# alibaba/EasyRec

Hardware: NVIDIA H100
Metric: samples_per_sec (higher is better)
Workload: dtype f32

## Files before the change

easyrec_b200/_lib.py:

```python
import ctypes
import os

import numpy as np

_HERE = os.path.dirname(os.path.abspath(__file__))
LIB_PATH = os.environ.get('ER_LIB_PATH') or os.path.join(_HERE, 'lib', 'liber_b200.so')

c_i32, c_i64, c_f32 = ctypes.c_int32, ctypes.c_int64, ctypes.c_float
c_vp, c_sz = ctypes.c_void_p, ctypes.c_size_t

SLOT_DTYPE = np.dtype(
    [('num_buckets', '<i8'), ('row_offset', '<i8'), ('seg_begin', '<i4'),
     ('n_seg', '<i4'), ('bucket_mode', '<i4'), ('combiner', '<i4'),
     ('out_buf', '<i4'), ('out_stride', '<i4'), ('out_col', '<i4'),
     ('shard_n', '<i4')],
    align=True)
assert SLOT_DTYPE.itemsize == 48
DENSE_SEG_DTYPE = np.dtype([('offset', '<i8'), ('n', '<i8'), ('l2', '<f4'), ('lr_mult', '<f4')], align=True)
assert DENSE_SEG_DTYPE.itemsize == 24

BUCKET_FARM_DECIMAL, BUCKET_MOD, BUCKET_IDENTITY, BUCKET_NONE, BUCKET_ONE_ROW = 0, 1, 2, 3, 4
COMBINER_SUM, COMBINER_MEAN, COMBINER_SQRTN = 0, 1, 2
COMBINER_UNIT_WEIGHTS = 16
OPT_SGD, OPT_ADAGRAD, OPT_LAZY_ADAM, OPT_ADAM_ROWS, OPT_MOMENTUM = 0, 1, 2, 3, 4
ACT_GELU, ACT_LEAKY_RELU, ACT_ELU, ACT_SELU, ACT_TANH, ACT_SWISH, ACT_SIGMOID = 1, 2, 3, 4, 5, 6, 7
MAX_BUFS = 8
ABI_VERSION = 3
HYPER_LR, HYPER_BETA1_POWER, HYPER_BETA2_POWER, HYPER_GRAD_SCALE, HYPER_N = 0, 1, 2, 3, 4


class ErOpt(ctypes.Structure):
  _fields_ = [('kind', c_i32), ('lr', c_f32), ('beta1', c_f32),
              ('beta2', c_f32), ('eps', c_f32), ('beta1_power', c_f32),
              ('beta2_power', c_f32), ('grad_scale', c_f32), ('hyper_dev', c_vp)]


class ErBnStats(ctypes.Structure):
  _fields_ = [('bias', c_vp), ('save_mean', c_vp), ('save_rstd', c_vp), ('moving_mean', c_vp),
              ('moving_var', c_vp), ('eps', c_f32), ('momentum', c_f32)]


class ErCsvCol(ctypes.Structure):
  _fields_ = [('kind', c_i32), ('width', c_i32), ('inner_sep', ctypes.c_char), ('kv_sep', ctypes.c_char), ('pad_', ctypes.c_char * 6),
              ('default_i64', c_i64), ('default_f32', c_f32), ('pad2_', c_i32), ('default_str', ctypes.c_char_p),
              ('out', c_vp), ('lens', c_vp), ('list_cap', c_i64), ('n_vals', c_i64), ('hash_mod', ctypes.c_uint64), ('weights', c_vp),
              ('step_lens', c_vp)]


ER_OK, ER_ERR_INVALID_ARG, ER_ERR_WORKSPACE, ER_ERR_CUDA, ER_ERR_UNSUPPORTED = range(5)
CSV_SKIP, CSV_I64, CSV_F32, CSV_HASH, CSV_I64_LIST, CSV_F32_VEC, CSV_HASH_LIST, CSV_I64_KV_LIST, CSV_HASH_KV_LIST, CSV_F32_LIST, \
    CSV_I64_STEP_LIST, CSV_HASH_STEP_LIST = range(12)

SIGNATURES = {
    'er_abi_version': (c_i32, []),
    'er_last_error': (ctypes.c_char_p, []),
    'er_launch_count': (ctypes.c_uint64, []),
    'er_csr_workspace_bytes': (c_sz, [c_i64]),
    'er_csr_from_lens': (c_i32, [c_vp, c_i64, c_vp, c_vp, c_i64, c_vp, c_sz,
                                 c_vp]),
    'er_bucketize': (c_i32, [c_vp, c_vp, c_vp, c_i64, c_i64, c_vp, c_i32,
                             c_vp, c_vp, c_vp]),
    'er_bucketize_weighted': (c_i32, [c_vp, c_vp, c_vp, c_vp, c_i64, c_i64, c_vp, c_i32,
                                      c_vp, c_vp, c_vp]),
    'er_bucketize_seq': (c_i32, [c_vp, c_vp, c_i64, c_i32, c_i32, c_vp, c_i32, c_vp, c_vp, c_vp]),
    'er_dropout': (c_i32, [c_vp, c_i64, ctypes.c_float, ctypes.c_uint64, c_vp, c_vp, c_vp]),
    'er_gemm_small_workspace_bytes': (c_sz, [c_i64, c_i64, c_i64]),
    'er_gemm_small': (c_i32, [c_vp, c_i64, c_i64, c_vp, c_i64, c_i64, c_vp, c_vp, c_i64, c_i64, c_i64, c_i64, c_vp, c_sz,
                              c_vp]),
    'er_dice_fwd': (c_i32, [c_vp, c_vp, c_vp, c_i64, c_i32, c_vp, c_vp]),
    'er_dice_bwd': (c_i32, [c_vp, c_vp, c_vp, c_vp, c_i64, c_i32, c_vp, c_vp, c_vp, c_vp]),
    'er_act_fwd': (c_i32, [c_vp, c_i64, c_i32, c_vp, c_vp]),
    'er_act_bwd': (c_i32, [c_vp, c_vp, c_i64, c_i32, c_vp, c_vp]),
    'er_auc_hist': (c_i32, [c_vp, c_vp, c_i64, c_vp, c_i32, c_vp, c_vp]),
    'er_shard_group_workspace_bytes': (c_sz, [c_i64]),
    'er_shard_group': (c_i32, [c_vp, c_vp, c_i64, c_i32, c_i64, c_vp, c_vp, c_vp, c_vp, c_sz, c_vp]),
    'er_fingerprint64_host': (ctypes.c_uint64, [ctypes.c_char_p, c_sz]),
    'er_csv_parse': (c_i32, [c_vp, c_sz, ctypes.c_char, ctypes.POINTER(ErCsvCol), c_i32, c_i64, c_i32,
                             ctypes.POINTER(c_i64), ctypes.POINTER(c_sz)]),
    'er_fingerprint64_i64': (c_i32, [c_vp, c_i64, c_vp]),
    'er_load_embed': (c_i32, [ctypes.c_char_p, ctypes.c_char_p, c_i32, c_i32, c_i32, c_i64, c_vp, c_vp]),
    'er_embedding_fwd': (c_i32, [
        c_vp, c_i64, c_i32, c_i32, c_vp, c_vp, c_vp, c_i64, c_i64, c_vp,
        c_i32, ctypes.POINTER(c_vp), c_i32, c_vp, c_vp
    ]),
    'er_embedding_bwd_workspace_bytes': (c_sz, [c_i64, c_i32]),
    'er_embedding_bwd_presort': (c_i32, [c_vp, c_i64, c_vp, c_vp, c_i64, c_i64, c_vp, c_i32, c_i32, c_vp, c_sz, c_vp]),
    'er_embedding_bwd_reuse_sort': (c_i32, [
        c_vp, c_vp, c_vp, c_i64, c_i32, c_i32, c_vp, c_vp, c_vp, c_vp, c_i64,
        c_i64, c_vp, c_i32, ctypes.POINTER(c_vp), c_i32, c_vp,
        ctypes.POINTER(ErOpt), c_vp, c_vp, c_vp, c_vp, c_sz, c_vp, c_sz, c_i32, c_vp
    ]),
    'er_embedding_bwd': (c_i32, [
        c_vp, c_vp, c_vp, c_i64, c_i32, c_i32, c_vp, c_vp, c_vp, c_vp, c_i64,
        c_i64, c_vp, c_i32, ctypes.POINTER(c_vp), c_i32, c_vp,
        ctypes.POINTER(ErOpt), c_vp, c_vp, c_vp, c_vp, c_sz, c_vp
    ]),
    'er_sparse_apply': (c_i32, [
        c_vp, c_vp, c_vp, c_i32, c_i32, c_vp, c_vp, c_vp, c_i64,
        ctypes.POINTER(ErOpt), c_vp
    ]),
    'er_adam_dense_sweep': (c_i32, [
        c_vp, c_vp, c_vp, c_i64, c_i32, c_i32, c_vp,
        ctypes.POINTER(ErOpt), c_vp
    ]),
    'er_mark_rows': (c_i32, [c_vp, c_i64, c_vp, c_i64, c_vp, c_i32, c_vp]),
    'er_sort_workspace_bytes': (c_sz, [c_i64]),
    'er_sort_rows': (c_i32, [c_vp, c_i64, c_vp, c_i64, c_vp, c_vp, c_vp, c_sz,
                             c_vp]),
    'er_fm_fwd': (c_i32, [c_vp, c_i64, c_i32, c_i32, c_i32, c_vp, c_vp]),
    'er_fm_bwd': (c_i32, [c_vp, c_vp, c_i64, c_i32, c_i32, c_i32, c_vp, c_i32,
                          c_i32, c_vp]),
    'er_sigmoid_ce_fwd_bwd': (c_i32, [c_vp, c_vp, c_vp, c_i64, c_f32, c_vp,
                                      c_vp, c_vp, c_vp]),
    'er_dense_workspace_bytes': (c_sz, [c_i64, c_i32]),
    'er_dense_apply': (c_i32, [c_vp, c_vp, c_vp, c_vp, c_vp, c_i32, c_i64, ctypes.POINTER(ErOpt), c_vp,
                               c_vp, c_vp]),
    'er_concat_cols': (c_i32, [ctypes.POINTER(c_vp), ctypes.POINTER(c_i32), ctypes.POINTER(c_i32), c_i32, c_i64,
                               c_vp, c_i32, c_vp]),
    'er_split_cols': (c_i32, [c_vp, c_i32, c_i64, ctypes.POINTER(c_vp), ctypes.POINTER(c_i32),
                              ctypes.POINTER(c_i32), c_i32, c_vp]),
    'er_rowsum_block_fwd': (c_i32, [c_vp, c_i64, c_i32, c_i32, c_vp, c_vp, c_vp, c_sz, c_vp]),
    'er_rowsum_block_bwd': (c_i32, [c_vp, c_vp, c_vp, c_f32, c_i64, c_i32, c_i32, c_vp, c_i32, c_vp]),
    'er_dense1_workspace_bytes': (c_sz, [c_i32]),
    'er_dense1_fwd': (c_i32, [c_vp, c_vp, c_vp, c_i64, c_i32, c_i32, c_vp, c_vp]),
    'er_dense1_bwd': (c_i32, [c_vp, c_vp, c_vp, c_i64, c_i32, c_i32, c_vp, c_i32, c_vp, c_vp, c_vp, c_sz, c_vp]),
    'er_gemm_bn_workspace_bytes': (c_sz, [c_i64, c_i64]),
    'er_gemm_bn': (c_i32, [c_vp, c_i64, c_i32, c_vp, c_i64, c_i32, c_vp, c_i64, c_i64, c_i64, c_i64,
                           ctypes.POINTER(ErBnStats), c_vp, c_sz, c_vp]),
    'er_bn_act_apply': (c_i32, [c_vp, c_vp, c_vp, c_vp, c_vp, c_vp, c_i64, c_i32, c_i32, c_vp, c_vp]),
    'er_fm_block_workspace_bytes': (c_sz, [c_i64]),
    'er_fm_block_fwd': (c_i32, [c_vp, c_i64, c_i32, c_i32, c_i32, c_vp, c_vp, c_vp, c_sz, c_vp]),
    'er_fm_block_bwd': (c_i32, [c_vp, c_vp, c_vp, c_vp, c_f32, c_i64, c_i32, c_i32, c_i32, c_i32, c_vp, c_i32,
                                c_vp]),
    'er_gemm_workspace_bytes': (c_sz, [c_i64, c_i64, c_i64]),
    'er_gemm': (c_i32, [c_vp, c_i64, c_i32, c_vp, c_i64, c_i32, c_vp, c_vp, c_i64, c_i64, c_i64, c_i64,
                        c_vp, c_sz, c_vp]),
    'er_bias_bn_act_fwd': (c_i32, [c_vp, c_vp, c_vp, c_vp, c_vp, c_vp, c_i64,
                                   c_i32, c_f32, c_f32, c_i32, c_i32, c_vp,
                                   c_vp, c_vp, c_vp, c_sz, c_vp]),
    'er_bias_bn_act_bwd': (c_i32, [c_vp, c_vp, c_vp, c_vp, c_vp, c_vp, c_vp,
                                   c_i64, c_i32, c_i32, c_vp, c_vp, c_vp, c_vp,
                                   c_vp, c_sz, c_vp]),
    'er_din_concat_fwd': (c_i32, [c_vp, c_vp, c_i64, c_i32, c_i32, c_vp, c_vp]),
    'er_din_concat_bwd': (c_i32, [c_vp, c_vp, c_vp, c_i64, c_i32, c_i32, c_vp, c_vp, c_i32, c_vp]),
    'er_din_pool_fwd': (c_i32, [c_vp, c_vp, c_vp, c_i64, c_i32, c_i32, c_vp, c_vp, c_vp]),
    'er_din_pool_bwd': (c_i32, [c_vp, c_vp, c_vp, c_vp, c_i64, c_i32, c_i32, c_vp, c_vp, c_i32, c_vp]),
    'er_din_sigmoid_pool_fwd': (c_i32, [c_vp, c_vp, c_vp, c_i64, c_i32, c_i32, c_f32, c_vp, c_vp, c_vp]),
    'er_din_sigmoid_pool_bwd': (c_i32, [c_vp, c_vp, c_vp, c_vp, c_i64, c_i32, c_i32, c_f32, c_vp, c_vp, c_i32,
                                        c_vp]),
    'er_cross_fwd': (c_i32, [c_vp, c_vp, c_vp, c_vp, c_i64, c_i32, c_vp, c_vp, c_vp]),
    'er_cross_workspace_bytes': (c_sz, [c_i64, c_i32]),
    'er_cross_bwd': (c_i32, [c_vp, c_vp, c_vp, c_vp, c_vp, c_i64, c_i32, c_vp, c_vp, c_vp, c_vp, c_i32,
                             c_vp, c_sz, c_vp]),
    'er_mmoe_mix_fwd': (c_i32, [c_vp, c_vp, c_i64, c_i32, c_i32, c_vp, c_vp, c_vp]),
    'er_mmoe_mix_bwd': (c_i32, [c_vp, c_vp, c_vp, c_i64, c_i32, c_i32, c_vp, c_vp, c_i32, c_vp]),
    'er_gram_fwd': (c_i32, [c_vp, c_i64, c_i32, c_i32, c_vp, c_vp]),
    'er_gram_bwd': (c_i32, [c_vp, c_vp, c_i64, c_i32, c_i32, c_vp, c_vp]),
    'er_l2norm_fwd': (c_i32, [c_vp, c_i64, c_i32, c_vp, c_vp, c_vp]),
    'er_l2norm_bwd': (c_i32, [c_vp, c_vp, c_vp, c_i64, c_i32, c_vp, c_vp]),
    'er_inbatch_softmax_ce': (c_i32, [c_vp, c_vp, c_vp, c_i64, c_i32, c_f32, c_vp, c_vp, c_vp, c_vp]),
}

_lib = None


class ErError(RuntimeError):
  pass


def load():
  global _lib
  if _lib is not None:
    return _lib
  if not os.path.exists(LIB_PATH):
    raise ErError(
        'liber_b200.so not found at %s: build it with '
        '`python -c "import __graft_entry__ as g; g.build()"` or '
        '`make -C easyrec_b200/csrc`. There is no CPU fallback.' % LIB_PATH)
  lib = ctypes.CDLL(LIB_PATH)
  for name, (res, args) in SIGNATURES.items():
    fn = getattr(lib, name)
    fn.restype = res
    fn.argtypes = args
  if lib.er_abi_version() != ABI_VERSION:
    raise ErError('liber_b200.so has ABI version %d, this binding needs %d: rebuild it (make -C easyrec_b200/csrc)'
                  % (lib.er_abi_version(), ABI_VERSION))
  _lib = lib
  return lib


def check(status, what):
  if status != 0:
    msg = load().er_last_error()
    raise ErError('%s failed (status %d): %s' %
                  (what, status, msg.decode() if msg else ''))


def fingerprint64(data):
  if isinstance(data, str):
    data = data.encode('utf-8')
  return int(load().er_fingerprint64_host(data, len(data)))
```

easyrec_b200/csrc/embedding_bwd.cu:

```cuda
#include "common.cuh"
#include "scan.cuh"
#include "slots.cuh"
#include "sort.cuh"
#include "bucket_bwd.cuh"

namespace er {

struct CBufs {
  const float* p[ER_MAX_BUFS];
};

constexpr int kLongRun = 64;
constexpr int kBatch = 4;
constexpr int kChunk = 512;

struct BwdArgs {
  float* table;
  float* state0;
  float* state1;
  int dim;
  int row_stride;
  uint32_t sentinel;
  const uint32_t* keys;
  const uint32_t* vals;
  const uint64_t* pairs;
  int64_t n;
  const float* weights;
  const int32_t* seg_ids;
  const er_slot_t* slots;
  int n_slots;
  CBufs gbufs;
  const float* seg_scale;
  er_opt_t opt;
  float lr_t;
  const float* hyper;
  int64_t* uniq_rows;
  float* uniq_grads;
  const int32_t* head_rank;
  int32_t* counters;
  int4* long_list;
  int32_t* run_done;
  int2* chunk_list;
  float* partials;
  const int64_t* or_rows;
  float* or_partials;
  int32_t* or_tickets;
  int or_chunks;
  int main_ctas;
};

__device__ __forceinline__ const float* grad_src(const BwdArgs& a, const SlotView& sv, uint32_t l,
                                                 float* coef) {
  const int32_t s = a.seg_ids ? a.seg_ids[l] : (int32_t)l;
  const SlotLite sl = slot_lite(sv, slot_of(sv, s));
  float c = (a.weights && !slot_unit_weights(sl)) ? a.weights[l] : 1.0f;
  if (a.seg_scale) c = __fmul_rn(c, a.seg_scale[s]);
  *coef = c;
  return a.gbufs.p[sl.misc & 0xff] + (int64_t)(s - sl.seg_begin) * sl.out_stride + sl.out_col;
}

struct Hyper {
  float lr, lr_t, grad_scale;
};

__device__ __forceinline__ Hyper load_hyper(const er_opt_t& o, float lr_t_arg, const float* __restrict__ hyper) {
  Hyper h;
  if (hyper) {
    h.lr = __ldg(hyper + ER_HYPER_LR);
    h.grad_scale = __ldg(hyper + ER_HYPER_GRAD_SCALE);
    h.lr_t = h.lr;
    if (o.kind == ER_OPT_LAZY_ADAM || o.kind == ER_OPT_ADAM_ROWS)
      h.lr_t = adam_lr_t_of(h.lr, __ldg(hyper + ER_HYPER_BETA1_POWER), __ldg(hyper + ER_HYPER_BETA2_POWER));
  } else {
    h.lr = o.lr;
    h.lr_t = lr_t_arg;
    h.grad_scale = o.grad_scale;
  }
  return h;
}

__device__ __forceinline__ void upd_one(const BwdArgs& a, const Hyper& h, float g, float& w, float& s0, float& s1) {
  switch (a.opt.kind) {
    case ER_OPT_ADAGRAD: {
      s0 = __fadd_rn(s0, __fmul_rn(g, g));
      w = __fsub_rn(w, __fmul_rn(__fmul_rn(h.lr, g), __frsqrt_rn(s0)));
      break;
    }
    case ER_OPT_LAZY_ADAM:
    case ER_OPT_ADAM_ROWS: {
      s0 = __fadd_rn(__fmul_rn(g, 1.0f - a.opt.beta1), __fmul_rn(s0, a.opt.beta1));
      s1 = __fadd_rn(__fmul_rn(__fmul_rn(g, g), 1.0f - a.opt.beta2), __fmul_rn(s1, a.opt.beta2));
      w = __fadd_rn(w, __fdiv_rn(__fmul_rn(-h.lr_t, s0), __fadd_rn(__fsqrt_rn(s1), a.opt.eps)));
      break;
    }
    case ER_OPT_MOMENTUM: {
      s0 = __fadd_rn(__fmul_rn(s0, a.opt.beta1), g);
      w = __fsub_rn(w, __fmul_rn(h.lr, s0));
      break;
    }
    default:
      w = __fsub_rn(w, __fmul_rn(h.lr, g));
  }
}

__device__ __forceinline__ void f4_fma_sep(float4& g, const float4& v, float c) {
  g.x = __fadd_rn(g.x, __fmul_rn(v.x, c));
  g.y = __fadd_rn(g.y, __fmul_rn(v.y, c));
  g.z = __fadd_rn(g.z, __fmul_rn(v.z, c));
  g.w = __fadd_rn(g.w, __fmul_rn(v.w, c));
}
__device__ __forceinline__ void f4_acc(float4& g, const float4& v) {
  g.x = __fadd_rn(g.x, v.x);
  g.y = __fadd_rn(g.y, v.y);
  g.z = __fadd_rn(g.z, v.z);
  g.w = __fadd_rn(g.w, v.w);
}

__device__ __forceinline__ float4 f4_scale1(const float4& v, float c) {
  return make_float4(__fmul_rn(v.x, c), __fmul_rn(v.y, c), __fmul_rn(v.z, c), __fmul_rn(v.w, c));
}

struct RowRegs {
  float4 w, s0, s1;
};

__device__ __forceinline__ RowRegs load_row(const BwdArgs& a, uint32_t row, int lane) {
  RowRegs r;
  r.w = r.s0 = r.s1 = make_float4(0.f, 0.f, 0.f, 0.f);
  if (!a.table) return r;
  const int64_t off = (int64_t)row * a.row_stride;
  r.w = reinterpret_cast<const float4*>(a.table + off)[lane];
  if (a.state0) r.s0 = reinterpret_cast<const float4*>(a.state0 + off)[lane];
  if (a.state1) r.s1 = reinterpret_cast<const float4*>(a.state1 + off)[lane];
  return r;
}

__device__ __forceinline__ void apply_row_vec(const BwdArgs& a, uint32_t row, int lane, float4 g,
                                              int64_t head_pos, RowRegs r) {
  const Hyper h = load_hyper(a.opt, a.lr_t, a.hyper);
  g.x = __fmul_rn(g.x, h.grad_scale);
  g.y = __fmul_rn(g.y, h.grad_scale);
  g.z = __fmul_rn(g.z, h.grad_scale);
  g.w = __fmul_rn(g.w, h.grad_scale);
  if (a.uniq_rows) {
    const int32_t u = a.head_rank[head_pos];
    if (lane == 0) a.uniq_rows[u] = (int64_t)row;
    reinterpret_cast<float4*>(a.uniq_grads + (int64_t)u * a.dim)[lane] = g;
  }
  if (!a.table) return;
  upd_one(a, h, g.x, r.w.x, r.s0.x, r.s1.x);
  upd_one(a, h, g.y, r.w.y, r.s0.y, r.s1.y);
  upd_one(a, h, g.z, r.w.z, r.s0.z, r.s1.z);
  upd_one(a, h, g.w, r.w.w, r.s0.w, r.s1.w);
  const int64_t off = (int64_t)row * a.row_stride;
  reinterpret_cast<float4*>(a.table + off)[lane] = r.w;
  if (a.state0) reinterpret_cast<float4*>(a.state0 + off)[lane] = r.s0;
  if (a.state1) reinterpret_cast<float4*>(a.state1 + off)[lane] = r.s1;
}

// ... 221 lines not shown
  }
}

template <int LANES>
__global__ void __launch_bounds__(256) bwd_scan_vec_kernel(const __grid_constant__ BwdArgs a) {
  extern __shared__ __align__(16) unsigned char s_raw[];
  const SlotView sv = load_slots(s_raw, a.slots, a.n_slots);
  constexpr int D4 = LANES;
  constexpr int GROUPS = 32 / LANES;
  float4* s_stage = reinterpret_cast<float4*>(s_raw + ((slot_smem_bytes(a.n_slots) + 15) & ~(size_t)15));
  const int warp = threadIdx.x >> 5, lane = threadIdx.x & 31;
  float4* my_stage = s_stage + (size_t)warp * 32 * D4;
  __shared__ int s_tail_lane[8][32];
  __shared__ int s_tail_head[8][32];
  const int64_t base = ((int64_t)blockIdx.x * 8 + warp) * 32;
  if (base >= a.n) return;
  const int64_t pos = base + lane;
  const bool in = pos < a.n;
  const uint32_t k = in ? a.keys[pos] : a.sentinel;
  const uint32_t l = in ? a.vals[pos] : 0u;
  const bool valid = in && k < a.sentinel;
  uint32_t kprev = __shfl_up_sync(0xffffffffu, k, 1);
  if (lane == 0) kprev = (base > 0) ? a.keys[base - 1] : ~k;
  uint32_t knext = __shfl_down_sync(0xffffffffu, k, 1);
  if (lane == 31) knext = (base + 32 < a.n) ? a.keys[base + 32] : ~k;
  const bool is_head = valid && (pos == 0 || kprev != k);
  const uint32_t k0 = __shfl_sync(0xffffffffu, k, 0);
  const int head0 = __shfl_sync(0xffffffffu, (int)is_head, 0);
  const bool owned = valid && (head0 || k != k0);
  bool is_tail = owned && (knext != k);
  const int cont = __shfl_sync(0xffffffffu, (int)(owned && knext == k), 31);
  const unsigned lt_mask = (1u << lane) - 1u;
  const unsigned tails0 = __ballot_sync(0xffffffffu, is_tail || (lane == 31 && cont));
  if (is_tail || (lane == 31 && cont)) s_tail_lane[warp][__popc(tails0 & lt_mask)] = lane;
  __syncwarp();
  const int n_tails = __popc(tails0);
  const int glane = lane % LANES, grp = lane / LANES;
  RowRegs row0, row1;
  uint32_t row0_key = a.sentinel, row1_key = a.sentinel;
  if (grp < n_tails) {
    const int tl = s_tail_lane[warp][grp];
    row0_key = a.keys[base + tl];
    row0 = load_row(a, row0_key, glane);
  }
  if (grp + GROUPS < n_tails) {
    const int tl = s_tail_lane[warp][grp + GROUPS];
    row1_key = a.keys[base + tl];
    row1 = load_row(a, row1_key, glane);
  }
  float4 g[D4];
#pragma unroll
  for (int c = 0; c < D4; ++c) g[c] = make_float4(0.f, 0.f, 0.f, 0.f);
  if (owned) {
    float coef;
    const float4* src = reinterpret_cast<const float4*>(grad_src(a, sv, l, &coef));
    float4 v[D4];
#pragma unroll
    for (int c = 0; c < D4; ++c) v[c] = src[c];
#pragma unroll
    for (int c = 0; c < D4; ++c) f4_fma_sep(g[c], v[c], coef);
  }
  int cnt = owned ? 1 : 0;
#pragma unroll
  for (int off = 1; off < 32; off <<= 1) {
    const uint32_t kk = __shfl_up_sync(0xffffffffu, k, off);
    const int oo = __shfl_up_sync(0xffffffffu, (int)owned, off);
    const int cc = __shfl_up_sync(0xffffffffu, cnt, off);
    const bool take = lane >= off && owned && oo && kk == k;
#pragma unroll
    for (int c = 0; c < D4; ++c) {
      float4 y;
      y.x = __shfl_up_sync(0xffffffffu, g[c].x, off);
      y.y = __shfl_up_sync(0xffffffffu, g[c].y, off);
      y.z = __shfl_up_sync(0xffffffffu, g[c].z, off);
      y.w = __shfl_up_sync(0xffffffffu, g[c].w, off);
      if (take) f4_acc(g[c], y);
    }
    if (take) cnt += cc;
  }
  int handed_off = 0;
  if (cont) {
    const uint32_t key = __shfl_sync(0xffffffffu, k, 31);
    int total = __shfl_sync(0xffffffffu, cnt, 31);
    const int64_t start = base + 32 - total;
    int64_t j = base + 32;
    while (true) {
      const int64_t p = j + lane;
      const bool m = p < a.n && a.keys[p] == key;
      const unsigned mm = __ballot_sync(0xffffffffu, m);
      float4 x[D4];
#pragma unroll
      for (int c = 0; c < D4; ++c) x[c] = make_float4(0.f, 0.f, 0.f, 0.f);
      if (m) {
        float coef;
        const float4* src = reinterpret_cast<const float4*>(grad_src(a, sv, a.vals[p], &coef));
#pragma unroll
        for (int c = 0; c < D4; ++c) f4_fma_sep(x[c], src[c], coef);
      }
#pragma unroll
      for (int o = 16; o >= 1; o >>= 1) {
#pragma unroll
        for (int c = 0; c < D4; ++c) {
          float4 y;
          y.x = __shfl_xor_sync(0xffffffffu, x[c].x, o);
          y.y = __shfl_xor_sync(0xffffffffu, x[c].y, o);
          y.z = __shfl_xor_sync(0xffffffffu, x[c].z, o);
          y.w = __shfl_xor_sync(0xffffffffu, x[c].w, o);
          f4_acc(x[c], y);
        }
      }
      if (lane == 31) {
#pragma unroll
        for (int c = 0; c < D4; ++c) f4_acc(g[c], x[c]);
      }
      const int got = __popc(mm);
      total += got;
      j += got;
      if (mm != 0xffffffffu) break;
      if (total >= kLongRun) {
        if (j < a.n && a.keys[j] == key) {
          if (lane == 0) enqueue_long(a, start, j, key);
          handed_off = 1;
        }
        break;
      }
    }
  }
  const bool finish = (is_tail || (lane == 31 && cont && !handed_off));
  if (finish) {
#pragma unroll
    for (int c = 0; c < D4; ++c) my_stage[lane * D4 + c] = g[c];
  }
  if (is_tail || (lane == 31 && cont))
    s_tail_head[warp][__popc(tails0 & lt_mask)] = (lane == 31 && cont && handed_off) ? -1 : cnt;
  __syncwarp();
  for (int r = grp; r < n_tails; r += GROUPS) {
    const int tl = s_tail_lane[warp][r];
    const int run_cnt = s_tail_head[warp][r];
    if (run_cnt < 0) continue;
    const uint32_t key = (r == grp) ? row0_key : (r == grp + GROUPS) ? row1_key : a.keys[base + tl];
    RowRegs row = (r == grp) ? row0 : (r == grp + GROUPS) ? row1 : load_row(a, key, glane);
    const int64_t head_pos = base + tl - (run_cnt - 1);
    apply_row_vec(a, key, glane, my_stage[tl * D4 + glane], head_pos, row);
  }
}

__device__ __forceinline__ uint32_t key_at(const BwdArgs& a, int64_t i) {
  return a.pairs ? (uint32_t)(a.pairs[i] >> 32) : a.keys[i];
}
__device__ __forceinline__ uint32_t val_at(const BwdArgs& a, int64_t i) {
  return a.pairs ? (uint32_t)a.pairs[i] : a.vals[i];
}

template <int LANES, int TPE>
__global__ void __launch_bounds__(256) bwd_long_vec_kernel(const __grid_constant__ BwdArgs a) {
  extern __shared__ __align__(16) unsigned char s_raw[];
  const SlotView sv = load_slots(s_raw, a.slots, a.n_slots);
  float4* s_part = reinterpret_cast<float4*>(s_raw + ((slot_smem_bytes(a.n_slots) + 15) & ~(size_t)15));
  __shared__ int s_last;
  constexpr int CH = LANES / TPE;
  constexpr int G = 256 / TPE;
  const int lane32 = threadIdx.x & 31, warp = threadIdx.x >> 5;
  const int sub = threadIdx.x % TPE;
  const int grp = threadIdx.x / TPE;
  const int n_chunks = a.counters[1];
  for (int x = blockIdx.x; x < n_chunks; x += gridDim.x) {
    const int2 qc = a.chunk_list[x];
    const int4 run = a.long_list[qc.x];
    const int64_t i = run.x;
    const int len = run.y, c0 = run.z, nch = run.w;
    const uint32_t key = key_at(a, i);
    const int e0 = qc.y * kChunk, e1 = min(len, e0 + kChunk);
    float4 g[CH];
#pragma unroll
    for (int c = 0; c < CH; ++c) g[c] = make_float4(0.f, 0.f, 0.f, 0.f);
    for (int e = e0 + grp; e < e1; e += 2 * G) {
      const bool two = (e + G < e1);
      float w0, w1 = 0.f;
      const float* p0 = grad_src(a, sv, val_at(a, i + e), &w0);
      const float* p1 = two ? grad_src(a, sv, val_at(a, i + e + G), &w1) : p0;
      float4 v0[CH], v1[CH];
#pragma unroll
      for (int c = 0; c < CH; ++c) {
        v0[c] = reinterpret_cast<const float4*>(p0)[sub * CH + c];
        v1[c] = reinterpret_cast<const float4*>(p1)[sub * CH + c];
      }
#pragma unroll
      for (int c = 0; c < CH; ++c) {
        f4_fma_sep(g[c], v0[c], w0);
        if (two) f4_fma_sep(g[c], v1[c], w1);
      }
    }
#pragma unroll
    for (int o = 16; o >= TPE; o >>= 1) {
#pragma unroll
      for (int c = 0; c < CH; ++c) {
        float4 y;
        y.x = __shfl_xor_sync(0xffffffffu, g[c].x, o);
        y.y = __shfl_xor_sync(0xffffffffu, g[c].y, o);
        y.z = __shfl_xor_sync(0xffffffffu, g[c].z, o);
        y.w = __shfl_xor_sync(0xffffffffu, g[c].w, o);
        f4_acc(g[c], y);
      }
    }
    if (lane32 < TPE) {
#pragma unroll
      for (int c = 0; c < CH; ++c) s_part[warp * LANES + lane32 * CH + c] = g[c];
    }
    __syncthreads();
    float4 tot = make_float4(0.f, 0.f, 0.f, 0.f);
    if (threadIdx.x < LANES) {
      for (int ww = 0; ww < 8; ++ww) f4_acc(tot, s_part[ww * LANES + threadIdx.x]);
    }
    bool finish = (nch == 1);
    if (nch > 1) {
      if (threadIdx.x < LANES)
        __stcg(reinterpret_cast<float4*>(a.partials + (int64_t)(c0 + qc.y) * a.dim) + threadIdx.x, tot);
      __threadfence();
      __syncthreads();
      if (threadIdx.x == 0) s_last = (atomicAdd(&a.run_done[qc.x], 1) == nch - 1);
      __syncthreads();
      finish = s_last != 0;
      if (finish && threadIdx.x < LANES) {
        __threadfence();
        tot = make_float4(0.f, 0.f, 0.f, 0.f);
        for (int c = 0; c < nch; ++c)
          f4_acc(tot, __ldcg(reinterpret_cast<const float4*>(a.partials + (int64_t)(c0 + c) * a.dim) +
                             threadIdx.x));
      }
    }
    if (finish && threadIdx.x < LANES) {
      RowRegs row = load_row(a, key, threadIdx.x);
      apply_row_vec(a, key, threadIdx.x, tot, i, row);
    }
    __syncthreads();
  }
}

__global__ void __launch_bounds__(256) bwd_runs_scalar_kernel(const __grid_constant__ BwdArgs a) {
  extern __shared__ __align__(16) unsigned char s_raw[];
  const SlotView sv = load_slots(s_raw, a.slots, a.n_slots);
  const int64_t t = (int64_t)blockIdx.x * blockDim.x + threadIdx.x;
  const int64_t i = t / a.dim;
  const int c = (int)(t - i * a.dim);
  if (i >= a.n) return;
  const uint32_t key = a.keys[i];
  if (key >= a.sentinel) return;
  if (i > 0 && a.keys[i - 1] == key) return;
  float g = 0.f;
  int64_t j = i;
  for (; j < a.n && a.keys[j] == key; ++j) {
    if (j - i >= kLongRun) {
      if (c == 0) enqueue_long(a, i, j, key);
      return;
    }
    float coef;
    const float* src = grad_src(a, sv, a.vals[j], &coef);
    g = __fadd_rn(g, __fmul_rn(src[c], coef));
  }
  apply_scalar(a, key, c, g, i);
}

__global__ void __launch_bounds__(256) bwd_long_scalar_kernel(const __grid_constant__ BwdArgs a) {
  extern __shared__ __align__(16) unsigned char s_raw[];
  const SlotView sv = load_slots(s_raw, a.slots, a.n_slots);
  __shared__ float s_w[8];
  __shared__ int s_last;
  const int lane32 = threadIdx.x & 31, warp = threadIdx.x >> 5;
  const int n_chunks = a.counters[1];
  for (int x = blockIdx.x; x < n_chunks; x += gridDim.x) {
    const int2 qc = a.chunk_list[x];
    const int4 run = a.long_list[qc.x];
    const int64_t i = run.x;
    const int len = run.y, c0 = run.z, nch = run.w;
    const uint32_t key = key_at(a, i);
    const int e0 = qc.y * kChunk, e1 = min(len, e0 + kChunk);
    for (int c = 0; c < a.dim; ++c) {
      float g = 0.f;
      for (int e = e0 + threadIdx.x; e < e1; e += 256) {
        float coef;
        const float* src = grad_src(a, sv, val_at(a, i + e), &coef);
        g = __fadd_rn(g, __fmul_rn(src[c], coef));
      }
#pragma unroll
      for (int o = 16; o >= 1; o >>= 1) g = __fadd_rn(g, __shfl_xor_sync(0xffffffffu, g, o));
      if (lane32 == 0) s_w[warp] = g;
      __syncthreads();
      if (threadIdx.x == 0) {
        float tot = 0.f;
        for (int ww = 0; ww < 8; ++ww) tot = __fadd_rn(tot, s_w[ww]);
        if (nch == 1)
          apply_scalar(a, key, c, tot, i);
        else
          __stcg(a.partials + (int64_t)(c0 + qc.y) * a.dim + c, tot);
      }
      __syncthreads();
    }
    if (nch > 1) {
      __threadfence();
      __syncthreads();
      if (threadIdx.x == 0) s_last = (atomicAdd(&a.run_done[qc.x], 1) == nch - 1);
      __syncthreads();
      if (s_last && (int)threadIdx.x < a.dim) {
        __threadfence();
        float tot = 0.f;
        for (int c = 0; c < nch; ++c)
          tot = __fadd_rn(tot, __ldcg(a.partials + (int64_t)(c0 + c) * a.dim + threadIdx.x));
        apply_scalar(a, key, (int)threadIdx.x, tot, i);
      }
      __syncthreads();
    }
  }
}

__global__ void __launch_bounds__(256) bwd_scan_d1_kernel(const __grid_constant__ BwdArgs a) {
  extern __shared__ __align__(16) unsigned char s_raw[];
  const SlotView sv = load_slots(s_raw, a.slots, a.n_slots);
  const int warp = threadIdx.x >> 5, lane = threadIdx.x & 31;
  const int64_t base = ((int64_t)blockIdx.x * 8 + warp) * 32;
  if (base >= a.n) return;
  const int64_t pos = base + lane;
  const bool in = pos < a.n;
  const uint32_t k = in ? a.keys[pos] : a.sentinel;
  const uint32_t l = in ? a.vals[pos] : 0u;
  const bool valid = in && k < a.sentinel;
  uint32_t kprev = __shfl_up_sync(0xffffffffu, k, 1);
  if (lane == 0) kprev = (base > 0) ? a.keys[base - 1] : ~k;
  uint32_t knext = __shfl_down_sync(0xffffffffu, k, 1);
  if (lane == 31) knext = (base + 32 < a.n) ? a.keys[base + 32] : ~k;
  const bool is_head = valid && (pos == 0 || kprev != k);
  const uint32_t k0 = __shfl_sync(0xffffffffu, k, 0);
  const int head0 = __shfl_sync(0xffffffffu, (int)is_head, 0);
  const bool owned = valid && (head0 || k != k0);
  const bool is_tail = owned && (knext != k);
  const int cont = __shfl_sync(0xffffffffu, (int)(owned && knext == k), 31);
  float g = 0.f;
  if (owned) {
    float coef;
    const float* src = grad_src(a, sv, l, &coef);
    g = __fmul_rn(src[0], coef);
  }
  int cnt = owned ? 1 : 0;
#pragma unroll
  for (int off = 1; off < 32; off <<= 1) {
    const uint32_t kk = __shfl_up_sync(0xffffffffu, k, off);
    const int oo = __shfl_up_sync(0xffffffffu, (int)owned, off);
    const int cc = __shfl_up_sync(0xffffffffu, cnt, off);
    const float y = __shfl_up_sync(0xffffffffu, g, off);
    if (lane >= off && owned && oo && kk == k) {
      g = __fadd_rn(g, y);
      cnt += cc;
    }
  }
  int handed_off = 0;
  if (cont) {
    const uint32_t key = __shfl_sync(0xffffffffu, k, 31);
    int total = __shfl_sync(0xffffffffu, cnt, 31);
    const int64_t start = base + 32 - total;
    int64_t j = base + 32;
    while (true) {
      const int64_t p = j + lane;
      const bool m = p < a.n && a.keys[p] == key;
      const unsigned mm = __ballot_sync(0xffffffffu, m);
      float x = 0.f;
      if (m) {
        float coef;
        const float* src = grad_src(a, sv, a.vals[p], &coef);
        x = __fmul_rn(src[0], coef);
      }
#pragma unroll
      for (int o = 16; o >= 1; o >>= 1) x = __fadd_rn(x, __shfl_xor_sync(0xffffffffu, x, o));
      if (lane == 31) g = __fadd_rn(g, x);
      const int got = __popc(mm);
      total += got;
      j += got;
      if (mm != 0xffffffffu) break;
      if (total >= kLongRun) {
        if (j < a.n && a.keys[j] == key) {
          if (lane == 0) enqueue_long(a, start, j, key);
          handed_off = 1;
        }
        break;
      }
    }
  }
  if (is_tail || (lane == 31 && cont && !handed_off)) apply_scalar(a, k, 0, g, pos - (cnt - 1));
}

#ifndef ER_BK_MINB
#define ER_BK_MINB 4
#endif

struct BkArgs {
  bk::Ws w;
  int log2_nb;
  int warp_ctas;
  int med_ctas;
};

template <int LANES>
__device__ __forceinline__ float4 sum_entries(const BwdArgs& a, const SlotView& sv, const uint64_t* sp, int j0, int j1,
                                              int lane) {
  float4 g = make_float4(0.f, 0.f, 0.f, 0.f);
  for (int j = j0; j < j1; j += kBatch) {
    float4 gv[kBatch];
    float c[kBatch];
#pragma unroll
    for (int u = 0; u < kBatch; ++u) {
      if (j + u < j1) {
        const float* src = grad_src(a, sv, (uint32_t)sp[j + u], &c[u]);
        gv[u] = reinterpret_cast<const float4*>(src)[lane];
      }
    }
#pragma unroll
    for (int u = 0; u < kBatch; ++u)
      if (j + u < j1) f4_fma_sep(g, gv[u], c[u]);
  }
  return g;
}

constexpr int kStageF4 = 1024;
constexpr uint32_t kDonePos = 0xFFFFFFFFu;

template <typename IdxT>
__device__ __forceinline__ bool run_is_long(const IdxT* s_start, int r) {
  return (int)s_start[r + 1] - (int)s_start[r] > bk::kCoopRun;
}

template <int LANES, int THREADS, typename IdxT>
__device__ __forceinline__ void process_runs_vec(const BwdArgs& a, const SlotView& sv, uint64_t* sp,
                                                 const IdxT* s_start, int R, float4* s_stage, float4* s_part,
                                                 int* s_coop, int* s_ncoop, int64_t queue_base) {
  constexpr int G = THREADS / LANES;
  constexpr int S_ENT = kStageF4 / LANES;
  const int grp = threadIdx.x / LANES, lane = threadIdx.x % LANES;
  if (threadIdx.x == 0) *s_ncoop = 0;
  __syncthreads();
  for (int r = threadIdx.x; r < R; r += THREADS)
    if (run_is_long(s_start, r)) s_coop[atomicAdd(s_ncoop, 1)] = r;
  __syncthreads();
  const int nco = *s_ncoop;
  for (int c = 0; c < nco; ++c) {
    const int r = s_coop[c];
    const int st = s_start[r], en = s_start[r + 1], len = en - st;
    if (queue_base >= 0 && len > bk::kQueueRun) {
      if (threadIdx.x == 0) enqueue_run(a, queue_base + st, len);
    } else {
      const int chunk = (len + G - 1) / G;
      const int j0 = st + grp * chunk, j1 = min(en, j0 + chunk);
      const float4 g = sum_entries<LANES>(a, sv, sp, j0, j1, lane);
      s_part[grp * LANES + lane] = g;
      __syncthreads();
      if (threadIdx.x < LANES) {
        const uint32_t key = (uint32_t)(sp[st] >> 32);
        RowRegs row = load_row(a, key, threadIdx.x);
        const int used = (len + chunk - 1) / chunk;
        float4 tot = make_float4(0.f, 0.f, 0.f, 0.f);
        for (int q = 0; q < used; ++q) f4_acc(tot, s_part[q * LANES + threadIdx.x]);
        apply_row_vec(a, key, threadIdx.x, tot, 0, row);
      }
    }
    __syncthreads();
    for (int i = st + threadIdx.x; i < en; i += THREADS) sp[i] |= (uint64_t)kDonePos;
  }
  __syncthreads();
  const int n = s_start[R];
  int r = grp;
  while (r < R && run_is_long(s_start, r)) r += G;
  RowRegs row;
  row.w = row.s0 = row.s1 = make_float4(0.f, 0.f, 0.f, 0.f);
  if (r < R) row = load_row(a, (uint32_t)(sp[s_start[r]] >> 32), lane);
  float4 acc = make_float4(0.f, 0.f, 0.f, 0.f);
  for (int c0 = 0; c0 < n; c0 += S_ENT) {
    const int c1 = min(n, c0 + S_ENT);
    for (int q = threadIdx.x; q < (c1 - c0) * LANES; q += THREADS) {
      const int e = q / LANES;
      const uint32_t pos = (uint32_t)sp[c0 + e];
      if (pos != kDonePos) {
        float coef;
        const float* src = grad_src(a, sv, pos, &coef);
        s_stage[q] = f4_scale1(reinterpret_cast<const float4*>(src)[q % LANES], coef);
      }
    }
    __syncthreads();
    while (r < R && (int)s_start[r] < c1) {
      const int st = s_start[r], en = s_start[r + 1];
      const int lo = max(st, c0), hi = min(en, c1);
      for (int i = lo; i < hi; ++i) f4_acc(acc, s_stage[(i - c0) * LANES + lane]);
      if (en > c1) break;
      const uint32_t key = (uint32_t)(sp[st] >> 32);
      int rn = r + G;
      while (rn < R && run_is_long(s_start, rn)) rn += G;
      RowRegs nxt;
      nxt.w = nxt.s0 = nxt.s1 = make_float4(0.f, 0.f, 0.f, 0.f);
      if (rn < R) nxt = load_row(a, (uint32_t)(sp[s_start[rn]] >> 32), lane);
      apply_row_vec(a, key, lane, acc, 0, row);
      acc = make_float4(0.f, 0.f, 0.f, 0.f);
      row = nxt;
      r = rn;
    }
    __syncthreads();
  }
}

template <int THREADS, typename IdxT>
__device__ __forceinline__ void process_runs_scalar(const BwdArgs& a, const SlotView& sv, uint64_t* sp,
                                                    const IdxT* s_start, int R, float* s_stagef, float* s_partf,
                                                    int* s_coop, int* s_ncoop, int64_t queue_base) {
  const int dim = a.dim;
  if (threadIdx.x == 0) *s_ncoop = 0;
  __syncthreads();
  for (int r = threadIdx.x; r < R; r += THREADS)
    if (run_is_long(s_start, r)) s_coop[atomicAdd(s_ncoop, 1)] = r;
  __syncthreads();
  const int nco = *s_ncoop;
  for (int cc = 0; cc < nco; ++cc) {
    const int r = s_coop[cc];
    const int st = s_start[r], en = s_start[r + 1], len = en - st;
    if (queue_base >= 0 && len > bk::kQueueRun) {
      if (threadIdx.x == 0) enqueue_run(a, queue_base + st, len);
    } else {
      const int chunk = (len + THREADS - 1) / THREADS;
      const int j0 = st + threadIdx.x * chunk, j1 = min(en, j0 + chunk);
      const int used = (len + chunk - 1) / chunk;
      for (int c = 0; c < dim; ++c) {
        float g = 0.f;
        for (int j = j0; j < j1; ++j) {
          float coef;
          const float* src = grad_src(a, sv, (uint32_t)sp[j], &coef);
          g = __fadd_rn(g, __fmul_rn(src[c], coef));
        }
        s_partf[threadIdx.x] = g;
        __syncthreads();
        if (threadIdx.x == 0) {
          float tot = 0.f;
          for (int q = 0; q < used; ++q) tot = __fadd_rn(tot, s_partf[q]);
          apply_scalar(a, (uint32_t)(sp[st] >> 32), c, tot, 0);
        }
        __syncthreads();
      }
    }
    __syncthreads();
    for (int i = st + threadIdx.x; i < en; i += THREADS) sp[i] |= (uint64_t)kDonePos;
  }
  __syncthreads();
  const int n = s_start[R];
  const int S_ENT = max(1, (kStageF4 * 4) / dim);
  const int total = R * dim;
  int idx = threadIdx.x;
  float acc = 0.f;
  for (int c0 = 0; c0 < n; c0 += S_ENT) {
    const int c1 = min(n, c0 + S_ENT);
    for (int q = threadIdx.x; q < (c1 - c0) * dim; q += THREADS) {
      const int e = q / dim;
      const uint32_t pos = (uint32_t)sp[c0 + e];
      if (pos != kDonePos) {
        float coef;
        const float* src = grad_src(a, sv, pos, &coef);
        s_stagef[q] = __fmul_rn(src[q - e * dim], coef);
      }
    }
    __syncthreads();
    while (idx < total) {
      const int r = idx / dim, c = idx - r * dim;
      if (run_is_long(s_start, r)) {
        idx += THREADS;
        continue;
      }
      const int st = s_start[r], en = s_start[r + 1];
      if (st >= c1) break;
      const int lo = max(st, c0), hi = min(en, c1);
      for (int i = lo; i < hi; ++i) acc = __fadd_rn(acc, s_stagef[(i - c0) * dim + c]);
      if (en > c1) break;
      apply_scalar(a, (uint32_t)(sp[st] >> 32), c, acc, 0);
      acc = 0.f;
      idx += THREADS;
    }
    __syncthreads();
  }
}

inline size_t bk_reduce_smem(int n_slots, int cap, int threads) {
  return ((slot_smem_bytes(n_slots) + 15) & ~(size_t)15) + (size_t)cap * 8 + (((size_t)(cap + 1) * 2 + 15) & ~(size_t)15) +
         (size_t)max(kStageF4, threads) * 16 + (size_t)(cap / bk::kCoopRun + 2) * 4 + 64;
}

struct BkSmem {
  uint64_t* pairs;
  uint16_t* start;
  float4* stage;
  float4* part;
  int* coop;
  int* ncoop;
};
__device__ __forceinline__ BkSmem bk_carve(unsigned char* s_raw, int n_slots, int cap, int threads) {
  BkSmem m;
  unsigned char* p = s_raw + ((slot_smem_bytes(n_slots) + 15) & ~(size_t)15);
  m.pairs = reinterpret_cast<uint64_t*>(p); p += (size_t)cap * 8;
  m.start = reinterpret_cast<uint16_t*>(p); p += ((size_t)(cap + 1) * 2 + 15) & ~(size_t)15;
  m.stage = reinterpret_cast<float4*>(p); p += (size_t)max(kStageF4, threads) * 16;
  m.part = m.stage;
  m.coop = reinterpret_cast<int*>(p); p += (size_t)(cap / bk::kCoopRun + 1) * 4;
  m.ncoop = reinterpret_cast<int*>(p);
  return m;
}

__device__ __forceinline__ void cx(uint64_t& lo, uint64_t& hi, bool up) {
  if ((lo > hi) == up) {
    const uint64_t t = lo;
    lo = hi;
    hi = t;
  }
}

template <int LANES>
struct WarpSmem {
  float4 stage[32 * LANES];
  float4 carry[LANES];
  uint32_t keys[32];
};

__device__ __forceinline__ void sort4(uint64_t (&x)[4], int P, int lane) {
  for (int kk = 2; kk <= P; kk <<= 1) {
    for (int j = kk >> 1; j > 0; j >>= 1) {
      if (j == 64) {
        cx(x[0], x[2], ((lane) & kk) == 0);
        cx(x[1], x[3], ((lane + 32) & kk) == 0);
      } else if (j == 32) {
        cx(x[0], x[1], ((lane) & kk) == 0);
        if (P > 64) cx(x[2], x[3], ((lane + 64) & kk) == 0);
      } else {
        const bool lower = (lane & j) == 0;
#pragma unroll
        for (int r = 0; r < 4; ++r) {
          if (r * 32 < P) {
            const uint64_t other = __shfl_xor_sync(0xffffffffu, x[r], j);
            const bool up = ((lane + 32 * r) & kk) == 0;
            if ((x[r] > other) == (lower == up)) x[r] = other;
          }
        }
      }
    }
  }
}

template <int LANES>
__device__ __forceinline__ void warp_bucket_vec(const BwdArgs& a, const SlotView& sv, const BkArgs& k, int b,
                                                WarpSmem<LANES>* ws) {
  constexpr int G = 32 / LANES;
  const int lane = threadIdx.x & 31;
  const int gi = lane / LANES, gl = lane % LANES;
  const int n = k.w.bcnt[b];
  if (n == 0 || n > bk::kWarpCap) return;
  const int64_t off = k.w.boff[b];
  uint64_t x[4];
#pragma unroll
  for (int r = 0; r < 4; ++r) {
    const int q = r * 32 + lane;
    x[r] = q < n ? k.w.pairs[off + q] : ~0ull;
  }
  sort4(x, n <= 32 ? 32 : (n <= 64 ? 64 : 128), lane);
  uint32_t carry_key = 0xFFFFFFFFu;
#pragma unroll
  for (int r = 0; r < 4; ++r) {
    if (r * 32 >= n) break;
    const uint32_t key = (uint32_t)(x[r] >> 32), pos = (uint32_t)x[r];
    const int nv = min(32, n - r * 32);
    const uint32_t next_first = (r < 3 && (r + 1) * 32 < n) ? __shfl_sync(0xffffffffu, (uint32_t)(x[r < 3 ? r + 1 : 3] >> 32), 0)
                                                            : 0xFFFFFFFFu;
    uint32_t prevk = __shfl_up_sync(0xffffffffu, key, 1);
    if (lane == 0) prevk = carry_key;
    const bool is_head = lane < nv && key != prevk;
    const unsigned H = __ballot_sync(0xffffffffu, is_head);
    const int nh = __popc(H);
    ws->keys[lane] = key;
    const float4 open_sum = ws->carry[gl];
    RowRegs row0, row1;
    row0.w = row0.s0 = row0.s1 = row1.w = row1.s0 = row1.s1 = make_float4(0.f, 0.f, 0.f, 0.f);
    {
      const unsigned h0 = __fns(H, 0, gi + 1), h1 = __fns(H, 0, gi + G + 1);
      const uint32_t k0 = __shfl_sync(0xffffffffu, key, h0 & 31), k1 = __shfl_sync(0xffffffffu, key, h1 & 31);
      if (gi < nh) row0 = load_row(a, k0, gl);
      if (gi + G < nh) row1 = load_row(a, k1, gl);
    }
#pragma unroll
    for (int t = 0; t < LANES; ++t) {
      const int e = t * G + gi;
      const uint32_t pe = __shfl_sync(0xffffffffu, pos, e);
      if (e < nv) {
        float coef;
        const float* src = grad_src(a, sv, pe, &coef);
        ws->stage[e * LANES + gl] = f4_scale1(reinterpret_cast<const float4*>(src)[gl], coef);
      }
    }
    __syncwarp();
    const uint32_t lastk = ws->keys[31];
    const bool chunk_open = (nv == 32) && next_first == lastk;
    const int lead = nh ? (__ffs(H) - 1) : nv;
    if (lead > 0 && gi == 0) {
      float4 acc = open_sum;
      for (int i = 0; i < lead; ++i) f4_acc(acc, ws->stage[i * LANES + gl]);
      if (lead == 32 && chunk_open) {
        ws->carry[gl] = acc;
      } else {
        RowRegs row = load_row(a, carry_key, gl);
        apply_row_vec(a, carry_key, gl, acc, 0, row);
      }
    }
    for (int q = gi; q < nh; q += G) {
      const int h = __fns(H, 0, q + 1);
      const unsigned rest = (h == 31) ? 0u : (H >> (h + 1)) << (h + 1);
      const int e_end = rest ? (__ffs(rest) - 1) : nv;
      const uint32_t kh = ws->keys[h];
      float4 acc = make_float4(0.f, 0.f, 0.f, 0.f);
      for (int i = h; i < e_end; ++i) f4_acc(acc, ws->stage[i * LANES + gl]);
      if (e_end == 32 && chunk_open) {
        ws->carry[gl] = acc;
      } else {
        RowRegs row = (q == gi) ? row0 : (q == gi + G) ? row1 : load_row(a, kh, gl);
        apply_row_vec(a, kh, gl, acc, 0, row);
      }
    }
    carry_key = chunk_open ? lastk : 0xFFFFFFFFu;
    __syncwarp();
  }
}

struct WarpSmem1 {
  float stage[32];
  float carry;
  uint32_t keys[32];
};

__device__ __forceinline__ void warp_bucket_d1(const BwdArgs& a, const SlotView& sv, const BkArgs& k, int b,
                                               WarpSmem1* ws) {
  const int lane = threadIdx.x & 31;
  const int n = k.w.bcnt[b];
  if (n == 0 || n > bk::kWarpCap) return;
  const int64_t off = k.w.boff[b];
  uint64_t x[4];
#pragma unroll
  for (int r = 0; r < 4; ++r) {
    const int q = r * 32 + lane;
    x[r] = q < n ? k.w.pairs[off + q] : ~0ull;
  }
  sort4(x, n <= 32 ? 32 : (n <= 64 ? 64 : 128), lane);
  uint32_t carry_key = 0xFFFFFFFFu;
#pragma unroll
  for (int r = 0; r < 4; ++r) {
    if (r * 32 >= n) break;
    const uint32_t key = (uint32_t)(x[r] >> 32), pos = (uint32_t)x[r];
    const int nv = min(32, n - r * 32);
    const uint32_t next_first = (r < 3 && (r + 1) * 32 < n) ? __shfl_sync(0xffffffffu, (uint32_t)(x[r < 3 ? r + 1 : 3] >> 32), 0)
                                                            : 0xFFFFFFFFu;
    uint32_t prevk = __shfl_up_sync(0xffffffffu, key, 1);
    if (lane == 0) prevk = carry_key;
    const bool is_head = lane < nv && key != prevk;
    const unsigned H = __ballot_sync(0xffffffffu, is_head);
    const int nh = __popc(H);
    ws->keys[lane] = key;
    const float open_sum = ws->carry;
    if (lane < nv) {
      float coef;
      const float* src = grad_src(a, sv, pos, &coef);
      ws->stage[lane] = __fmul_rn(src[0], coef);
    }
    __syncwarp();
    const uint32_t lastk = ws->keys[31];
    const bool chunk_open = (nv == 32) && next_first == lastk;
    const int lead = nh ? (__ffs(H) - 1) : nv;
    if (lead > 0 && lane == 31) {
      float acc = open_sum;
      for (int i = 0; i < lead; ++i) acc = __fadd_rn(acc, ws->stage[i]);
      if (lead == 32 && chunk_open)
        ws->carry = acc;
      else
        apply_scalar(a, carry_key, 0, acc, 0);
    }
    if (lane < nh && !(lead > 0 && lane == 31)) {
      const int h = __fns(H, 0, lane + 1);
      const unsigned rest = (h == 31) ? 0u : (H >> (h + 1)) << (h + 1);
      const int e_end = rest ? (__ffs(rest) - 1) : nv;
      float acc = 0.f;
      for (int i = h; i < e_end; ++i) acc = __fadd_rn(acc, ws->stage[i]);
      if (e_end == 32 && chunk_open)
        ws->carry = acc;
      else
        apply_scalar(a, ws->keys[h], 0, acc, 0);
    }
    carry_key = chunk_open ? lastk : 0xFFFFFFFFu;
    __syncwarp();
  }
}

constexpr bool warp_mode_lanes(int lanes) { return lanes == 1 || lanes == 2 || lanes == 4 || lanes == 8; }

template <int LANES>
inline size_t bk_fused_smem(int n_slots, bool warp_mode) {
  size_t warp_bytes = 0;
  if (warp_mode) {
    if constexpr (LANES > 0)
      warp_bytes = ((slot_smem_bytes(n_slots) + 15) & ~(size_t)15) + 8 * sizeof(WarpSmem<(LANES > 0 && LANES <= 8) ? LANES : 1>);
    else
      warp_bytes = ((slot_smem_bytes(n_slots) + 15) & ~(size_t)15) + 8 * sizeof(WarpSmem1);
  }
  const size_t med = bk_reduce_smem(n_slots, bk::kCap, bk::kThreads);
  return warp_bytes > med ? warp_bytes : med;
}

template <int LANES>
__global__ void __launch_bounds__(bk::kThreads, ER_BK_MINB) bk_fused_kernel(const __grid_constant__ BwdArgs a,
                                                                const __grid_constant__ BkArgs k) {
  extern __shared__ __align__(16) unsigned char s_raw[];
  __shared__ int s_warp[bk::kThreads / 32 + 1];
  const int bid = blockIdx.x;
  if (bid >= k.warp_ctas + k.med_ctas) {
    one_row_cta<LANES>(a, bid - k.warp_ctas - k.med_ctas);
    return;
  }
  const SlotView sv = load_slots(s_raw, a.slots, a.n_slots);
  if (bid < k.warp_ctas) {
    unsigned char* p = s_raw + ((slot_smem_bytes(a.n_slots) + 15) & ~(size_t)15);
    const int b = bid * 8 + (threadIdx.x >> 5);
    if constexpr (LANES > 0 && LANES <= 8) {
      warp_bucket_vec<LANES>(a, sv, k, b, reinterpret_cast<WarpSmem<LANES>*>(p) + (threadIdx.x >> 5));
    } else if constexpr (LANES == 0) {
      warp_bucket_d1(a, sv, k, b, reinterpret_cast<WarpSmem1*>(p) + (threadIdx.x >> 5));
    }
    return;
  }
  const BkSmem m = bk_carve(s_raw, a.n_slots, bk::kCap, bk::kThreads);
  const int n_med = k.w.n_big[1];
  for (int xi = bid - k.warp_ctas; xi < n_med; xi += k.med_ctas) {
    const int b = k.w.med_list[xi];
    const int n = k.w.bcnt[b];
    const int off = k.w.boff[b];
    int P = 32;
    while (P < n) P <<= 1;
    for (int i = threadIdx.x; i < P; i += bk::kThreads) m.pairs[i] = i < n ? k.w.pairs[off + i] : ~0ull;
    __syncthreads();
    bk::bitonic_sort<bk::kThreads>(m.pairs, P);
    const int R = bk::run_starts<bk::kThreads, bk::kCap / bk::kThreads>(m.pairs, n, m.start, s_warp);
    if constexpr (LANES > 0)
      process_runs_vec<LANES, bk::kThreads>(a, sv, m.pairs, m.start, R, m.stage, m.part, m.coop, m.ncoop, -1);
    else
      process_runs_scalar<bk::kThreads>(a, sv, m.pairs, m.start, R, reinterpret_cast<float*>(m.stage),
                                        reinterpret_cast<float*>(m.part), m.coop, m.ncoop, -1);
    __syncthreads();
  }
}

__device__ __forceinline__ bool cta_radix_pass(const uint64_t* __restrict__ in, uint64_t* __restrict__ out, int n,
                                               int shift, int* s_wh , int* s_cur ) {
  const int lane = threadIdx.x & 31, wid = threadIdx.x >> 5;
  const unsigned lt_mask = (1u << lane) - 1u;
  for (int i = threadIdx.x; i < 256; i += bk::kBigThreads) s_cur[i] = 0;
  __syncthreads();
  for (int i = threadIdx.x; i < n; i += bk::kBigThreads) atomicAdd(&s_cur[(int)((in[i] >> shift) & 255)], 1);
  __syncthreads();
  int single = 0;
  if (threadIdx.x < 256) single = (s_cur[threadIdx.x] == n);
  if (__syncthreads_or(single)) return false;
  if (threadIdx.x < 32) {
    int carry = 0;
    for (int base = 0; base < 256; base += 32) {
      const int v = s_cur[base + lane];
      int incl = v;
#pragma unroll
      for (int o = 1; o < 32; o <<= 1) {
        const int t = __shfl_up_sync(0xffffffffu, incl, o);
        if (lane >= o) incl += t;
      }
      s_cur[base + lane] = carry + incl - v;
      carry += __shfl_sync(0xffffffffu, incl, 31);
    }
  }
  __syncthreads();
  for (int base = 0; base < n; base += bk::kBigThreads) {
    for (int i = threadIdx.x; i < 32 * 256; i += bk::kBigThreads) s_wh[i] = 0;
    __syncthreads();
    const int i = base + threadIdx.x;
    const bool valid = i < n;
    const uint64_t e = valid ? in[i] : 0ull;
    const int d = (int)((e >> shift) & 255);
    const unsigned peers = __match_any_sync(0xffffffffu, valid ? d : (256 + lane));
    const int r = __popc(peers & lt_mask);
    if (valid && r == 0) s_wh[wid * 256 + d] = __popc(peers);
    __syncthreads();
    if (threadIdx.x < 256) {
      int run = s_cur[threadIdx.x];
      for (int ww = 0; ww < 32; ++ww) {
        const int t = s_wh[ww * 256 + threadIdx.x];
        s_wh[ww * 256 + threadIdx.x] = run;
        run += t;
      }
      s_cur[threadIdx.x] = run;
    }
    __syncthreads();
    if (valid) out[s_wh[wid * 256 + d] + r] = e;
    __syncthreads();
  }
  return true;
}

template <int LANES>
__global__ void __launch_bounds__(bk::kBigThreads) bk_reduce_big_kernel(const __grid_constant__ BwdArgs a,
                                                                        const __grid_constant__ BkArgs k) {
  extern __shared__ __align__(16) unsigned char s_raw[];
  __shared__ int s_warp[bk::kBigThreads / 32 + 1];
  __shared__ int s_flag;
  const int n_big = k.w.n_big[0];
  if ((int)blockIdx.x >= n_big) return;
  const SlotView sv = load_slots(s_raw, a.slots, a.n_slots);
  const BkSmem m = bk_carve(s_raw, a.n_slots, bk::kBigCap, bk::kBigThreads);
  for (int x = blockIdx.x; x < n_big; x += gridDim.x) {
    const int b = k.w.big_list[x];
    const int n = k.w.bcnt[b];
    const int64_t off = k.w.boff[b];
    uint64_t* gp = k.w.pairs + off;
    bool sorted_in_global = false;
    if (n > bk::kBigCap) {
      int* s_wh = reinterpret_cast<int*>(m.pairs);
      int* s_cur = s_wh + 32 * 256;
      uint64_t* src = gp;
      uint64_t* dst = k.w.pairs_tmp + off;
      for (int shift = 0; shift < 64; shift += 8) {
        if (cta_radix_pass(src, dst, n, shift, s_wh, s_cur)) {
          uint64_t* t = src; src = dst; dst = t;
        }
        __syncthreads();
      }
      if (src != gp) {
        for (int i = threadIdx.x; i < n; i += bk::kBigThreads) gp[i] = src[i];
      }
      __threadfence_block();
      __syncthreads();
      sorted_in_global = true;
    }
    int p = 0;
    while (p < n) {
      const int mwin = min(bk::kBigCap, n - p);
      if (!sorted_in_global) {
        int P = 32;
        while (P < mwin) P <<= 1;
        for (int i = threadIdx.x; i < P; i += bk::kBigThreads) m.pairs[i] = i < mwin ? gp[i] : ~0ull;
        __syncthreads();
        bk::bitonic_sort<bk::kBigThreads>(m.pairs, P);
      } else {
        for (int i = threadIdx.x; i < mwin; i += bk::kBigThreads) m.pairs[i] = gp[p + i];
        __syncthreads();
      }
      int R = bk::run_starts<bk::kBigThreads, bk::kBigCap / bk::kBigThreads>(m.pairs, mwin, m.start, s_warp);
      int advance = mwin;
      if (sorted_in_global && p + mwin < n &&
          (uint32_t)(m.pairs[mwin - 1] >> 32) == (uint32_t)(gp[p + mwin] >> 32)) {
        if (R == 1) {
          const uint32_t key = (uint32_t)(m.pairs[0] >> 32);
          int lo = p + mwin, hi = n;
          while (lo < hi) {
            const int mid = (lo + hi) >> 1;
            if ((uint32_t)(gp[mid] >> 32) <= key) lo = mid + 1; else hi = mid;
          }
          if (threadIdx.x == 0) enqueue_run(a, off + p, lo - p);
          p = lo;
          __syncthreads();
          continue;
        }
        advance = m.start[R - 1];
        R -= 1;
      }
      if (!sorted_in_global) {
        if (threadIdx.x == 0) s_flag = 0;
        __syncthreads();
        for (int r = threadIdx.x; r < R; r += bk::kBigThreads)
          if (m.start[r + 1] - m.start[r] > bk::kQueueRun) s_flag = 1;
        __syncthreads();
        if (s_flag)
          for (int i = threadIdx.x; i < mwin; i += bk::kBigThreads) gp[i] = m.pairs[i];
      }
      if constexpr (LANES > 0)
        process_runs_vec<LANES, bk::kBigThreads>(a, sv, m.pairs, m.start, R, m.stage, m.part, m.coop, m.ncoop, off + p);
      else
        process_runs_scalar<bk::kBigThreads>(a, sv, m.pairs, m.start, R, reinterpret_cast<float*>(m.stage),
                                             reinterpret_cast<float*>(m.part), m.coop, m.ncoop, off + p);
      p += advance;
      __syncthreads();
    }
  }
}

struct HeadIn {
  const uint32_t* keys;
  uint32_t sentinel;
  __device__ int operator()(int64_t j) const {
    uint32_t k = keys[j];
    return (k < sentinel && (j == 0 || keys[j - 1] != k)) ? 1 : 0;
  }
};
struct HeadOut {
  int32_t* rank;
  __device__ void operator()(int64_t j, int ex, int) const { rank[j] = ex; }
};

inline size_t a256(size_t x) { return (x + 255) & ~(size_t)255; }

struct BwdWs {
  uint32_t* keys;
  uint32_t* vals;
  int32_t* head_rank;
  int4* long_list;
  int32_t* run_done;
  int2* chunk_list;
  float* partials;
  int32_t* counters;
  void* sort_ws;
  void* scan_ws;
  bk::Ws bk;
  int32_t* tickets;
  float* one_row_partials;
};

inline int64_t max_long_runs(int64_t n) { return n / kLongRun + 1; }
inline int64_t max_chunks(int64_t n) { return n / kChunk + max_long_runs(n) + 1; }
inline int64_t max_one_row_parts(int64_t n) { return n / bk::kOneRowChunk + 2048 + 1; }

inline BwdWs bwd_carve(void* ws, int64_t n, int dim, char** end = nullptr) {
  char* p = reinterpret_cast<char*>(a256(reinterpret_cast<size_t>(ws)));
  BwdWs w;
  w.keys = reinterpret_cast<uint32_t*>(p); p += a256((size_t)n * 4);
  w.vals = reinterpret_cast<uint32_t*>(p); p += a256((size_t)n * 4);
  w.head_rank = reinterpret_cast<int32_t*>(p); p += a256((size_t)n * 4);
  w.long_list = reinterpret_cast<int4*>(p); p += a256((size_t)max_long_runs(n) * 16);
  w.run_done = reinterpret_cast<int32_t*>(p); p += a256((size_t)max_long_runs(n) * 4);
  w.chunk_list = reinterpret_cast<int2*>(p); p += a256((size_t)max_chunks(n) * 8);
  w.partials = reinterpret_cast<float*>(p); p += a256((size_t)max_chunks(n) * dim * 4);
  w.bk = bk::carve(p, n, &w.counters, &w.tickets, &p);
  w.one_row_partials = reinterpret_cast<float*>(p); p += a256((size_t)max_one_row_parts(n) * dim * 4);
  w.sort_ws = p; p += a256(rsort::workspace_bytes(n));
  w.scan_ws = p; p += a256(scan::workspace_bytes(n));
  if (end) *end = p;
  return w;
}

inline size_t bwd_ws_bytes(int64_t n, int dim) {
  char* end;
  bwd_carve(nullptr, n, dim, &end);
  return reinterpret_cast<size_t>(end) + 768;
}

static float adam_lr_t(const er_opt_t& o) { return adam_lr_t_of(o.lr, o.beta1_power, o.beta2_power); }

template <int LANES>
static void launch_long(const BwdArgs& a, cudaStream_t st) {
  const size_t sl = slot_smem_bytes(a.n_slots);
  if constexpr (LANES > 0) {
    constexpr int TPE = (LANES <= 8) ? 1 : LANES;
    const size_t smem_long = ((sl + 15) & ~(size_t)15) + (size_t)8 * LANES * sizeof(float4);
    bwd_long_vec_kernel<LANES, TPE><<<4 * kSmCount, 256, smem_long, st>>>(a);
  } else {
    bwd_long_scalar_kernel<<<4 * kSmCount, 256, sl, st>>>(a);
  }
}

template <int LANES>
static void launch_radix(const BwdArgs& a, cudaStream_t st) {
  const size_t smem = slot_smem_bytes(a.n_slots);
  const unsigned grid = (unsigned)ceil_div(a.n, 256);
  if constexpr (LANES > 8) {
    bwd_runs_vec_kernel<LANES><<<grid, 256, smem, st>>>(a);
  } else if constexpr (LANES > 0) {
    const size_t smem_scan = ((smem + 15) & ~(size_t)15) + (size_t)8 * 32 * LANES * sizeof(float4);
    bwd_scan_vec_kernel<LANES><<<grid, 256, smem_scan, st>>>(a);
  } else if (a.dim == 1) {
    bwd_scan_d1_kernel<<<grid, 256, smem, st>>>(a);
  } else {
    bwd_runs_scalar_kernel<<<(unsigned)ceil_div(a.n * a.dim, 256), 256, smem, st>>>(a);
  }
  launch_long<LANES>(a, st);
  count_launches(2);
}

static int log2_of(int v) {
  int l = 0;
  while ((1 << l) < v) ++l;
  return l;
}

static bool k7_warp_mode(int dim) { return dim == 1 || dim == 4 || dim == 8 || dim == 16 || dim == 32; }

static void bk_place(const int64_t* rows, int64_t cap, const int32_t* n_dev, int64_t n_rows, const int32_t* seg_ids,
                     const er_slot_t* slots, int n_slots, bool one_row, bool warp_mode, const BwdWs& w,
                     bool zero_call_block, cudaStream_t st) {
  bk::PlaceArgs pa;
  pa.rows = rows;
  pa.cap = cap;
  pa.n_dev = n_dev;
  pa.sentinel = (uint32_t)n_rows;
  pa.seg_ids = seg_ids;
  pa.slots = one_row ? slots : nullptr;
  pa.n_slots = n_slots;
  const int nb = bk::num_buckets(cap, warp_mode);
  pa.log2_nb = log2_of(nb);
  pa.warp_cap = warp_mode ? bk::kWarpCap : 0;
  pa.w = w.bk;
  cudaMemsetAsync(w.bk.bcnt, 0, bk::zero_place_bytes() + (zero_call_block ? bk::zero_call_bytes() : 0), st);
  const size_t smem = bk::place_smem_bytes(n_slots, nb, pa.slots != nullptr);
  static bool attr = false;
  if (!attr) {
    const int mx = (int)bk::place_smem_bytes(2048, bk::kMaxBuckets, true);
    cudaFuncSetAttribute(bk::bk_count_kernel, cudaFuncAttributeMaxDynamicSharedMemorySize, mx);
    cudaFuncSetAttribute(bk::bk_place_kernel, cudaFuncAttributeMaxDynamicSharedMemorySize, mx);
    attr = true;
  }
  const unsigned tiles = (unsigned)ceil_div(cap, (int64_t)bk::kTile);
  bk::bk_count_kernel<<<tiles, bk::kTileThreads, smem, st>>>(pa);
  bk::bk_place_kernel<<<tiles, bk::kTileThreads, smem, st>>>(pa);
  count_launches(2);
}

template <int LANES>
static void bk_launch_fused(BwdArgs a, const BwdWs& place, bool place_warp_mode, cudaStream_t st) {
  BkArgs k;
  k.w = place.bk;
  const int nb = bk::num_buckets(a.n, place_warp_mode);
  k.log2_nb = log2_of(nb);
  k.warp_ctas = place_warp_mode ? (nb >> 3) : 0;
  k.med_ctas = place_warp_mode ? kSmCount : nb;
  const size_t smem = bk_fused_smem<LANES>(a.n_slots, place_warp_mode);
  const size_t smem_big = bk_reduce_smem(a.n_slots, bk::kBigCap, bk::kBigThreads);
  static bool attr = false;
  if (!attr) {
    cudaFuncSetAttribute(bk_fused_kernel<LANES>, cudaFuncAttributeMaxDynamicSharedMemorySize,
                         (int)bk_fused_smem<LANES>(2048, true));
    cudaFuncSetAttribute(bk_fused_kernel<LANES>, cudaFuncAttributePreferredSharedMemoryCarveout,
                         (int)cudaSharedmemCarveoutMaxShared);
    cudaFuncSetAttribute(bk_reduce_big_kernel<LANES>, cudaFuncAttributeMaxDynamicSharedMemorySize,
                         (int)bk_reduce_smem(2048, bk::kBigCap, bk::kBigThreads));
    attr = true;
  }
  const int extra = a.or_chunks * a.n_slots;
  a.main_ctas = k.warp_ctas + k.med_ctas;
  bk_fused_kernel<LANES><<<k.warp_ctas + k.med_ctas + extra, bk::kThreads, smem, st>>>(a, k);
  bk_reduce_big_kernel<LANES><<<kSmCount, bk::kBigThreads, smem_big, st>>>(a, k);
  launch_long<LANES>(a, st);
  count_launches(3);
}

}

extern "C" size_t er_sort_workspace_bytes(int64_t n) { return er::rsort::workspace_bytes(n > 0 ? n : 1); }

extern "C" int er_sort_rows(const int64_t* rows, int64_t n, const int32_t* n_dev, int64_t max_row,
                            uint32_t* keys_out, uint32_t* vals_out, void* ws, size_t ws_bytes,
                            er_stream_t stream) {
  using namespace er;
  ER_REQUIRE(rows && keys_out && vals_out, "null argument");
  ER_REQUIRE(n > 0 && n < (1LL << 31), "n out of range");
  ER_REQUIRE(max_row > 0 && max_row < 0xFFFFFFFFLL, "max_row must be in (0, 2^32-1)");
  if (!ws || ws_bytes < rsort::workspace_bytes(n))
    return fail(ER_ERR_WORKSPACE, "er_sort_rows: workspace too small");
  rsort::sort_rows(rows, n, n_dev, max_row, keys_out, vals_out, ws, nullptr, as_stream(stream));
  ER_CUDA_LAUNCH_CHECK();
  return ER_OK;
}

extern "C" size_t er_embedding_bwd_workspace_bytes(int64_t n_lookups_cap, int32_t dim) {
  return er::bwd_ws_bytes(n_lookups_cap > 0 ? n_lookups_cap : 1, dim > 0 ? dim : 1);
}

static int embedding_bwd_impl(float* table, float* state0, float* state1, int64_t n_rows,
                              int32_t dim, int32_t row_stride, const int64_t* rows,
                              const float* weights, const int32_t* seg_ids,
                              const int32_t* row_ptr, int64_t n_seg, int64_t n_lookups_cap,
                              const er_slot_t* slots, int32_t n_slots,
                              const float* const* grad_bufs, int32_t n_bufs,
                              const float* seg_scale, const er_opt_t* opt, int64_t* uniq_rows,
                              float* uniq_grads, int32_t* n_uniq, void* ws, size_t ws_bytes,
                              const void* sorted_ws, size_t sorted_ws_bytes, int32_t sorted_dim,
                              er_stream_t stream) {
  using namespace er;
  ER_REQUIRE(rows && slots && grad_bufs && opt, "null argument");
  ER_REQUIRE(table || uniq_rows, "nothing to do: table and uniq_rows are both NULL");
  ER_REQUIRE((uniq_rows == nullptr) == (uniq_grads == nullptr) &&
                 (uniq_rows == nullptr) == (n_uniq == nullptr),
             "uniq_rows, uniq_grads and n_uniq go together");
  ER_REQUIRE(dim > 0 && row_stride >= dim, "bad dim / row_stride");
  ER_REQUIRE(n_rows > 0 && n_rows < 0xFFFFFFFFLL, "n_rows must be in (0, 2^32-1)");
  ER_REQUIRE(n_slots > 0 && n_slots <= 2048, "n_slots must be in [1, 2048]");
  ER_REQUIRE(n_bufs > 0 && n_bufs <= ER_MAX_BUFS, "n_bufs must be in [1, ER_MAX_BUFS]");
  ER_REQUIRE(n_lookups_cap >= 0 && n_lookups_cap < (1LL << 31), "n_lookups_cap out of range");
  ER_REQUIRE(row_ptr || seg_ids || n_lookups_cap == n_seg,
             "without row_ptr / seg_ids every segment must hold exactly one lookup");
  ER_REQUIRE(!row_ptr || seg_ids, "CSR input needs seg_ids (er_csr_from_lens)");
  if (table) {
    const int k = opt->kind;
    ER_REQUIRE(k == ER_OPT_SGD || k == ER_OPT_ADAGRAD || k == ER_OPT_LAZY_ADAM || k == ER_OPT_ADAM_ROWS || k == ER_OPT_MOMENTUM,
               "unknown optimizer kind");
    ER_REQUIRE(k == ER_OPT_SGD || state0, "optimizer state0 missing");
    ER_REQUIRE((k != ER_OPT_LAZY_ADAM && k != ER_OPT_ADAM_ROWS) || state1, "adam needs state1 (v)");
  }
  if (n_lookups_cap == 0) return ER_OK;
  if (!ws || ws_bytes < bwd_ws_bytes(n_lookups_cap, dim))
    return fail(ER_ERR_WORKSPACE, "er_embedding_bwd: workspace too small");
  cudaStream_t st = as_stream(stream);
  BwdWs w = bwd_carve(ws, n_lookups_cap, dim);
  const int32_t* n_dev = row_ptr ? row_ptr + n_seg : nullptr;
  const bool bucketed = (uniq_rows == nullptr);
  const bool one_row = bucketed && seg_ids == nullptr;
  BwdWs src = w;
  if (sorted_ws) {
    if (sorted_ws_bytes < bwd_ws_bytes(n_lookups_cap, sorted_dim))
      return fail(ER_ERR_WORKSPACE, "er_embedding_bwd_reuse_sort: source workspace too small");
    if (!bucketed)
      return fail(ER_ERR_UNSUPPORTED, "er_embedding_bwd_reuse_sort: uniq_rows output needs the rows (er_embedding_bwd)");
    if (k7_warp_mode(sorted_dim) != k7_warp_mode(dim))
      return fail(ER_ERR_UNSUPPORTED, "er_embedding_bwd_reuse_sort: the placement was made in the other placement mode "
                                      "(warp-sized buckets for dims 1, 4, 8, 16 and 32, CTA-sized for the others)");
    src = bwd_carve(const_cast<void*>(sorted_ws), n_lookups_cap, sorted_dim);
    cudaMemsetAsync(w.counters, 0, bk::zero_call_bytes(), st);
  } else if (bucketed) {
    bk_place(rows, n_lookups_cap, n_dev, n_rows, seg_ids, slots, n_slots, one_row, k7_warp_mode(dim), w, true, st);
  } else {
    rsort::sort_rows(rows, n_lookups_cap, n_dev, n_rows, w.keys, w.vals, w.sort_ws, w.counters, st);
  }
  const bool place_warp = k7_warp_mode(dim);

  BwdArgs a = {};
  a.table = table;
  a.state0 = state0;
  a.state1 = state1;
  a.dim = dim;
  a.row_stride = row_stride;
  a.sentinel = (uint32_t)n_rows;
  a.keys = w.keys;
  a.vals = w.vals;
  a.pairs = nullptr;
  a.n = n_lookups_cap;
  a.weights = weights;
  a.seg_ids = seg_ids;
  a.slots = slots;
  a.n_slots = n_slots;
  bool aligned = true;
  for (int i = 0; i < ER_MAX_BUFS; ++i) {
    a.gbufs.p[i] = i < n_bufs ? grad_bufs[i] : nullptr;
    if (i < n_bufs) {
      ER_REQUIRE(grad_bufs[i] != nullptr, "null gradient buffer");
      aligned = aligned && (reinterpret_cast<uintptr_t>(grad_bufs[i]) % 16 == 0);
    }
  }
  a.seg_scale = seg_scale;
  a.opt = *opt;
  a.lr_t = (opt->kind == ER_OPT_LAZY_ADAM || opt->kind == ER_OPT_ADAM_ROWS) ? adam_lr_t(*opt) : opt->lr;
  a.hyper = opt->hyper_dev;
  a.uniq_rows = uniq_rows;
  a.uniq_grads = uniq_grads;
  a.head_rank = nullptr;
  a.counters = w.counters;
  a.long_list = w.long_list;
  a.run_done = w.run_done;
  a.chunk_list = w.chunk_list;
  a.partials = w.partials;
  a.or_rows = rows;
  a.or_partials = w.one_row_partials;
  a.or_tickets = w.tickets;
  a.or_chunks = one_row ? (int)ceil_div(ceil_div(n_lookups_cap, (int64_t)n_slots), (int64_t)bk::kOneRowChunk) : 0;
  if (uniq_rows) {
    scan::exclusive_scan(HeadIn{w.keys, a.sentinel}, HeadOut{w.head_rank}, n_lookups_cap, n_uniq,
                         w.scan_ws, st);
    a.head_rank = w.head_rank;
    count_launches(3);
  }
  if (table) {
    aligned = aligned && reinterpret_cast<uintptr_t>(table) % 16 == 0 && row_stride % 4 == 0 &&
              (!state0 || reinterpret_cast<uintptr_t>(state0) % 16 == 0) &&
              (!state1 || reinterpret_cast<uintptr_t>(state1) % 16 == 0);
  }
  if (uniq_grads) aligned = aligned && reinterpret_cast<uintptr_t>(uniq_grads) % 16 == 0;
  const bool vec_dim = (dim == 4 || dim == 8 || dim == 16 || dim == 32 || dim == 64 || dim == 128);
  if (bucketed) {
    ER_REQUIRE(table != nullptr, "the bucketed path updates a table");
    a.keys = nullptr;
    a.vals = nullptr;
    a.pairs = src.bk.pairs;
    if (vec_dim && aligned) {
      switch (dim / 4) {
        case 1: bk_launch_fused<1>(a, src, place_warp, st); break;
        case 2: bk_launch_fused<2>(a, src, place_warp, st); break;
        case 4: bk_launch_fused<4>(a, src, place_warp, st); break;
        case 8: bk_launch_fused<8>(a, src, place_warp, st); break;
        case 16: bk_launch_fused<16>(a, src, place_warp, st); break;
        default: bk_launch_fused<32>(a, src, place_warp, st); break;
      }
    } else {
      bk_launch_fused<0>(a, src, place_warp, st);
    }
    ER_CUDA_LAUNCH_CHECK();
    return ER_OK;
  }
  if (vec_dim && aligned) {
    switch (dim / 4) {
      case 1: launch_radix<1>(a, st); break;
      case 2: launch_radix<2>(a, st); break;
      case 4: launch_radix<4>(a, st); break;
      case 8: launch_radix<8>(a, st); break;
      case 16: launch_radix<16>(a, st); break;
      default: launch_radix<32>(a, st); break;
    }
  } else {
    launch_radix<0>(a, st);
  }
  ER_CUDA_LAUNCH_CHECK();
  return ER_OK;
}

extern "C" int er_embedding_bwd(float* table, float* state0, float* state1, int64_t n_rows,
                                int32_t dim, int32_t row_stride, const int64_t* rows,
                                const float* weights, const int32_t* seg_ids,
                                const int32_t* row_ptr, int64_t n_seg, int64_t n_lookups_cap,
                                const er_slot_t* slots, int32_t n_slots,
                                const float* const* grad_bufs, int32_t n_bufs,
                                const float* seg_scale, const er_opt_t* opt, int64_t* uniq_rows,
                                float* uniq_grads, int32_t* n_uniq, void* ws, size_t ws_bytes,
                                er_stream_t stream) {
  return embedding_bwd_impl(table, state0, state1, n_rows, dim, row_stride, rows, weights, seg_ids, row_ptr,
                            n_seg, n_lookups_cap, slots, n_slots, grad_bufs, n_bufs, seg_scale, opt,
                            uniq_rows, uniq_grads, n_uniq, ws, ws_bytes, nullptr, 0, 0, stream);
}

extern "C" int er_embedding_bwd_presort(const int64_t* rows, int64_t n_rows, const int32_t* seg_ids,
                                        const int32_t* row_ptr, int64_t n_seg, int64_t n_lookups_cap,
                                        const er_slot_t* slots, int32_t n_slots, int32_t dim, void* ws,
                                        size_t ws_bytes, er_stream_t stream) {
  using namespace er;
  ER_REQUIRE(rows && slots, "null argument");
  ER_REQUIRE(n_rows > 0 && n_rows < 0xFFFFFFFFLL, "n_rows must be in (0, 2^32-1)");
  ER_REQUIRE(n_slots > 0 && n_slots <= 2048, "n_slots must be in [1, 2048]");
  ER_REQUIRE(n_lookups_cap >= 0 && n_lookups_cap < (1LL << 31) && dim > 0, "bad shape");
  if (n_lookups_cap == 0) return ER_OK;
  if (!ws || ws_bytes < bwd_ws_bytes(n_lookups_cap, dim))
    return fail(ER_ERR_WORKSPACE, "er_embedding_bwd_presort: workspace too small");
  BwdWs w = bwd_carve(ws, n_lookups_cap, dim);
  const int32_t* n_dev = row_ptr ? row_ptr + n_seg : nullptr;
  bk_place(rows, n_lookups_cap, n_dev, n_rows, seg_ids, slots, n_slots, seg_ids == nullptr, k7_warp_mode(dim), w, false,
           as_stream(stream));
  ER_CUDA_LAUNCH_CHECK();
  return ER_OK;
}

extern "C" int er_embedding_bwd_reuse_sort(float* table, float* state0, float* state1, int64_t n_rows,
                                           int32_t dim, int32_t row_stride, const int64_t* rows,
                                           const float* weights, const int32_t* seg_ids,
                                           const int32_t* row_ptr, int64_t n_seg, int64_t n_lookups_cap,
                                           const er_slot_t* slots, int32_t n_slots,
                                           const float* const* grad_bufs, int32_t n_bufs,
                                           const float* seg_scale, const er_opt_t* opt, int64_t* uniq_rows,
                                           float* uniq_grads, int32_t* n_uniq, void* ws, size_t ws_bytes,
                                           const void* sorted_ws, size_t sorted_ws_bytes,
                                           int32_t sorted_dim, er_stream_t stream) {
  if (!sorted_ws) return er::fail(ER_ERR_INVALID_ARG, "er_embedding_bwd_reuse_sort: sorted_ws is NULL");
  if (!rows) return er::fail(ER_ERR_INVALID_ARG, "er_embedding_bwd_reuse_sort: rows is NULL");
  return embedding_bwd_impl(table, state0, state1, n_rows, dim, row_stride, rows, weights, seg_ids,
                            row_ptr, n_seg, n_lookups_cap, slots, n_slots, grad_bufs, n_bufs, seg_scale,
                            opt, uniq_rows, uniq_grads, n_uniq, ws, ws_bytes, sorted_ws, sorted_ws_bytes,
                            sorted_dim, stream);
}

namespace er {

__global__ void __launch_bounds__(256)
    sparse_apply_kernel(const __grid_constant__ BwdArgs a, const int64_t* __restrict__ uniq_rows,
                        const float* __restrict__ uniq_grads, const int32_t* __restrict__ n_uniq,
                        int64_t n_cap) {
  const int64_t n = n_uniq ? (int64_t)(*n_uniq < n_cap ? *n_uniq : n_cap) : n_cap;
  const Hyper h = load_hyper(a.opt, a.lr_t, a.hyper);
  for (int64_t t = (int64_t)blockIdx.x * blockDim.x + threadIdx.x; t < n * a.dim;
       t += (int64_t)gridDim.x * blockDim.x) {
    const int64_t u = t / a.dim;
    const int c = (int)(t - u * a.dim);
    const int64_t row = uniq_rows[u];
    if (row < 0) continue;
    const int64_t off = row * a.row_stride + c;
    float g = __fmul_rn(uniq_grads[u * a.dim + c], h.grad_scale);
    float w = a.table[off];
    float s0 = a.state0 ? a.state0[off] : 0.f;
    float s1 = a.state1 ? a.state1[off] : 0.f;
    upd_one(a, h, g, w, s0, s1);
    a.table[off] = w;
    if (a.state0) a.state0[off] = s0;
    if (a.state1) a.state1[off] = s1;
  }
}

struct SweepArgs {
  float* table;
  float* m;
  float* v;
  int64_t n_rows;
  int dim;
  int row_stride;
  const uint8_t* touched;
  er_opt_t opt;
  float lr_t;
  const float* hyper;
};

__device__ __forceinline__ void sweep_one(float& w, float& m, float& v, float b1, float b2, float eps, float lr_t) {
  m = __fmul_rn(m, b1);
  v = __fmul_rn(v, b2);
  w = __fsub_rn(w, __fdiv_rn(__fmul_rn(lr_t, m), __fadd_rn(__fsqrt_rn(v), eps)));
}

__global__ void __launch_bounds__(256) adam_sweep_vec_kernel(const __grid_constant__ SweepArgs a) {
  const Hyper h = load_hyper(a.opt, a.lr_t, a.hyper);
  const int d4 = a.dim >> 2;
  const int64_t total = a.n_rows * d4;
  for (int64_t t = (int64_t)blockIdx.x * blockDim.x + threadIdx.x; t < total;
       t += (int64_t)gridDim.x * blockDim.x) {
    const int64_t r = t / d4;
    const int c = (int)(t - r * d4);
    if (a.touched && a.touched[r]) continue;
    const int64_t off = r * a.row_stride;
    float4* pm = reinterpret_cast<float4*>(a.m + off) + c;
    float4* pv = reinterpret_cast<float4*>(a.v + off) + c;
    float4 m = *pm, v = *pv;
    if (m.x == 0.f && m.y == 0.f && m.z == 0.f && m.w == 0.f && v.x == 0.f && v.y == 0.f && v.z == 0.f &&
        v.w == 0.f)
      continue;
    float4* pw = reinterpret_cast<float4*>(a.table + off) + c;
    float4 w = *pw;
    sweep_one(w.x, m.x, v.x, a.opt.beta1, a.opt.beta2, a.opt.eps, h.lr_t);
    sweep_one(w.y, m.y, v.y, a.opt.beta1, a.opt.beta2, a.opt.eps, h.lr_t);
    sweep_one(w.z, m.z, v.z, a.opt.beta1, a.opt.beta2, a.opt.eps, h.lr_t);
    sweep_one(w.w, m.w, v.w, a.opt.beta1, a.opt.beta2, a.opt.eps, h.lr_t);
    *pm = m;
    *pv = v;
    *pw = w;
  }
}

__global__ void __launch_bounds__(256) adam_sweep_kernel(const __grid_constant__ SweepArgs a) {
  const Hyper h = load_hyper(a.opt, a.lr_t, a.hyper);
  const int64_t total = a.n_rows * a.dim;
  for (int64_t t = (int64_t)blockIdx.x * blockDim.x + threadIdx.x; t < total;
       t += (int64_t)gridDim.x * blockDim.x) {
    const int64_t r = t / a.dim;
    const int c = (int)(t - r * a.dim);
    if (a.touched && a.touched[r]) continue;
    const int64_t off = r * a.row_stride + c;
    float m = a.m[off], v = a.v[off];
    if (m == 0.f && v == 0.f) continue;
    float w = a.table[off];
    sweep_one(w, m, v, a.opt.beta1, a.opt.beta2, a.opt.eps, h.lr_t);
    a.m[off] = m;
    a.v[off] = v;
    a.table[off] = w;
  }
}

}

extern "C" int er_sparse_apply(float* table, float* state0, float* state1, int32_t dim,
                               int32_t row_stride, const int64_t* uniq_rows,
                               const float* uniq_grads, const int32_t* n_uniq, int64_t n_cap,
                               const er_opt_t* opt, er_stream_t stream) {
  using namespace er;
  ER_REQUIRE(table && uniq_rows && uniq_grads && opt, "null argument");
  ER_REQUIRE(dim > 0 && row_stride >= dim, "bad dim / row_stride");
  const int k = opt->kind;
  ER_REQUIRE(k == ER_OPT_SGD || state0, "optimizer state0 missing");
  ER_REQUIRE((k != ER_OPT_LAZY_ADAM && k != ER_OPT_ADAM_ROWS) || state1, "adam needs state1 (v)");
  if (n_cap <= 0) return ER_OK;
  BwdArgs a = {};
  a.table = table;
  a.state0 = state0;
  a.state1 = state1;
  a.dim = dim;
  a.row_stride = row_stride;
  a.opt = *opt;
  a.lr_t = (k == ER_OPT_LAZY_ADAM || k == ER_OPT_ADAM_ROWS) ? adam_lr_t(*opt) : opt->lr;
  a.hyper = opt->hyper_dev;
  sparse_apply_kernel<<<grid_for(n_cap * dim, 256, 8), 256, 0, as_stream(stream)>>>(
      a, uniq_rows, uniq_grads, n_uniq, n_cap);
  count_launches(1);
  ER_CUDA_LAUNCH_CHECK();
  return ER_OK;
}

extern "C" int er_adam_dense_sweep(float* table, float* m, float* v, int64_t n_rows, int32_t dim,
                                   int32_t row_stride, const uint8_t* touched,
                                   const er_opt_t* opt, er_stream_t stream) {
  using namespace er;
  ER_REQUIRE(table && m && v && opt, "null argument");
  ER_REQUIRE(dim > 0 && row_stride >= dim && n_rows > 0, "bad shape");
  SweepArgs a;
  a.table = table;
  a.m = m;
  a.v = v;
  a.n_rows = n_rows;
  a.dim = dim;
  a.row_stride = row_stride;
  a.touched = touched;
  a.opt = *opt;
  a.opt.kind = ER_OPT_ADAM_ROWS;
  a.lr_t = adam_lr_t(*opt);
  a.hyper = opt->hyper_dev;
  const bool vec = dim % 4 == 0 && row_stride % 4 == 0 && reinterpret_cast<uintptr_t>(table) % 16 == 0 &&
                   reinterpret_cast<uintptr_t>(m) % 16 == 0 && reinterpret_cast<uintptr_t>(v) % 16 == 0;
  if (vec)
    adam_sweep_vec_kernel<<<grid_for(n_rows * (dim / 4), 256, 8), 256, 0, as_stream(stream)>>>(a);
  else
    adam_sweep_kernel<<<grid_for(n_rows * dim, 256, 8), 256, 0, as_stream(stream)>>>(a);
  count_launches(1);
  ER_CUDA_LAUNCH_CHECK();
  return ER_OK;
}
```

easyrec_b200/embedding.py:

```python
import math
import os

import numpy as np
import torch

from easyrec_b200 import _lib
from easyrec_b200 import kernels as K


class Slot(object):

  def __init__(self, name, table, bucket_mode, num_buckets, combiner=_lib.COMBINER_SUM,
               out_buf=0, n_seg_per_sample=1):
    self.name = name
    self.table = table
    self.bucket_mode = bucket_mode
    self.num_buckets = int(num_buckets)
    self.combiner = combiner
    self.out_buf = out_buf
    self.n_seg_per_sample = n_seg_per_sample
    self.unit_weights = False


class Arena(object):

  def __init__(self, dim, device, shard_n=1, shard_rank=0):
    self.dim = dim
    self.device = device
    self.shard_n = shard_n
    self.shard_rank = shard_rank
    self.tables = {}
    self.n_rows = 0
    self.weight = None
    self.state0 = None
    self.state1 = None

  def add_table(self, name, n_rows_global):
    if name in self.tables:
      assert self.tables[name][2] == n_rows_global, 'shared table %s: size mismatch' % name
      return
    local = (n_rows_global + self.shard_n - 1) // self.shard_n
    self.tables[name] = (self.n_rows, local, n_rows_global)
    self.n_rows += local

  def materialize(self, opt_kind, init_fn=None, adagrad_init=0.1, generator=None, interleave=True):
    assert self.n_rows > 0
    n_state = {_lib.OPT_SGD: 0, _lib.OPT_ADAGRAD: 1, _lib.OPT_MOMENTUM: 1}.get(opt_kind, 2)
    k = (1 + n_state) if interleave else 1
    self.storage = torch.empty(self.n_rows, k * self.dim, dtype=torch.float32, device=self.device)
    w = self.storage[:, :self.dim]
    plan_only = os.environ.get('ER_PLAN_ONLY') == '1'
    if plan_only:
      init_fn = lambda t: None
    if init_fn is not None:
      init_fn(w)
    else:
      std = 0.01 / math.sqrt(self.dim)
      tmp = torch.empty(self.n_rows, self.dim, dtype=torch.float32, device=self.device)
      torch.nn.init.trunc_normal_(tmp, mean=0.0, std=std, a=-2 * std, b=2 * std,
                                  generator=generator)
      w.copy_(tmp)
      del tmp
    self.weight = w
    self.opt_kind = opt_kind

    def state(i, fill):
      if interleave:
        v = self.storage[:, (1 + i) * self.dim:(2 + i) * self.dim]
        if not plan_only:
          v.fill_(fill)
        return v
      return torch.full((self.n_rows, self.dim), fill, dtype=torch.float32, device=self.device)

    self.state0 = self.state1 = None
    if opt_kind == _lib.OPT_ADAGRAD:
      self.state0 = state(0, adagrad_init)
    elif opt_kind == _lib.OPT_MOMENTUM:
      self.state0 = state(0, 0.0)
    elif opt_kind in (_lib.OPT_LAZY_ADAM, _lib.OPT_ADAM_ROWS):
      self.state0 = state(0, 0.0)
      self.state1 = state(1, 0.0)
    self.touched = (torch.zeros(self.n_rows, dtype=torch.uint8, device=self.device)
                    if opt_kind == _lib.OPT_ADAM_ROWS else None)

  def table_view(self, name):
    off, n, _ = self.tables[name]
    return self.weight[off:off + n]


class ArenaCall(object):

  def __init__(self, arena, slots, batch_size, out_widths, single_valued, max_lookups=None):
    self.arena = arena
    self.slots = slots
    self.batch_size = batch_size
    dim = arena.dim
    recs = []
    seg = 0
    cols = [0] * len(out_widths)
    self.out_strides = [((w + 3) // 4) * 4 if dim % 4 == 0 else w for w in out_widths]
    self.out_widths = out_widths
    self.slot_cols = []
    for s in slots:
      off, _, _ = arena.tables[s.table]
      n_seg = batch_size * s.n_seg_per_sample
      col = cols[s.out_buf]
      cols[s.out_buf] += dim
      stride = self.out_strides[s.out_buf]
      self.slot_cols.append(col)
      recs.append(dict(num_buckets=s.num_buckets, row_offset=off, seg_begin=seg, n_seg=n_seg,
                       bucket_mode=s.bucket_mode,
                       combiner=s.combiner | (_lib.COMBINER_UNIT_WEIGHTS if s.unit_weights else 0), out_buf=s.out_buf,
                       out_stride=stride, out_col=col, shard_n=arena.shard_n))
      seg += n_seg
    self.n_seg = seg
    self.slots_np = K.make_slots(recs, dim)
    self.slots_dev = K.slots_to_device(self.slots_np, arena.device)
    self.n_slots = len(recs)
    self.single_valued = single_valued
    self.max_lookups = self.n_seg if single_valued else int(max_lookups)
    self.needs_scale = any((s.combiner & 0xf) != _lib.COMBINER_SUM for s in slots)
    self.ws = K.bwd_workspace(self.max_lookups, arena.device, arena.dim)
    self.seg_scale = (torch.empty(self.n_seg, dtype=torch.float32, device=arena.device)
                      if self.needs_scale else None)

  def out_rows(self, buf):
    for s in self.slots:
      if s.out_buf == buf:
        return self.batch_size * s.n_seg_per_sample
    raise KeyError(buf)

  def alloc_outputs(self):
    return [torch.empty(self.out_rows(i), st, dtype=torch.float32, device=self.arena.device)
            for i, st in enumerate(self.out_strides)]


def fused_lookup(call, rows, weights=None, row_ptr=None, outs=None):
  a = call.arena
  if outs is None:
    outs = call.alloc_outputs()
  K.embedding_fwd(a.weight, a.dim, rows, call.slots_dev, call.n_slots, call.n_seg, outs,
                  weights=weights, row_ptr=row_ptr, seg_scale=call.seg_scale)
  for o in outs:
    o.requires_grad_(True)
  return outs


def adam_dense_decay(arena, rows, opt, n_dev=None):
  if arena.opt_kind != _lib.OPT_ADAM_ROWS:
    return
  if rows is not None and rows.numel():
    K.mark_rows(rows, arena.n_rows, arena.touched, 1, n_dev=n_dev)
  K.adam_dense_sweep(arena.weight, arena.state0, arena.state1, arena.dim, arena.touched, opt)
  if rows is not None and rows.numel():
    K.mark_rows(rows, arena.n_rows, arena.touched, 0, n_dev=n_dev)


def fused_backward_update(call, rows, outs, opt, weights=None, row_ptr=None, seg_ids=None, sorted_from=None):
  a = call.arena
  gbufs = []
  for i, o in enumerate(outs):
    g = o.grad
    if g is None:
      g = torch.zeros_like(o)
    gbufs.append(g.contiguous())
  K.embedding_bwd(a.weight, a.state0, a.state1, a.dim, rows, call.slots_dev, call.n_slots,
                  call.n_seg, gbufs, opt, call.ws, weights=weights, seg_ids=seg_ids,
                  row_ptr=row_ptr, seg_scale=call.seg_scale, sorted_from=sorted_from)
  adam_dense_decay(a, rows, opt, n_dev=None if row_ptr is None else row_ptr[call.n_seg:])


class Placements(object):

  def __init__(self):
    self.clear()

  def presort(self, rows, n_rows, dim, ws, slots_dev, n_slots, seg_ids=None):
    if self.sorted_from(rows, n_rows, dim, ws) is None:
      K.embedding_bwd_presort(rows, n_rows, dim, ws, slots_dev, n_slots, seg_ids=seg_ids)
      self.presorted = True

  def sorted_from(self, rows, n_rows, dim, ws):
    key = (id(rows), int(n_rows), K.k7_warp_mode(dim))
    hit = self._placed.get(key)
    if hit is None:
      self._placed[key] = (ws, dim)
    return hit

  def clear(self):
    self._placed = {}
    self.presorted = False


class _FM(torch.autograd.Function):

  @staticmethod
  def forward(ctx, x, n_field, dim):
    ctx.n_field, ctx.dim = n_field, dim
    ctx.save_for_backward(x)
    return K.fm_fwd(x, n_field, dim)

  @staticmethod
  def backward(ctx, gy):
    (x,) = ctx.saved_tensors
    gx = torch.empty(x.shape[0], x.shape[1], dtype=torch.float32, device=x.device)
    if x.shape[1] > ctx.n_field * ctx.dim:
      gx.zero_()
    K.fm_bwd(x, gy.contiguous(), ctx.n_field, ctx.dim, gx=gx)
    return gx, None, None


def fm(x, n_field, dim):
  return _FM.apply(x, n_field, dim)


class _FMBlock(torch.autograd.Function):

  @staticmethod
  def forward(ctx, x, n_field, dim):
    ctx.n_field, ctx.dim = n_field, dim
    y, sumsq = K.fm_block_fwd(x, n_field, dim, want_sumsq=True)
    ctx.save_for_backward(x)
    return y, x.view_as(x), sumsq

  @staticmethod
  def backward(ctx, gy, g_pass, g_sumsq):
    (x,) = ctx.saved_tensors
    gx = K.fm_block_bwd(x, None if gy is None else gy.contiguous(), g_pass,
                        None if g_sumsq is None else g_sumsq.contiguous(), 2.0, ctx.n_field, ctx.dim)
    return gx, None, None


def fm_block(x, n_field, dim):
  return _FMBlock.apply(x, n_field, dim)


class _RowsumBlock(torch.autograd.Function):

  @staticmethod
  def forward(ctx, x):
    y, sumsq = K.rowsum_block_fwd(x, want_sumsq=True)
    ctx.save_for_backward(x)
    return y.unsqueeze(1), sumsq

  @staticmethod
  def backward(ctx, gy, g_sumsq):
    (x,) = ctx.saved_tensors
    gx = K.rowsum_block_bwd(x, None if gy is None else gy.contiguous().view(-1),
                            None if g_sumsq is None else g_sumsq.contiguous(), 2.0)
    return gx


def rowsum_block(x):
  return _RowsumBlock.apply(x)


class _ConcatCols(torch.autograd.Function):

  @staticmethod
  def forward(ctx, *mats):
    ctx.widths = [m.shape[1] for m in mats]
    return K.concat_cols(list(mats))

  @staticmethod
  def backward(ctx, g):
    return tuple(K.split_cols(g, ctx.widths))


def concat_cols(mats):
  if len(mats) > 8 or not mats[0].is_cuda:
    return torch.cat(mats, dim=1)
  return _ConcatCols.apply(*mats)


class _SigmoidCE(torch.autograd.Function):

  @staticmethod
  def forward(ctx, logits, labels, weights, inv_count):
    loss, probs, g = K.sigmoid_ce(logits.contiguous(), labels, weights, inv_count)
    ctx.save_for_backward(g)
    ctx.mark_non_differentiable(probs)
    return loss[0], probs

  @staticmethod
  def backward(ctx, gl, _gp):
    (g,) = ctx.saved_tensors
    return g * gl, None, None, None


def sigmoid_cross_entropy(logits, labels, weights=None, inv_count=None):
  if inv_count is None:
    inv_count = 1.0 / logits.numel()
  return _SigmoidCE.apply(logits, labels, weights, inv_count)
```

easyrec_b200/input_layer.py:

```python
import collections
import os

import numpy as np
import torch

from easyrec_b200 import _lib
from easyrec_b200 import embedding as E
from easyrec_b200 import kernels as K

FeatureSpec = collections.namedtuple(
    'FeatureSpec',
    ['name', 'kind',
     'embedding_dim', 'bucket_mode', 'num_buckets', 'combiner', 'embedding_name',
     'min_val', 'max_val', 'raw_input_dim', 'seq_len'])


def _bucket_rule(hash_bucket_size, num_buckets, packed_mod, host_hashed=False):
  if hash_bucket_size > 0:
    if host_hashed:
      return _lib.BUCKET_IDENTITY, hash_bucket_size
    return _lib.BUCKET_FARM_DECIMAL, hash_bucket_size
  if packed_mod:
    return _lib.BUCKET_MOD, num_buckets
  return _lib.BUCKET_IDENTITY, num_buckets


def id_feature(name, embedding_dim, hash_bucket_size=0, num_buckets=0, combiner='sum',
               embedding_name='', packed_mod=False, host_hashed=False):
  mode, nb = _bucket_rule(hash_bucket_size, num_buckets, packed_mod, host_hashed)
  return FeatureSpec(name, 'id', embedding_dim, mode, nb, combiner, embedding_name, 0., 0., 1, 1)


def raw_feature(name, embedding_dim=0, min_val=0.0, max_val=0.0, raw_input_dim=1):
  mode = _lib.BUCKET_ONE_ROW if raw_input_dim == 1 else _lib.BUCKET_NONE
  return FeatureSpec(name, 'raw', embedding_dim, mode, raw_input_dim, 'sum', '',
                     float(min_val), float(max_val), raw_input_dim, 1)


def multi_feature(name, kind, embedding_dim, hash_bucket_size=0, num_buckets=0, combiner='sum',
                  embedding_name='', seq_len=1, packed_mod=False, host_hashed=False):
  assert kind in ('tag', 'seq')
  mode, nb = _bucket_rule(hash_bucket_size, num_buckets, packed_mod, host_hashed)
  return FeatureSpec(name, kind, embedding_dim, mode, nb, combiner, embedding_name, 0., 0., 1,
                     max(int(seq_len), 1))


_COMBINER = {'sum': _lib.COMBINER_SUM, 'mean': _lib.COMBINER_MEAN, 'sqrtn': _lib.COMBINER_SQRTN}

GroupColumn = collections.namedtuple('GroupColumn', ['name', 'kind', 'width', 'dim', 'out_key', 'col', 'need_key', 'slot'],
                                     defaults=(None,) * 5)
SeqColumn = collections.namedtuple('SeqColumn', ['name', 'dim', 'out_key', 'col', 'slot'], defaults=(None, None))
Pending = collections.namedtuple('Pending', ['call', 'rows', 'weights', 'outs', 'seg_ids'])


class _SubCall(object):

  def __init__(self, kind, n_seg_per_slot):
    self.kind = kind
    self.n_seg_per_slot = n_seg_per_slot
    self.items = []
    self.call = None


class MergedCall(object):

  def __init__(self, arena, subcalls):
    self.arena = arena
    recs = []
    self.buf_of = []
    seg = 0
    lookups = 0
    self.sub_lookup_off = []
    self.sub_seg_off = []
    for si, sc in enumerate(subcalls):
      c = sc.call
      base_buf = len(self.buf_of)
      for b in range(len(c.out_strides)):
        self.buf_of.append((si, b))
      self.sub_seg_off.append(seg)
      self.sub_lookup_off.append(lookups)
      for r in c.slots_np:
        recs.append(dict(num_buckets=int(r['num_buckets']), row_offset=int(r['row_offset']),
                         seg_begin=int(r['seg_begin']) + seg, n_seg=int(r['n_seg']),
                         bucket_mode=int(r['bucket_mode']), combiner=int(r['combiner']),
                         out_buf=int(r['out_buf']) + base_buf, out_stride=int(r['out_stride']),
                         out_col=int(r['out_col']), shard_n=int(r['shard_n'])))
      seg += c.n_seg
      lookups += c.max_lookups
    assert len(self.buf_of) <= _lib.MAX_BUFS, 'too many output matrices on one arena'
    self.slots_np = K.make_slots(recs, arena.dim)
    self.slots_dev = K.slots_to_device(self.slots_np, arena.device)
    self.n_slots = len(recs)
    self.n_seg = seg
    self.max_lookups = lookups
    self.out_strides = [subcalls[si].call.out_strides[b] for si, b in self.buf_of]
    self._out_rows = [subcalls[si].call.out_rows(b) for si, b in self.buf_of]
    self.ws = K.bwd_workspace(lookups, arena.device, arena.dim)
    self.has_csr = any(sc.kind in ('tag', 'mseq') for sc in subcalls)
    self.single_valued = not self.has_csr
    self.needs_scale = any(sc.call.needs_scale for sc in subcalls)
    dev = arena.device
    self.rows = torch.empty(lookups, dtype=torch.int64, device=dev) if len(subcalls) > 1 else None
    self.weights = None
    self.seg_ids = torch.empty(lookups, dtype=torch.int32, device=dev) if self.has_csr else None
    if len(subcalls) == 1:
      self.seg_scale = subcalls[0].call.seg_scale
    else:
      self.seg_scale = torch.ones(seg, dtype=torch.float32, device=dev) if self.needs_scale else None

  def out_rows(self, buf):
    return self._out_rows[buf]


class InputLayer(object):

  def __init__(self, features, groups, batch_size, device, wide_output_dim=1,
               embedding_optimizer=_lib.OPT_ADAGRAD, shard_n=1, shard_rank=0, generator=None,
               adagrad_init=0.1, seq_att_groups=None, max_tag_lookups=None, uniform_tables=None,
               dense_generator=None, multi_valued_seq=(), seq_combiners=None, seq_output_groups=()):
    self.features = collections.OrderedDict((f.name, f) for f in features)
    self.seq_output_groups = set(seq_output_groups)
    self.multi_valued_seq = set(multi_valued_seq)
    self.seq_combiners = dict(seq_combiners or {})
    self.groups = groups
    self.seq_att_groups = seq_att_groups or collections.OrderedDict()
    self.batch_size = batch_size
    self.device = device
    self.wide_output_dim = wide_output_dim
    self.sparse_names = [f.name for f in features if f.kind == 'id']
    self.raw_names = [f.name for f in features if f.kind == 'raw']
    self.raw_cols = {}
    c = 0
    for n in self.raw_names:
      self.raw_cols[n] = (c, c + self.features[n].raw_input_dim)
      c += self.features[n].raw_input_dim
    self.n_dense = c
    self.arenas = collections.OrderedDict()
    self.subcalls = collections.OrderedDict()
    self.group_layout = {}
    self.seq_layout = {}
    self.seq_group_layout = {}
    self.attention_modules = collections.OrderedDict()
    self.seqc_order = {}
    self._shard = (shard_n, shard_rank)
    for gname, g in groups.items():
      self._plan_group(gname, g, dense_generator)
    for sname, maps in self.seq_att_groups.items():
      self._plan_seq_layout(sname, sname, maps)
    for gname, g in groups.items():
      for sub in g.get('seq') or []:
        self._plan_sequence_features(gname, g, sub, dense_generator)
    self._materialize(embedding_optimizer, generator, adagrad_init, uniform_tables)
    self._plan_calls(max_tag_lookups)
# ... 114 lines not shown
        if mine is not None:
          if mine.out_key != scope:
            raise NotImplementedError('sequence_features key %s is a multi-valued feature of group %s' % (k, scope))
          key.append(SeqColumn(k, mine.dim, mine.out_key, slot=mine.slot))
          continue
        table = f.embedding_name or '%s/%s_embedding' % (scope, k)
        slot = self._add_slot(f.embedding_dim, sname + '/key', k, table, 'single')
        key.append(SeqColumn(k, f.embedding_dim, sname + '/key', slot=slot))
      for h in hists:
        f = self.features[h]
        assert f.kind == 'seq', '%s must be a SequenceFeature' % h
        assert T in (None, f.seq_len), 'hist_seq features of one group must share seq_len'
        T = f.seq_len
        table = f.embedding_name or '%s/%s_embedding' % (scope, h)
        slot = self._add_slot(f.embedding_dim, sname + '/hist', h, table, 'seq')
        hist.append(SeqColumn(h, f.embedding_dim, sname + '/hist', slot=slot))
    self.seq_layout[sname] = lay = dict(key=key, hist=hist, T=T)
    return lay

  def _plan_sequence_features(self, gname, g, sub, dense_generator):
    if g.get('wide'):
      raise NotImplementedError('sequence_features in the wide group %s' % gname)
    from easyrec_b200 import layers as L
    sname = '%s/%s' % (gname, sub['name'])
    lay = self._plan_seq_layout(sname, gname, sub['maps'], own=self.group_layout[gname])
    dk, dh = sum(e.dim for e in lay['key']), sum(e.dim for e in lay['hist'])
    if dk != dh:
      raise NotImplementedError('sequence_features %s: key width %d != history width %d (allow_key_transform)'
                                % (sname, dk, dh))
    need_key = bool(sub.get('need_key', True))
    self.group_layout[gname].append(GroupColumn('seq_fea/' + sub['name'], 'att', dh + (dk if need_key else 0),
                                                out_key=sname, need_key=need_key))
    self.attention_modules[sname] = L.DNN(4 * dh, sub['units'], last_layer_no_activation=True,
                                          last_layer_no_batch_norm=True, generator=dense_generator)

  def _materialize(self, embedding_optimizer, generator, adagrad_init, uniform_tables):
    for subs in self.subcalls.values():
      uses = collections.Counter(slot.table for sc in subs.values() for _, _, slot, _ in sc.items)
      for sc in subs.values():
        for _, _, slot, _ in sc.items:
          if slot.bucket_mode == _lib.BUCKET_ONE_ROW and (uses[slot.table] > 1 or sc.kind != 'single'):
            slot.bucket_mode = _lib.BUCKET_NONE
    for a in self.arenas.values():
      a.materialize(embedding_optimizer, generator=generator, adagrad_init=adagrad_init)
      for tname, limit in (uniform_tables or {}).items():
        if tname in a.tables and os.environ.get('ER_PLAN_ONLY') != '1':
          off, local, _ = a.tables[tname]
          rows = torch.empty(local, a.dim, dtype=torch.float32, device=self.device)
          rows.uniform_(-limit, limit, generator=generator)
          a.weight[off:off + local].copy_(rows)

  def _plan_calls(self, max_tag_lookups):
    B, device = self.batch_size, self.device
    self.calls = collections.OrderedDict()
    self.merged = collections.OrderedDict()
    self._gather_plan = {}
    self.static_ids = {}
    self.static_w = {}
    self.out_index = {}
    for dim, subs in self.subcalls.items():
      for sk, sc in subs.items():
        keys = list(dict.fromkeys(out_key for out_key, _, _, _ in sc.items))
        widths = [0] * len(keys)
        slots = []
        for out_key, _, slot, _ in sc.items:
          slot.out_buf = keys.index(out_key)
          widths[slot.out_buf] += dim
          slots.append(slot)
        if sc.kind == 'tag':
          cap = max_tag_lookups or 8 * B * len(slots)
          sc.call = E.ArenaCall(self.arenas[dim], slots, B, widths, single_valued=False, max_lookups=cap)
        elif sc.kind == 'mseq':
          cap = max_tag_lookups or 4 * B * sk[1] * len(slots)
          sc.call = E.ArenaCall(self.arenas[dim], slots, B, widths, single_valued=False, max_lookups=cap)
        else:
          sc.call = E.ArenaCall(self.arenas[dim], slots, B, widths, single_valued=True)
        for j, k in enumerate(keys):
          self.out_index[(dim, k)] = (sk, j)
        if sc.kind == 'single':
          self.calls[dim] = sc.call
          src = [s for _, _, _, s in sc.items]
          self.static_ids[dim] = torch.zeros(sc.call.n_seg, dtype=torch.int64, device=device)
          has_raw = any(k == 'raw' for k, _ in src)
          self.static_w[dim] = (torch.ones(sc.call.n_seg, dtype=torch.float32, device=device)
                                if has_raw else None)
          sc.call.identity_ids = ([k for k, _ in src] == ['id'] * len(src) and
                                  [i for _, i in src] == list(range(len(self.sparse_names))))
          sc.call.sources = src
      self.merged[dim] = MergedCall(self.arenas[dim], list(subs.values()))
    cols = {id(slot): c for subs in self.subcalls.values() for sc in subs.values()
            for slot, c in zip(sc.call.slots, sc.call.slot_cols)}

    def resolved(columns):
      return [e if e.slot is None else e._replace(col=cols[id(e.slot)]) for e in columns]
    self.group_layout = {g: resolved(lay) for g, lay in self.group_layout.items()}
    self.seq_layout = {s: dict(lay, key=resolved(lay['key']), hist=resolved(lay['hist']))
                       for s, lay in self.seq_layout.items()}
    self.seq_group_layout = {g: dict(lay, seq=resolved(lay['seq'])) for g, lay in self.seq_group_layout.items()}

  def _plan_exchanges(self):
    from easyrec_b200.sharded import ShardedLookup
    shard_n, shard_rank = self._shard
    exchanges = {}
    for dim, subs in self.subcalls.items():
      for sk, sc in subs.items():
        if sc.kind != 'single':
          mine = set(slot.table for _, _, slot, _ in sc.items)
          for sk2, sc2 in subs.items():
            shared = sorted(mine & set(slot.table for _, _, slot, _ in sc2.items)) if sc2 is not sc else None
            if shared and 'seq' in (sc.kind, sc2.kind):
              raise NotImplementedError('EmbeddingParallel: table(s) %s are read both by history (SequenceFeature) '
                                        'steps and by other features; give the histories tables of their own'
                                        % shared)
            if shared:
              raise NotImplementedError('EmbeddingParallel: table(s) %s are shared by single- and multi-valued features'
                                        % shared)
          if sc.kind == 'seq' and len(subs) > 1 and self.arenas[dim].opt_kind == _lib.OPT_ADAM_ROWS:
            raise NotImplementedError('EmbeddingParallel: adam_optimizer with histories next to other features of '
                                      'embedding_dim %d (their tables share one arena and two exchanges)' % dim)
          seq = (self.batch_size, sk[1]) if sc.kind == 'seq' else None
          sc.sharded = ShardedLookup(sc.call, shard_n, shard_rank, seq=seq)
          if len(subs) == 1:
            self.merged[dim].sharded = sc.sharded
          continue
        key = self._rows_key(sc)
        sc.sharded = ShardedLookup(sc.call, shard_n, shard_rank, exchange=exchanges.get(key))
        exchanges.setdefault(key, sc.sharded.ex)
        self.merged[dim].sharded = sc.sharded

  def group_width(self, name):
    return sum(e.width for e in self.group_layout[name])

  def discard_pending(self):
    self._pending = []

  def set_optimizer_step(self, lr, step, beta1=0.9, beta2=0.999, eps=1e-8, grad_scale=1.0):
    kind = next(iter(self.arenas.values())).opt_kind
    h = self.hyper
    if np.float32(beta1) != h.beta1 or np.float32(beta2) != h.beta2:
      h.beta1, h.beta2, h._pow_step = np.float32(beta1), np.float32(beta2), None
    h.set(lr, step, grad_scale * self.emb_grad_mult * self.replica_grad_scale)
    self.opt_holder['opt'] = h.opt(kind, eps)

  def backward_update(self):
    if self.ep:
      for m, rows, w, outs, seg_ids in self._pending:
        m.sharded.backward_update(outs, self.opt_holder['opt'])
      self._pending = []
      return
    if self.placements.presorted:
      torch.cuda.current_stream().wait_stream(self._side)
    cur = torch.cuda.current_stream() if str(self.device).startswith('cuda') else None
    forked = False
    for idx, (m, rows, w, outs, seg_ids) in enumerate(self._pending):
      src = self.placements.sorted_from(rows, m.arena.n_rows, m.arena.dim, m.ws)
      if idx > 0 and src is not None and self._side is not None and cur is not None:
        if not forked:
          self._side.wait_stream(cur)
          forked = True
        with torch.cuda.stream(self._side):
          E.fused_backward_update(m, rows, outs, self.opt_holder['opt'], weights=w, seg_ids=seg_ids, sorted_from=src)
      else:
        E.fused_backward_update(m, rows, outs, self.opt_holder['opt'], weights=w, seg_ids=seg_ids, sorted_from=src)
    if forked:
      cur.wait_stream(self._side)
    self._pending = []

  def ep_hold_updates(self, on=True):
    for ex in self._exchanges():
      ex.hold = bool(on)

  def ep_recv_sqnorm(self):
    total = torch.zeros((), dtype=torch.float32, device=self.device)
    for ex in self._exchanges():
      total = total + (ex.recv_g * ex.recv_g).sum()
    return total * float(self.emb_grad_mult) ** 2

  def ep_apply_held(self):
    for ex in self._exchanges():
      if ex.members:
        ex.members[0].apply_held()

  def check_exchange(self):
    if self.ep:
      for subs in self.subcalls.values():
        for sc in subs.values():
          sc.sharded.check()

  def sparse_grad_sqnorm(self):
    total = torch.zeros((), dtype=torch.float32, device=self.device)
    for m, rows, w, outs, seg_ids in self._pending:
      if seg_ids is None and rows.numel() != m.n_seg:
        raise NotImplementedError('gradient_clipping_by_norm: a call whose lookups are not its segments needs seg_ids')
      a = m.arena
      n_l = rows.numel()
      st = self._clip_state.get(id(m))
      if st is None:
        if a.n_rows * m.n_slots >= 0xFFFFFFFF:
          raise NotImplementedError('gradient_clipping_by_norm: %d rows x %d columns exceed the 32-bit row key' %
                                    (a.n_rows, m.n_slots))
        off = torch.zeros(m.n_seg, dtype=torch.int64)
        for j, r in enumerate(m.slots_np):
          off[int(r['seg_begin']):int(r['seg_begin']) + int(r['n_seg'])] = j * a.n_rows
        st = dict(off=off.to(self.device), ws=K.bwd_workspace(n_l, self.device, a.dim),
                  ur=torch.empty(n_l, dtype=torch.int64, device=self.device),
                  ug=torch.empty(n_l, a.dim, dtype=torch.float32, device=self.device),
                  nu=torch.zeros(1, dtype=torch.int32, device=self.device),
                  idx=torch.arange(n_l, device=self.device, dtype=torch.int32))
        self._clip_state[id(m)] = st
      off = st['off'] if seg_ids is None else st['off'][seg_ids[:n_l].clamp(0, m.n_seg - 1).long()]
      vr = torch.where(rows < 0, rows, rows + off)
      gbufs = [(o.grad if o.grad is not None else torch.zeros_like(o)).contiguous() for o in outs]
      opt = K.make_opt(_lib.OPT_SGD, 0.0, grad_scale=float(self.emb_grad_mult))
      K.embedding_bwd(None, None, None, a.dim, vr, m.slots_dev, m.n_slots, m.n_seg, gbufs, opt, st['ws'], weights=w,
                      seg_ids=seg_ids, seg_scale=m.seg_scale, uniq_rows=st['ur'], uniq_grads=st['ug'], n_uniq=st['nu'],
                      n_rows=a.n_rows * m.n_slots)
      rowsq = (st['ug'] * st['ug']).sum(dim=1)
      total = total + torch.where(st['idx'] < st['nu'], rowsq, torch.zeros_like(rowsq)).sum()
    return total

  def _rows_buf(self, key, call):
    buf = self._rows_bufs.get(key)
    if buf is None:
      buf = torch.empty(call.n_seg, dtype=torch.int64, device=self.device)
      self._rows_bufs[key] = buf
    return buf

  def precompute_rows(self, features):
    dense = features.get('dense_fea')
    dense_norm = self.normalize_dense(dense) if dense is not None else None
    out = []
    self._preset_rows = {}
    for dim, subs in self.subcalls.items():
      for sk, sc in subs.items():
        if sc.kind != 'single' or len(subs) != 1:
          continue
        call = sc.call
        key = self._rows_key(sc)
        hit = self._preset_rows.get(key)
        if hit is None:
          cids, w = self._gather_inputs(dim, features.get('sparse_fea'), dense_norm)
          rows = K.bucketize(cids, call.slots_dev, call.n_slots, call.n_seg, rows=self._rows_buf(key, call))
          hit = (rows, w)
          self._preset_rows[key] = hit
        out.append((dim, self.merged[dim], hit[0], hit[1]))
    return out

  def _presort(self):
    self.placements.clear()
    if not (self._pending and self.presort_enabled and not self.ep and torch.is_grad_enabled() and
            str(self.device).startswith('cuda')):
      return
    if self._side is None:
      self._side = torch.cuda.Stream(device=self.device)
    self._side.wait_stream(torch.cuda.current_stream())
    with torch.cuda.stream(self._side):
      for m, rows, w, outs, seg_ids in self._pending:
        self.placements.presort(rows, m.arena.n_rows, m.arena.dim, m.ws, m.slots_dev, m.n_slots, seg_ids=seg_ids)

  def normalize_dense(self, dense):
    if self.raw_has_range:
      dense = (dense - self.raw_sub) / self.raw_range
    if self.raw_normalizers:
      dense = dense.clone() if not self.raw_has_range else dense
      for name, fn in self.raw_normalizers.items():
        c0, c1 = self.raw_cols[name]
        dense[:, c0:c1] = fn(dense[:, c0:c1])
    return dense

  def prefetch_exchange(self, next_features):
    if not self.ep:
      return
    done = set()
    for dim, subs in self.subcalls.items():
      for sk, sc in subs.items():
        if sc.kind != 'single':
          continue
        ex = sc.sharded.ex
        if id(ex) in done:
          continue
        done.add(id(ex))
        buf = self._next_ids.get(dim)
        if buf is None:
          buf = self._next_ids[dim] = torch.zeros_like(self.static_ids[dim])
        cids, _ = self._gather_inputs(dim, next_features.get('sparse_fea'), None, ids_buf=buf, want_w=False)
        ex.prefetch(ex.members[0], cids)

  def _exchanges(self):
    seen, out = set(), []
    if self.ep:
      for subs in self.subcalls.values():
        for sc in subs.values():
          if id(sc.sharded.ex) not in seen:
            seen.add(id(sc.sharded.ex))
            out.append(sc.sharded.ex)
    return out

  def join_prefetch(self):
    for ex in self._exchanges():
      ex.join_prefetch()

  def drop_prefetch(self):
    for ex in self._exchanges():
      ex._have_next = False

  def prefetch_ready(self):
    ex = self._exchanges()
    return bool(ex) and all(e._have_next for e in ex)

  def _gather_inputs(self, dim, ids, dense_norm, ids_buf=None, want_w=True):
    call = self.calls[dim]
    if call.identity_ids:
      return ids, None
    B = self.batch_size
    S = call.n_slots
    out_ids = self.static_ids[dim] if ids_buf is None else ids_buf
    out_w = self.static_w[dim] if want_w else None
    plan = self._gather_plan.get(dim)
    if plan is None:
# ... 289 lines not shown
```

easyrec_b200/kernels.py:

```python
import ctypes

import numpy as np
import torch

from easyrec_b200 import _lib
from easyrec_b200._lib import ErOpt, SLOT_DTYPE, c_vp


def _stream():
  return torch.cuda.current_stream().cuda_stream


def _p(t):
  return None if t is None else t.data_ptr()


def _chk(t, dtype, name):
  if t is None:
    return
  if not t.is_cuda:
    raise _lib.ErError('%s must be a CUDA tensor (no CPU fallback)' % name)
  if t.dtype != dtype:
    raise _lib.ErError('%s must be %s, got %s' % (name, dtype, t.dtype))
  if not t.is_contiguous():
# ... 131 lines not shown
  _lib.check(_lib.load().er_act_bwd(_p(x), _p(gy), x.numel(), int(kind), _p(gx), _stream()), 'er_act_bwd')
  return gx


def dice_fwd(x, xn, alpha):
  for t, nm in ((x, 'x'), (xn, 'xn'), (alpha, 'alpha')):
    _chk(t, torch.float32, nm)
  y = torch.empty_like(x)
  _lib.check(_lib.load().er_dice_fwd(_p(x), _p(xn), _p(alpha), x.shape[0], x.shape[1], _p(y), _stream()), 'er_dice_fwd')
  return y


def dice_bwd(x, xn, alpha, gy):
  gy = gy.contiguous()
  for t, nm in ((x, 'x'), (xn, 'xn'), (alpha, 'alpha'), (gy, 'gy')):
    _chk(t, torch.float32, nm)
  gd, gn, ga = torch.empty_like(x), torch.empty_like(x), torch.empty_like(x)
  _lib.check(_lib.load().er_dice_bwd(_p(x), _p(xn), _p(alpha), _p(gy), x.shape[0], x.shape[1], _p(gd), _p(gn), _p(ga),
                                     _stream()), 'er_dice_bwd')
  return gd, gn, ga


def auc_hist(probs, labels, thresholds, hist):
  probs, labels = probs.contiguous().view(-1), labels.contiguous().view(-1)
  _chk(probs, torch.float32, 'probs')
  _chk(labels, torch.float32, 'labels')
  _chk(thresholds, torch.float32, 'thresholds')
  _chk(hist, torch.int64, 'hist')
  assert probs.numel() == labels.numel() and hist.numel() == 2 * (thresholds.numel() + 1)
  _lib.check(_lib.load().er_auc_hist(_p(probs), _p(labels), probs.numel(), _p(thresholds), thresholds.numel(), _p(hist),
                                     _stream()), 'er_auc_hist')
  return hist


def shard_group_workspace(n_lookups, device):
  return torch.empty(_lib.load().er_shard_group_workspace_bytes(int(n_lookups)), dtype=torch.uint8, device=device)


def shard_group(rows, owner, world, cap_per_peer, send_rows, pos, counts, ws):
  _chk(rows, torch.int64, 'rows')
  _chk(owner, torch.int32, 'owner')
  _chk(send_rows, torch.int64, 'send_rows')
  _chk(pos, torch.int64, 'pos')
  _chk(counts, torch.int32, 'counts')
  assert send_rows.numel() == world * cap_per_peer and pos.numel() == rows.numel() and counts.numel() == world + 1
  _lib.check(_lib.load().er_shard_group(_p(rows), _p(owner), rows.numel(), int(world), int(cap_per_peer), _p(send_rows),
                                        _p(pos), _p(counts), _p(ws), ws.numel(), _stream()), 'er_shard_group')


def embedding_fwd(table, dim, rows, slots_dev, n_slots, n_seg, out_bufs, weights=None,
                  row_ptr=None, seg_scale=None, row_stride=None):
  lib = _lib.load()
  n_rows, row_stride = _chk_rows(table, 'table')
  _chk(rows, torch.int64, 'rows')
  _chk(weights, torch.float32, 'weights')
  _chk(row_ptr, torch.int32, 'row_ptr')
  _chk(seg_scale, torch.float32, 'seg_scale')
  for i, b in enumerate(out_bufs):
    _chk(b, torch.float32, 'out_bufs[%d]' % i)
  _lib.check(
      lib.er_embedding_fwd(_p(table), n_rows, dim, row_stride, _p(rows), _p(weights), _p(row_ptr),
                           n_seg, rows.numel(), _p(slots_dev), n_slots, _buf_array(out_bufs),
                           len(out_bufs), _p(seg_scale), _stream()), 'er_embedding_fwd')


def bwd_workspace(n_lookups_cap, device, dim):
  lib = _lib.load()
  return torch.empty(lib.er_embedding_bwd_workspace_bytes(n_lookups_cap, dim), dtype=torch.uint8,
                     device=device)


def make_opt(kind, lr, beta1=0.9, beta2=0.999, eps=1e-8, beta1_power=0.9, beta2_power=0.999,
             grad_scale=1.0, hyper_dev=None):
  return ErOpt(kind, lr, beta1, beta2, eps, beta1_power, beta2_power, grad_scale, _p(hyper_dev))


class StepHyper(object):

  def __init__(self, device, beta1=0.9, beta2=0.999):
    self.device = device
    self.beta1, self.beta2 = np.float32(beta1), np.float32(beta2)
    self.dev = torch.zeros(_lib.HYPER_N, dtype=torch.float32, device=device)
    self._pow_step = None
    self.b1p = self.b2p = None
    self.lr = 0.0
    self.grad_scale = 1.0

  def _powers(self, step):
    if self._pow_step is not None and step == self._pow_step + 1:
      self.b1p = np.float32(self.b1p * self.beta1)
      self.b2p = np.float32(self.b2p * self.beta2)
    elif self._pow_step is None or step != self._pow_step:
      b1p, b2p = self.beta1, self.beta2
      for _ in range(int(step)):
        b1p = np.float32(b1p * self.beta1)
        b2p = np.float32(b2p * self.beta2)
      self.b1p, self.b2p = b1p, b2p
    self._pow_step = step

  def set(self, lr, step, grad_scale=1.0):
    self._powers(step)
    self.lr, self.grad_scale = float(np.float32(lr)), float(np.float32(grad_scale))
    h = [0.0] * _lib.HYPER_N
    h[_lib.HYPER_LR] = self.lr
    h[_lib.HYPER_BETA1_POWER] = float(self.b1p)
    h[_lib.HYPER_BETA2_POWER] = float(self.b2p)
    h[_lib.HYPER_GRAD_SCALE] = self.grad_scale
    self.dev.copy_(torch.tensor(h, dtype=torch.float32), non_blocking=True)

  def opt(self, kind, eps=1e-8, grad_scale=None):
    return make_opt(kind, self.lr, float(self.beta1), float(self.beta2), eps, float(self.b1p), float(self.b2p),
                    self.grad_scale if grad_scale is None else grad_scale, hyper_dev=self.dev)


def embedding_bwd(table, state0, state1, dim, rows, slots_dev, n_slots, n_seg, grad_bufs, opt,
                  ws, weights=None, seg_ids=None, row_ptr=None, seg_scale=None, row_stride=None,
                  uniq_rows=None, uniq_grads=None, n_uniq=None, n_rows=None, sorted_from=None):
  lib = _lib.load()
  row_stride = dim
  if table is not None:
    n_rows_t, row_stride = _chk_rows(table, 'table')
    n_rows = n_rows if n_rows is not None else n_rows_t
    for st, nm in ((state0, 'state0'), (state1, 'state1')):
      if st is not None and _chk_rows(st, nm)[1] != row_stride:
        raise _lib.ErError('%s must share the table row stride' % nm)
  _chk(rows, torch.int64, 'rows')
  _chk(weights, torch.float32, 'weights')
  _chk(seg_ids, torch.int32, 'seg_ids')
  _chk(row_ptr, torch.int32, 'row_ptr')
  _chk(seg_scale, torch.float32, 'seg_scale')
  _chk(uniq_rows, torch.int64, 'uniq_rows')
  _chk(uniq_grads, torch.float32, 'uniq_grads')
  _chk(n_uniq, torch.int32, 'n_uniq')
  for i, b in enumerate(grad_bufs):
    _chk(b, torch.float32, 'grad_bufs[%d]' % i)
  if sorted_from is not None:
    src_ws, src_dim = sorted_from
    _lib.check(
        lib.er_embedding_bwd_reuse_sort(_p(table), _p(state0), _p(state1), n_rows, dim, row_stride, _p(rows),
                                        _p(weights), _p(seg_ids), _p(row_ptr), n_seg, rows.numel(),
                                        _p(slots_dev), n_slots, _buf_array(grad_bufs), len(grad_bufs),
                                        _p(seg_scale), ctypes.byref(opt), _p(uniq_rows), _p(uniq_grads),
                                        _p(n_uniq), _p(ws), ws.numel(), _p(src_ws), src_ws.numel(), src_dim,
                                        _stream()), 'er_embedding_bwd_reuse_sort')
    return
  _lib.check(
      lib.er_embedding_bwd(_p(table), _p(state0), _p(state1), n_rows, dim, row_stride, _p(rows),
                           _p(weights), _p(seg_ids), _p(row_ptr), n_seg, rows.numel(),
                           _p(slots_dev), n_slots, _buf_array(grad_bufs), len(grad_bufs),
                           _p(seg_scale), ctypes.byref(opt), _p(uniq_rows), _p(uniq_grads),
                           _p(n_uniq), _p(ws), ws.numel(), _stream()), 'er_embedding_bwd')


def k7_warp_mode(dim):
  return dim in (1, 4, 8, 16, 32)


def embedding_bwd_presort(rows, n_rows, dim, ws, slots_dev, n_slots, seg_ids=None, row_ptr=None, n_seg=0):
  lib = _lib.load()
  _chk(rows, torch.int64, 'rows')
  _chk(seg_ids, torch.int32, 'seg_ids')
  _lib.check(lib.er_embedding_bwd_presort(_p(rows), n_rows, _p(seg_ids), _p(row_ptr), n_seg, rows.numel(),
                                          _p(slots_dev), n_slots, dim, _p(ws), ws.numel(), _stream()),
             'er_embedding_bwd_presort')


def sparse_apply(table, state0, state1, dim, uniq_rows, uniq_grads, n_uniq, opt, row_stride=None):
  lib = _lib.load()
  _, row_stride = _chk_rows(table, 'table')
  _lib.check(
      lib.er_sparse_apply(_p(table), _p(state0), _p(state1), dim, row_stride, _p(uniq_rows),
                          _p(uniq_grads), _p(n_uniq), uniq_rows.numel(), ctypes.byref(opt),
                          _stream()), 'er_sparse_apply')


def adam_dense_sweep(table, m, v, dim, touched, opt, row_stride=None):
  lib = _lib.load()
  n_rows_t, row_stride = _chk_rows(table, 'table')
  _lib.check(
      lib.er_adam_dense_sweep(_p(table), _p(m), _p(v), n_rows_t, dim,
                              row_stride, _p(touched), ctypes.byref(opt), _stream()),
      'er_adam_dense_sweep')


def mark_rows(rows, n_rows, touched, value, n_dev=None):
  lib = _lib.load()
  _lib.check(
      lib.er_mark_rows(_p(rows), rows.numel(), _p(n_dev), n_rows, _p(touched), value, _stream()),
      'er_mark_rows')


def sort_rows(rows, max_row, n_dev=None):
  lib = _lib.load()
  _chk(rows, torch.int64, 'rows')
  n = rows.numel()
  keys = torch.empty(n, dtype=torch.int32, device=rows.device)
  vals = torch.empty(n, dtype=torch.int32, device=rows.device)
  ws_bytes = lib.er_sort_workspace_bytes(n)
  ws = torch.empty(ws_bytes, dtype=torch.uint8, device=rows.device)
  _lib.check(
      lib.er_sort_rows(_p(rows), n, _p(n_dev), max_row, _p(keys), _p(vals), _p(ws), ws_bytes,
                       _stream()), 'er_sort_rows')
  return keys, vals


def fm_fwd(x, n_field, dim, y=None):
  lib = _lib.load()
  _chk(x, torch.float32, 'x')
  batch = x.shape[0]
  if y is None:
    y = torch.empty(batch, dim, dtype=torch.float32, device=x.device)
  _lib.check(lib.er_fm_fwd(_p(x), batch, n_field, dim, x.stride(0), _p(y), _stream()), 'er_fm_fwd')
  return y


def fm_bwd(x, gy, n_field, dim, gx=None, accumulate=False):
  lib = _lib.load()
  _chk(x, torch.float32, 'x')
  _chk(gy, torch.float32, 'gy')
  batch = x.shape[0]
  if gx is None:
    gx = torch.empty(batch, n_field * dim, dtype=torch.float32, device=x.device)
    accumulate = False
  _lib.check(
      lib.er_fm_bwd(_p(x), _p(gy), batch, n_field, dim, x.stride(0), _p(gx), gx.stride(0),
                    1 if accumulate else 0, _stream()), 'er_fm_bwd')
  return gx


def fm_block_ok(n_field, dim):
  d4 = dim // 4
  return dim % 4 == 0 and 1 <= d4 <= 32 and (d4 & (d4 - 1)) == 0 and n_field * d4 <= 256


_fm_ws = {}


def fm_block_fwd(x, n_field, dim, want_sumsq=True):
  lib = _lib.load()
  if x.dtype != torch.float32 or x.stride(1) != 1:
    raise _lib.ErError('x must be float32 with unit column stride')
  batch = x.shape[0]
  y = torch.empty(batch, dim, dtype=torch.float32, device=x.device)
  sumsq = ws = None
  if want_sumsq:
    sumsq = torch.empty(1, dtype=torch.float32, device=x.device)
    ws = _fm_ws.get(x.device)
    if ws is None:
      ws = torch.zeros(lib.er_fm_block_workspace_bytes(batch), dtype=torch.uint8, device=x.device)
      _fm_ws[x.device] = ws
  _lib.check(lib.er_fm_block_fwd(_p(x), batch, n_field, dim, x.stride(0), _p(y), _p(sumsq), _p(ws),
                                 0 if ws is None else ws.numel(), _stream()), 'er_fm_block_fwd')
  return y, sumsq


def fm_block_bwd(x, gy, g_pass, coef_dev, coef_mul, n_field, dim):
  lib = _lib.load()
  batch = x.shape[0]
  gx = torch.empty(batch, n_field * dim, dtype=torch.float32, device=x.device)
  if g_pass is not None and g_pass.stride(1) != 1:
    g_pass = g_pass.contiguous()
  _lib.check(lib.er_fm_block_bwd(_p(x), _p(gy), _p(g_pass), _p(coef_dev), coef_mul, batch, n_field, dim,
                                 x.stride(0), 0 if g_pass is None else g_pass.stride(0), _p(gx), gx.stride(0),
                                 _stream()), 'er_fm_block_bwd')
  return gx


_blk_ws = {}


def _zero_ws(key, nbytes, device):
  ws = _blk_ws.get((key, device))
  if ws is None or ws.numel() < nbytes:
    ws = torch.zeros(nbytes, dtype=torch.uint8, device=device)
    _blk_ws[(key, device)] = ws
  return ws


def rowsum_block_fwd(x, want_sumsq=True):
  lib = _lib.load()
  batch, width = x.shape
  y = torch.empty(batch, dtype=torch.float32, device=x.device)
  sumsq = ws = None
  if want_sumsq:
    sumsq = torch.empty(1, dtype=torch.float32, device=x.device)
    ws = _zero_ws('rowsum', lib.er_fm_block_workspace_bytes(batch), x.device)
  _lib.check(lib.er_rowsum_block_fwd(_p(x), batch, width, x.stride(0), _p(y), _p(sumsq), _p(ws),
                                     0 if ws is None else ws.numel(), _stream()), 'er_rowsum_block_fwd')
  return y, sumsq


def rowsum_block_bwd(x, gy, coef_dev, coef_mul):
  lib = _lib.load()
  batch, width = x.shape
  gx = torch.empty(batch, width, dtype=torch.float32, device=x.device)
  _lib.check(lib.er_rowsum_block_bwd(_p(x), _p(gy), _p(coef_dev), coef_mul, batch, width, x.stride(0), _p(gx),
                                     gx.stride(0), _stream()), 'er_rowsum_block_bwd')
  return gx


def dense1_fwd(x, w, bias):
  lib = _lib.load()
  batch, width = x.shape
  y = torch.empty(batch, 1, dtype=torch.float32, device=x.device)
  _lib.check(lib.er_dense1_fwd(_p(x), _p(w), _p(bias), batch, width, x.stride(0), _p(y), _stream()), 'er_dense1_fwd')
  return y
# ... 210 lines not shown
```

include/er_b200.h:

```cpp
#ifndef ER_B200_H_
#define ER_B200_H_

#include <stddef.h>
#include <stdint.h>

#ifdef __cplusplus
extern "C" {
#endif

#define ER_B200_ABI_VERSION 3

typedef void* er_stream_t;

typedef enum er_status {
  ER_OK = 0,
  ER_ERR_INVALID_ARG = 1,
  ER_ERR_WORKSPACE = 2,
  ER_ERR_CUDA = 3,
  ER_ERR_UNSUPPORTED = 4
} er_status;

typedef enum er_bucket_mode {
  ER_BUCKET_FARM_DECIMAL = 0,
  ER_BUCKET_MOD = 1,
  ER_BUCKET_IDENTITY = 2,
  ER_BUCKET_NONE = 3,
  ER_BUCKET_ONE_ROW = 4
} er_bucket_mode;

typedef enum er_combiner {
  ER_COMBINER_SUM = 0,
  ER_COMBINER_MEAN = 1,
  ER_COMBINER_SQRTN = 2,
  ER_COMBINER_UNIT_WEIGHTS = 16
} er_combiner;

typedef struct er_slot {
  int64_t num_buckets;
  int64_t row_offset;
  int32_t seg_begin;
  int32_t n_seg;
  int32_t bucket_mode;
  int32_t combiner;
  int32_t out_buf;
  int32_t out_stride;
  int32_t out_col;
  int32_t shard_n;
} er_slot_t;

#define ER_MAX_BUFS 8

typedef enum er_opt_kind {
  ER_OPT_SGD = 0,
  ER_OPT_ADAGRAD = 1,
  ER_OPT_LAZY_ADAM = 2,
  ER_OPT_ADAM_ROWS = 3,
  ER_OPT_MOMENTUM = 4
} er_opt_kind;

enum {
  ER_HYPER_LR = 0,
  ER_HYPER_BETA1_POWER = 1,
  ER_HYPER_BETA2_POWER = 2,
  ER_HYPER_GRAD_SCALE = 3,
  ER_HYPER_N = 4
};

typedef struct er_opt {
  int32_t kind;
  float lr;
  float beta1;
  float beta2;
  float eps;
  float beta1_power;
  float beta2_power;
  float grad_scale;
  const float* hyper_dev;
} er_opt_t;

int er_abi_version(void);
const char* er_last_error(void);
uint64_t er_launch_count(void);

size_t er_csr_workspace_bytes(int64_t n_seg);
int er_csr_from_lens(const int32_t* lens, int64_t n_seg, int32_t* row_ptr,
                     int32_t* seg_ids, int64_t n_lookups_cap, void* ws,
                     size_t ws_bytes, er_stream_t stream);

int er_bucketize(const int64_t* ids, const int32_t* seg_ids,
                 const int32_t* row_ptr, int64_t n_seg, int64_t n_lookups_cap,
                 const er_slot_t* slots, int32_t n_slots, int64_t* rows,
                 int32_t* owner, er_stream_t stream);
int er_bucketize_weighted(const int64_t* ids, const float* weights, const int32_t* seg_ids,
                          const int32_t* row_ptr, int64_t n_seg, int64_t n_lookups_cap,
                          const er_slot_t* slots, int32_t n_slots, int64_t* rows,
                          int32_t* owner, er_stream_t stream);

int er_bucketize_seq(const int64_t* ids, const int32_t* lens, int64_t batch,
                     int32_t seq_len, int32_t n_features, const er_slot_t* slots,
                     int32_t n_slots, int64_t* rows, int32_t* owner,
                     er_stream_t stream);

size_t er_shard_group_workspace_bytes(int64_t n_lookups);
int er_shard_group(const int64_t* rows, const int32_t* owner, int64_t n_lookups,
                   int32_t world, int64_t cap_per_peer, int64_t* send_rows,
                   int64_t* pos, int32_t* counts, void* ws, size_t ws_bytes,
                   er_stream_t stream);

uint64_t er_fingerprint64_host(const char* s, size_t len);

int er_embedding_fwd(const float* table, int64_t n_rows, int32_t dim,
                     int32_t row_stride, const int64_t* rows,
                     const float* weights, const int32_t* row_ptr,
                     int64_t n_seg, int64_t n_lookups_cap,
                     const er_slot_t* slots, int32_t n_slots,
                     float* const* out_bufs, int32_t n_bufs, float* seg_scale,
                     er_stream_t stream);

size_t er_embedding_bwd_workspace_bytes(int64_t n_lookups_cap, int32_t dim);
int er_embedding_bwd(float* table, float* state0, float* state1,
                     int64_t n_rows, int32_t dim, int32_t row_stride,
                     const int64_t* rows, const float* weights,
                     const int32_t* seg_ids, const int32_t* row_ptr,
                     int64_t n_seg, int64_t n_lookups_cap,
                     const er_slot_t* slots, int32_t n_slots,
                     const float* const* grad_bufs, int32_t n_bufs,
                     const float* seg_scale, const er_opt_t* opt,
                     int64_t* uniq_rows, float* uniq_grads, int32_t* n_uniq,
                     void* ws, size_t ws_bytes, er_stream_t stream);

int er_embedding_bwd_presort(const int64_t* rows, int64_t n_rows, const int32_t* seg_ids,
                             const int32_t* row_ptr, int64_t n_seg, int64_t n_lookups_cap,
                             const er_slot_t* slots, int32_t n_slots, int32_t dim, void* ws,
                             size_t ws_bytes, er_stream_t stream);

int er_embedding_bwd_reuse_sort(float* table, float* state0, float* state1, int64_t n_rows,
                                int32_t dim, int32_t row_stride, const int64_t* rows,
                                const float* weights, const int32_t* seg_ids,
                                const int32_t* row_ptr, int64_t n_seg, int64_t n_lookups_cap,
                                const er_slot_t* slots, int32_t n_slots,
                                const float* const* grad_bufs, int32_t n_bufs,
                                const float* seg_scale, const er_opt_t* opt, int64_t* uniq_rows,
                                float* uniq_grads, int32_t* n_uniq, void* ws, size_t ws_bytes,
                                const void* sorted_ws, size_t sorted_ws_bytes, int32_t sorted_dim,
                                er_stream_t stream);

int er_sparse_apply(float* table, float* state0, float* state1, int32_t dim,
                    int32_t row_stride, const int64_t* uniq_rows,
                    const float* uniq_grads, const int32_t* n_uniq,
                    int64_t n_cap, const er_opt_t* opt, er_stream_t stream);

int er_adam_dense_sweep(float* table, float* m, float* v, int64_t n_rows,
                        int32_t dim, int32_t row_stride,
                        const uint8_t* touched, const er_opt_t* opt,
                        er_stream_t stream);

int er_mark_rows(const int64_t* rows, int64_t n_lookups_cap, const int32_t* n_dev,
                 int64_t n_rows, uint8_t* touched, int32_t value,
                 er_stream_t stream);

size_t er_sort_workspace_bytes(int64_t n);
int er_sort_rows(const int64_t* rows, int64_t n, const int32_t* n_dev,
                 int64_t max_row, uint32_t* keys_out, uint32_t* vals_out,
                 void* ws, size_t ws_bytes, er_stream_t stream);

int er_fm_fwd(const float* x, int64_t batch, int32_t n_field, int32_t dim,
              int32_t x_stride, float* y, er_stream_t stream);
int er_fm_bwd(const float* x, const float* gy, int64_t batch, int32_t n_field,
              int32_t dim, int32_t x_stride, float* gx, int32_t gx_stride,
              int32_t accumulate, er_stream_t stream);

size_t er_fm_block_workspace_bytes(int64_t batch);
int er_fm_block_fwd(const float* x, int64_t batch, int32_t n_field, int32_t dim, int32_t x_stride,
                    float* y, float* sumsq_out, void* ws, size_t ws_bytes, er_stream_t stream);
int er_fm_block_bwd(const float* x, const float* gy, const float* g_pass, const float* coef_dev,
                    float coef_mul, int64_t batch, int32_t n_field, int32_t dim, int32_t x_stride,
                    int32_t g_pass_stride, float* gx, int32_t gx_stride, er_stream_t stream);

#define ER_MAX_CAT 8
int er_concat_cols(const float* const* srcs, const int32_t* widths, const int32_t* strides, int32_t n,
                   int64_t batch, float* dst, int32_t dst_stride, er_stream_t stream);
int er_split_cols(const float* src, int32_t src_stride, int64_t batch, float* const* dsts,
                  const int32_t* widths, const int32_t* strides, int32_t n, er_stream_t stream);

int er_rowsum_block_fwd(const float* x, int64_t batch, int32_t width, int32_t x_stride, float* y,
                        float* sumsq_out, void* ws, size_t ws_bytes, er_stream_t stream);
int er_rowsum_block_bwd(const float* x, const float* gy, const float* coef_dev, float coef_mul,
                        int64_t batch, int32_t width, int32_t x_stride, float* gx, int32_t gx_stride,
                        er_stream_t stream);

size_t er_dense1_workspace_bytes(int32_t width);
int er_dense1_fwd(const float* x, const float* w, const float* bias, int64_t batch, int32_t width,
                  int32_t x_stride, float* y, er_stream_t stream);
int er_dense1_bwd(const float* x, const float* w, const float* g, int64_t batch, int32_t width,
                  int32_t x_stride, float* gx, int32_t gx_stride, float* gw, float* gb, void* ws,
                  size_t ws_bytes, er_stream_t stream);

size_t er_dense_workspace_bytes(int64_t batch, int32_t units);
int er_bias_bn_act_fwd(const float* z, const float* bias, const float* gamma,
                       const float* beta, float* moving_mean, float* moving_var,
                       int64_t batch, int32_t units, float eps, float momentum,
                       int32_t training, int32_t relu, float* y, float* save_mean,
                       float* save_rstd, void* ws, size_t ws_bytes,
                       er_stream_t stream);
int er_bias_bn_act_bwd(const float* z, const float* bias, const float* gamma,
                       const float* y, const float* gy, const float* save_mean,
                       const float* save_rstd, int64_t batch, int32_t units,
                       int32_t relu, float* gz, float* gbias, float* ggamma,
                       float* gbeta, void* ws, size_t ws_bytes, er_stream_t stream);

int er_dropout(const float* x, int64_t n, float rate, uint64_t seed, const int64_t* counter_dev, float* y,
               er_stream_t stream);

enum {
  ER_ACT_GELU = 1,
  ER_ACT_LEAKY_RELU = 2,
  ER_ACT_ELU = 3,
  ER_ACT_SELU = 4,
  ER_ACT_TANH = 5,
  ER_ACT_SWISH = 6,
  ER_ACT_SIGMOID = 7
};
int er_act_fwd(const float* x, int64_t n, int kind, float* y, er_stream_t stream);
int er_act_bwd(const float* x, const float* gy, int64_t n, int kind, float* gx, er_stream_t stream);

int er_dice_fwd(const float* x, const float* xn, const float* alpha, int64_t batch, int32_t units, float* y,
                er_stream_t stream);
int er_dice_bwd(const float* x, const float* xn, const float* alpha, const float* gy, int64_t batch, int32_t units,
                float* gx_direct, float* gxn, float* galpha_terms, er_stream_t stream);

int er_auc_hist(const float* probs, const float* labels, int64_t n, const float* thresholds, int32_t n_thresholds,
                uint64_t* hist, er_stream_t stream);

typedef struct er_dense_seg {
  int64_t offset;
  int64_t n;
  float l2;
  float lr_mult;
} er_dense_seg_t;
int er_dense_apply(float* params, const float* grads, float* state0, float* state1,
                   const er_dense_seg_t* segs, int32_t n_segs, int64_t max_seg_n,
                   const er_opt_t* opt, const float* lr_dev, float* reg_loss_out,
                   er_stream_t stream);

size_t er_gemm_workspace_bytes(int64_t M, int64_t N, int64_t K);
int er_gemm(const float* A, int64_t lda, int32_t a_mn_major, const float* B, int64_t ldb,
            int32_t b_mn_major, const float* bias, float* C, int64_t ldc, int64_t M, int64_t N,
            int64_t K, void* ws, size_t ws_bytes, er_stream_t stream);

size_t er_gemm_small_workspace_bytes(int64_t M, int64_t N, int64_t K);
int er_gemm_small(const float* A, int64_t sa_m, int64_t sa_k, const float* B, int64_t sb_k, int64_t sb_n,
                  const float* bias, float* C, int64_t ldc, int64_t M, int64_t N, int64_t K, void* ws, size_t ws_bytes,
                  er_stream_t stream);

typedef struct {
  const float* bias;
  float* save_mean;
  float* save_rstd;
  float* moving_mean;
  float* moving_var;
  float eps;
  float momentum;
} er_bn_stats_t;
size_t er_gemm_bn_workspace_bytes(int64_t M, int64_t N);
int er_gemm_bn(const float* A, int64_t lda, int32_t a_mn_major, const float* B, int64_t ldb,
               int32_t b_mn_major, float* C, int64_t ldc, int64_t M, int64_t N, int64_t K,
               const er_bn_stats_t* bn, void* ws, size_t ws_bytes, er_stream_t stream);
int er_bn_act_apply(const float* z, const float* bias, const float* gamma, const float* beta,
                    const float* mean, const float* rstd, int64_t batch, int32_t units, int32_t relu,
                    float* y, er_stream_t stream);

int er_sigmoid_ce_fwd_bwd(const float* logits, const float* labels,
                          const float* weights, int64_t batch, float inv_count,
                          float* loss_out, float* probs, float* g_logits,
                          er_stream_t stream);

int er_din_concat_fwd(const float* query, const float* keys, int64_t batch,
                      int32_t seq_len, int32_t dim, float* din_in, er_stream_t stream);
int er_din_concat_bwd(const float* query, const float* keys, const float* g_din_in,
                      int64_t batch, int32_t seq_len, int32_t dim, float* g_query,
                      float* g_keys, int32_t accumulate_gkeys, er_stream_t stream);
int er_din_pool_fwd(const float* scores, const float* keys, const int32_t* lens,
                    int64_t batch, int32_t seq_len, int32_t dim, float* probs,
                    float* out, er_stream_t stream);
int er_din_pool_bwd(const float* probs, const float* keys, const float* gout,
                    const int32_t* lens, int64_t batch, int32_t seq_len, int32_t dim,
                    float* g_scores, float* g_keys, int32_t accumulate_gkeys,
                    er_stream_t stream);
int er_din_sigmoid_pool_fwd(const float* scores, const float* keys, const int32_t* lens,
                            int64_t batch, int32_t seq_len, int32_t dim, float scale,
                            float* probs, float* out, er_stream_t stream);
int er_din_sigmoid_pool_bwd(const float* probs, const float* keys, const float* gout,
                            const int32_t* lens, int64_t batch, int32_t seq_len, int32_t dim,
                            float scale, float* g_scores, float* g_keys,
                            int32_t accumulate_gkeys, er_stream_t stream);

int er_cross_fwd(const float* x0, const float* xl, const float* w, const float* b,
                 int64_t batch, int32_t dim, float* out, float* xw_out,
// ... 71 lines not shown
```

Measured before the change: 9.940 million.

## Fuse dim-1 companion table backward into vector embedding backward kernels

Adds a paired backward path in which a dim-1 embedding table that shares its lookup rows with a vector table (dim 4-32) is updated inside the same sort/bucket/long-run kernels as the primary table. The companion reuses the primary's sorted keys, runs and chunk partials, so its own sort and launch sequence is no longer needed. The Python layer detects such pairs and dispatches the fused call. In exchange, shared memory grows, the kernels get extra scalar work and syncs, and big-bucket processing runs the companion pass serially before the primary.

```diff
diff --git a/easyrec_b200/_lib.py b/easyrec_b200/_lib.py
--- a/easyrec_b200/_lib.py
+++ b/easyrec_b200/_lib.py
@@ -89,6 +89,11 @@
         c_vp, c_vp, c_vp, c_i64, c_i32, c_i32, c_vp, c_vp, c_vp, c_vp, c_i64,
         c_i64, c_vp, c_i32, ctypes.POINTER(c_vp), c_i32, c_vp,
         ctypes.POINTER(ErOpt), c_vp, c_vp, c_vp, c_vp, c_sz, c_vp, c_sz, c_i32, c_vp
+    ]),
+    'er_embedding_bwd_pair': (c_i32, [
+        c_vp, c_vp, c_vp, c_i64, c_i32, c_i32, c_vp, c_vp, c_vp, c_vp, c_i64,
+        c_i64, c_vp, c_i32, ctypes.POINTER(c_vp), c_i32, c_vp, ctypes.POINTER(ErOpt), c_vp, c_sz,
+        c_vp, c_vp, c_vp, c_i32, c_vp, ctypes.POINTER(c_vp), c_i32, c_vp, c_vp, c_sz, c_vp, c_sz, c_i32, c_vp
     ]),
     'er_embedding_bwd': (c_i32, [
         c_vp, c_vp, c_vp, c_i64, c_i32, c_i32, c_vp, c_vp, c_vp, c_vp, c_i64,
diff --git a/easyrec_b200/csrc/embedding_bwd.cu b/easyrec_b200/csrc/embedding_bwd.cu
--- a/easyrec_b200/csrc/embedding_bwd.cu
+++ b/easyrec_b200/csrc/embedding_bwd.cu
@@ -5,6 +5,8 @@
 #include "bucket_bwd.cuh"
 
 namespace er {
+
+__host__ __device__ inline size_t slot_region(int n_slots) { return (slot_smem_bytes(n_slots) + 15) & ~(size_t)15; }
 
 struct CBufs {
   const float* p[ER_MAX_BUFS];
@@ -532,12 +534,17 @@
   return a.pairs ? (uint32_t)a.pairs[i] : a.vals[i];
 }
 
-template <int LANES, int TPE>
-__global__ void __launch_bounds__(256) bwd_long_vec_kernel(const __grid_constant__ BwdArgs a) {
-  extern __shared__ __align__(16) unsigned char s_raw[];
+template <int LANES, int TPE, bool PAIR = false>
+__global__ void __launch_bounds__(256) bwd_long_vec_kernel(const __grid_constant__ BwdArgs a,
+                                                           const __grid_constant__ BwdArgs cp) {
+  extern __shared__ __align__(16) unsigned char s_raw_all[];
+  unsigned char* s_raw = s_raw_all + (PAIR ? slot_region(cp.n_slots) : 0);
   const SlotView sv = load_slots(s_raw, a.slots, a.n_slots);
-  float4* s_part = reinterpret_cast<float4*>(s_raw + ((slot_smem_bytes(a.n_slots) + 15) & ~(size_t)15));
+  SlotView svc{};
+  if constexpr (PAIR) svc = load_slots(s_raw_all, cp.slots, cp.n_slots);
+  float4* s_part = reinterpret_cast<float4*>(s_raw + slot_region(a.n_slots));
   __shared__ int s_last;
+  __shared__ float s_w1[8];
   constexpr int CH = LANES / TPE;
   constexpr int G = 256 / TPE;
   const int lane32 = threadIdx.x & 31, warp = threadIdx.x >> 5;
@@ -592,10 +599,26 @@
     if (threadIdx.x < LANES) {
       for (int ww = 0; ww < 8; ++ww) f4_acc(tot, s_part[ww * LANES + threadIdx.x]);
     }
+    float ctot = 0.f;
+    if constexpr (PAIR) {
+      float g1 = 0.f;
+      for (int e = e0 + threadIdx.x; e < e1; e += 256) {
+        float coef;
+        const float* src = grad_src(cp, svc, val_at(a, i + e), &coef);
+        g1 = __fadd_rn(g1, __fmul_rn(src[0], coef));
+      }
+#pragma unroll
+      for (int o = 16; o >= 1; o >>= 1) g1 = __fadd_rn(g1, __shfl_xor_sync(0xffffffffu, g1, o));
+      if (lane32 == 0) s_w1[warp] = g1;
+      __syncthreads();
+      if (threadIdx.x == 0)
+        for (int ww = 0; ww < 8; ++ww) ctot = __fadd_rn(ctot, s_w1[ww]);
+    }
     bool finish = (nch == 1);
     if (nch > 1) {
       if (threadIdx.x < LANES)
         __stcg(reinterpret_cast<float4*>(a.partials + (int64_t)(c0 + qc.y) * a.dim) + threadIdx.x, tot);
+      if (PAIR && threadIdx.x == 0) __stcg(cp.partials + c0 + qc.y, ctot);
       __threadfence();
       __syncthreads();
       if (threadIdx.x == 0) s_last = (atomicAdd(&a.run_done[qc.x], 1) == nch - 1);
@@ -607,12 +630,17 @@
         for (int c = 0; c < nch; ++c)
           f4_acc(tot, __ldcg(reinterpret_cast<const float4*>(a.partials + (int64_t)(c0 + c) * a.dim) +
                              threadIdx.x));
+        if (PAIR && threadIdx.x == 0) {
+          ctot = 0.f;
+          for (int c = 0; c < nch; ++c) ctot = __fadd_rn(ctot, __ldcg(cp.partials + c0 + c));
+        }
       }
     }
     if (finish && threadIdx.x < LANES) {
       RowRegs row = load_row(a, key, threadIdx.x);
       apply_row_vec(a, key, threadIdx.x, tot, i, row);
     }
+    if (PAIR && finish && threadIdx.x == 0) apply_scalar(cp, key, 0, ctot, i);
     __syncthreads();
   }
 }
@@ -883,7 +911,7 @@
   }
 }
 
-template <int THREADS, typename IdxT>
+template <int THREADS, typename IdxT, bool COMP = false>
 __device__ __forceinline__ void process_runs_scalar(const BwdArgs& a, const SlotView& sv, uint64_t* sp,
                                                     const IdxT* s_start, int R, float* s_stagef, float* s_partf,
                                                     int* s_coop, int* s_ncoop, int64_t queue_base) {
@@ -898,7 +926,7 @@
     const int r = s_coop[cc];
     const int st = s_start[r], en = s_start[r + 1], len = en - st;
     if (queue_base >= 0 && len > bk::kQueueRun) {
-      if (threadIdx.x == 0) enqueue_run(a, queue_base + st, len);
+      if (!COMP && threadIdx.x == 0) enqueue_run(a, queue_base + st, len);
     } else {
       const int chunk = (len + THREADS - 1) / THREADS;
       const int j0 = st + threadIdx.x * chunk, j1 = min(en, j0 + chunk);
@@ -921,7 +949,8 @@
       }
     }
     __syncthreads();
-    for (int i = st + threadIdx.x; i < en; i += THREADS) sp[i] |= (uint64_t)kDonePos;
+    if (!COMP)
+      for (int i = st + threadIdx.x; i < en; i += THREADS) sp[i] |= (uint64_t)kDonePos;
   }
   __syncthreads();
   const int n = s_start[R];
@@ -1000,6 +1029,48 @@
   uint32_t keys[32];
 };
 
+struct WarpSmem1 {
+  float stage[32];
+  float carry;
+  uint32_t keys[32];
+};
+
+__device__ __forceinline__ float d1_stage(const BwdArgs& a, const SlotView& sv, WarpSmem1* ws, int lane, uint32_t key,
+                                          uint32_t pos, int nv) {
+  ws->keys[lane] = key;
+  if (lane < nv) {
+    float coef;
+    const float* src = grad_src(a, sv, pos, &coef);
+    ws->stage[lane] = __fmul_rn(src[0], coef);
+  }
+  return ws->carry;
+}
+
+__device__ __forceinline__ void d1_walk(const BwdArgs& a, WarpSmem1* ws, int lane, int nv, unsigned H, bool chunk_open,
+                                        uint32_t carry_key, float open_sum) {
+  const int nh = __popc(H);
+  const int lead = nh ? (__ffs(H) - 1) : nv;
+  if (lead > 0 && lane == 31) {
+    float acc = open_sum;
+    for (int i = 0; i < lead; ++i) acc = __fadd_rn(acc, ws->stage[i]);
+    if (lead == 32 && chunk_open)
+      ws->carry = acc;
+    else
+      apply_scalar(a, carry_key, 0, acc, 0);
+  }
+  if (lane < nh && !(lead > 0 && lane == 31)) {
+    const int h = __fns(H, 0, lane + 1);
+    const unsigned rest = (h == 31) ? 0u : (H >> (h + 1)) << (h + 1);
+    const int e_end = rest ? (__ffs(rest) - 1) : nv;
+    float acc = 0.f;
+    for (int i = h; i < e_end; ++i) acc = __fadd_rn(acc, ws->stage[i]);
+    if (e_end == 32 && chunk_open)
+      ws->carry = acc;
+    else
+      apply_scalar(a, ws->keys[h], 0, acc, 0);
+  }
+}
+
 __device__ __forceinline__ void sort4(uint64_t (&x)[4], int P, int lane) {
   for (int kk = 2; kk <= P; kk <<= 1) {
     for (int j = kk >> 1; j > 0; j >>= 1) {
@@ -1024,9 +1095,10 @@
   }
 }
 
-template <int LANES>
+template <int LANES, bool PAIR>
 __device__ __forceinline__ void warp_bucket_vec(const BwdArgs& a, const SlotView& sv, const BkArgs& k, int b,
-                                                WarpSmem<LANES>* ws) {
+                                                WarpSmem<LANES>* ws, const BwdArgs& cp, const SlotView& svc,
+                                                WarpSmem1* ws1) {
   constexpr int G = 32 / LANES;
   const int lane = threadIdx.x & 31;
   const int gi = lane / LANES, gl = lane % LANES;
@@ -1073,6 +1145,8 @@
         ws->stage[e * LANES + gl] = f4_scale1(reinterpret_cast<const float4*>(src)[gl], coef);
       }
     }
+    float open1 = 0.f;
+    if constexpr (PAIR) open1 = d1_stage(cp, svc, ws1, lane, key, pos, nv);
     __syncwarp();
     const uint32_t lastk = ws->keys[31];
     const bool chunk_open = (nv == 32) && next_first == lastk;
@@ -1101,16 +1175,11 @@
         apply_row_vec(a, kh, gl, acc, 0, row);
       }
     }
+    if constexpr (PAIR) d1_walk(cp, ws1, lane, nv, H, chunk_open, carry_key, open1);
     carry_key = chunk_open ? lastk : 0xFFFFFFFFu;
     __syncwarp();
   }
 }
-
-struct WarpSmem1 {
-  float stage[32];
-  float carry;
-  uint32_t keys[32];
-};
 
 __device__ __forceinline__ void warp_bucket_d1(const BwdArgs& a, const SlotView& sv, const BkArgs& k, int b,
                                                WarpSmem1* ws) {
@@ -1137,37 +1206,11 @@
     if (lane == 0) prevk = carry_key;
     const bool is_head = lane < nv && key != prevk;
     const unsigned H = __ballot_sync(0xffffffffu, is_head);
-    const int nh = __popc(H);
-    ws->keys[lane] = key;
-    const float open_sum = ws->carry;
-    if (lane < nv) {
-      float coef;
-      const float* src = grad_src(a, sv, pos, &coef);
-      ws->stage[lane] = __fmul_rn(src[0], coef);
-    }
+    const float open_sum = d1_stage(a, sv, ws, lane, key, pos, nv);
     __syncwarp();
     const uint32_t lastk = ws->keys[31];
     const bool chunk_open = (nv == 32) && next_first == lastk;
-    const int lead = nh ? (__ffs(H) - 1) : nv;
-    if (lead > 0 && lane == 31) {
-      float acc = open_sum;
-      for (int i = 0; i < lead; ++i) acc = __fadd_rn(acc, ws->stage[i]);
-      if (lead == 32 && chunk_open)
-        ws->carry = acc;
-      else
-        apply_scalar(a, carry_key, 0, acc, 0);
-    }
-    if (lane < nh && !(lead > 0 && lane == 31)) {
-      const int h = __fns(H, 0, lane + 1);
-      const unsigned rest = (h == 31) ? 0u : (H >> (h + 1)) << (h + 1);
-      const int e_end = rest ? (__ffs(rest) - 1) : nv;
-      float acc = 0.f;
-      for (int i = h; i < e_end; ++i) acc = __fadd_rn(acc, ws->stage[i]);
-      if (e_end == 32 && chunk_open)
-        ws->carry = acc;
-      else
-        apply_scalar(a, ws->keys[h], 0, acc, 0);
-    }
+    d1_walk(a, ws, lane, nv, H, chunk_open, carry_key, open_sum);
     carry_key = chunk_open ? lastk : 0xFFFFFFFFu;
     __syncwarp();
   }
@@ -1175,7 +1218,7 @@
 
 constexpr bool warp_mode_lanes(int lanes) { return lanes == 1 || lanes == 2 || lanes == 4 || lanes == 8; }
 
-template <int LANES>
+template <int LANES, bool PAIR = false>
 inline size_t bk_fused_smem(int n_slots, bool warp_mode) {
   size_t warp_bytes = 0;
   if (warp_mode) {
@@ -1183,27 +1226,39 @@
       warp_bytes = ((slot_smem_bytes(n_slots) + 15) & ~(size_t)15) + 8 * sizeof(WarpSmem<(LANES > 0 && LANES <= 8) ? LANES : 1>);
     else
       warp_bytes = ((slot_smem_bytes(n_slots) + 15) & ~(size_t)15) + 8 * sizeof(WarpSmem1);
+    if (PAIR) warp_bytes += 8 * sizeof(WarpSmem1);
   }
   const size_t med = bk_reduce_smem(n_slots, bk::kCap, bk::kThreads);
-  return warp_bytes > med ? warp_bytes : med;
-}
-
-template <int LANES>
+  return (warp_bytes > med ? warp_bytes : med) + (PAIR ? slot_region(n_slots) : 0);
+}
+
+template <int LANES, bool PAIR = false>
 __global__ void __launch_bounds__(bk::kThreads, ER_BK_MINB) bk_fused_kernel(const __grid_constant__ BwdArgs a,
-                                                                const __grid_constant__ BkArgs k) {
-  extern __shared__ __align__(16) unsigned char s_raw[];
+                                                                const __grid_constant__ BkArgs k,
+                                                                const __grid_constant__ BwdArgs cp) {
+  static_assert(!PAIR || (LANES > 0 && LANES <= 8), "a companion rides with a warp-mode vector primary");
+  extern __shared__ __align__(16) unsigned char s_raw_all[];
+  unsigned char* s_raw = s_raw_all + (PAIR ? slot_region(cp.n_slots) : 0);
   __shared__ int s_warp[bk::kThreads / 32 + 1];
   const int bid = blockIdx.x;
-  if (bid >= k.warp_ctas + k.med_ctas) {
-    one_row_cta<LANES>(a, bid - k.warp_ctas - k.med_ctas);
+  const int med_end = k.warp_ctas + (PAIR ? 2 : 1) * k.med_ctas;
+  if (bid >= med_end) {
+    const int x = bid - med_end, per_table = a.or_chunks * a.n_slots;
+    if (!PAIR || x < per_table)
+      one_row_cta<LANES>(a, x);
+    else if constexpr (PAIR)
+      one_row_cta<0>(cp, x - per_table);
     return;
   }
   const SlotView sv = load_slots(s_raw, a.slots, a.n_slots);
+  SlotView svc{};
+  if constexpr (PAIR) svc = load_slots(s_raw_all, cp.slots, cp.n_slots);
   if (bid < k.warp_ctas) {
     unsigned char* p = s_raw + ((slot_smem_bytes(a.n_slots) + 15) & ~(size_t)15);
     const int b = bid * 8 + (threadIdx.x >> 5);
     if constexpr (LANES > 0 && LANES <= 8) {
-      warp_bucket_vec<LANES>(a, sv, k, b, reinterpret_cast<WarpSmem<LANES>*>(p) + (threadIdx.x >> 5));
+      WarpSmem1* p1 = reinterpret_cast<WarpSmem1*>(reinterpret_cast<WarpSmem<LANES>*>(p) + 8) + (threadIdx.x >> 5);
+      warp_bucket_vec<LANES, PAIR>(a, sv, k, b, reinterpret_cast<WarpSmem<LANES>*>(p) + (threadIdx.x >> 5), cp, svc, p1);
     } else if constexpr (LANES == 0) {
       warp_bucket_d1(a, sv, k, b, reinterpret_cast<WarpSmem1*>(p) + (threadIdx.x >> 5));
     }
@@ -1211,7 +1266,8 @@
   }
   const BkSmem m = bk_carve(s_raw, a.n_slots, bk::kCap, bk::kThreads);
   const int n_med = k.w.n_big[1];
-  for (int xi = bid - k.warp_ctas; xi < n_med; xi += k.med_ctas) {
+  const bool comp = PAIR && bid >= k.warp_ctas + k.med_ctas;
+  for (int xi = bid - k.warp_ctas - (comp ? k.med_ctas : 0); xi < n_med; xi += k.med_ctas) {
     const int b = k.w.med_list[xi];
     const int n = k.w.bcnt[b];
     const int off = k.w.boff[b];
@@ -1221,7 +1277,10 @@
     __syncthreads();
     bk::bitonic_sort<bk::kThreads>(m.pairs, P);
     const int R = bk::run_starts<bk::kThreads, bk::kCap / bk::kThreads>(m.pairs, n, m.start, s_warp);
-    if constexpr (LANES > 0)
+    if (comp)
+      process_runs_scalar<bk::kThreads>(cp, svc, m.pairs, m.start, R, reinterpret_cast<float*>(m.stage),
+                                        reinterpret_cast<float*>(m.part), m.coop, m.ncoop, -1);
+    else if constexpr (LANES > 0)
       process_runs_vec<LANES, bk::kThreads>(a, sv, m.pairs, m.start, R, m.stage, m.part, m.coop, m.ncoop, -1);
     else
       process_runs_scalar<bk::kThreads>(a, sv, m.pairs, m.start, R, reinterpret_cast<float*>(m.stage),
@@ -1283,15 +1342,19 @@
   return true;
 }
 
-template <int LANES>
+template <int LANES, bool PAIR = false>
 __global__ void __launch_bounds__(bk::kBigThreads) bk_reduce_big_kernel(const __grid_constant__ BwdArgs a,
-                                                                        const __grid_constant__ BkArgs k) {
-  extern __shared__ __align__(16) unsigned char s_raw[];
+                                                                        const __grid_constant__ BkArgs k,
+                                                                        const __grid_constant__ BwdArgs cp) {
+  extern __shared__ __align__(16) unsigned char s_raw_all[];
+  unsigned char* s_raw = s_raw_all + (PAIR ? slot_region(cp.n_slots) : 0);
   __shared__ int s_warp[bk::kBigThreads / 32 + 1];
   __shared__ int s_flag;
   const int n_big = k.w.n_big[0];
   if ((int)blockIdx.x >= n_big) return;
   const SlotView sv = load_slots(s_raw, a.slots, a.n_slots);
+  SlotView svc{};
+  if constexpr (PAIR) svc = load_slots(s_raw_all, cp.slots, cp.n_slots);
   const BkSmem m = bk_carve(s_raw, a.n_slots, bk::kBigCap, bk::kBigThreads);
   for (int x = blockIdx.x; x < n_big; x += gridDim.x) {
     const int b = k.w.big_list[x];
@@ -1358,6 +1421,12 @@
         if (s_flag)
           for (int i = threadIdx.x; i < mwin; i += bk::kBigThreads) gp[i] = m.pairs[i];
       }
+      if constexpr (PAIR) {
+        process_runs_scalar<bk::kBigThreads, uint16_t, true>(cp, svc, m.pairs, m.start, R,
+                                                             reinterpret_cast<float*>(m.stage),
+                                                             reinterpret_cast<float*>(m.part), m.coop, m.ncoop, off + p);
+        __syncthreads();
+      }
       if constexpr (LANES > 0)
         process_runs_vec<LANES, bk::kBigThreads>(a, sv, m.pairs, m.start, R, m.stage, m.part, m.coop, m.ncoop, off + p);
       else
@@ -1430,13 +1499,14 @@
 
 static float adam_lr_t(const er_opt_t& o) { return adam_lr_t_of(o.lr, o.beta1_power, o.beta2_power); }
 
-template <int LANES>
-static void launch_long(const BwdArgs& a, cudaStream_t st) {
+template <int LANES, bool PAIR = false>
+static void launch_long(const BwdArgs& a, cudaStream_t st, const BwdArgs& cp = BwdArgs{}) {
   const size_t sl = slot_smem_bytes(a.n_slots);
   if constexpr (LANES > 0) {
     constexpr int TPE = (LANES <= 8) ? 1 : LANES;
-    const size_t smem_long = ((sl + 15) & ~(size_t)15) + (size_t)8 * LANES * sizeof(float4);
-    bwd_long_vec_kernel<LANES, TPE><<<4 * kSmCount, 256, smem_long, st>>>(a);
+    const size_t smem_long = ((sl + 15) & ~(size_t)15) + (size_t)8 * LANES * sizeof(float4) +
+                             (PAIR ? slot_region(cp.n_slots) : 0);
+    bwd_long_vec_kernel<LANES, TPE, PAIR><<<4 * kSmCount, 256, smem_long, st>>>(a, cp);
   } else {
     bwd_long_scalar_kernel<<<4 * kSmCount, 256, sl, st>>>(a);
   }
@@ -1498,31 +1568,41 @@
   count_launches(2);
 }
 
-template <int LANES>
-static void bk_launch_fused(BwdArgs a, const BwdWs& place, bool place_warp_mode, cudaStream_t st) {
+constexpr size_t kMaxDynSmem = 232448 - 1024;
+inline size_t bk_big_pair_smem(int n_slots) { return bk_reduce_smem(n_slots, bk::kBigCap, bk::kBigThreads) + slot_region(n_slots); }
+
+template <int LANES, bool PAIR = false>
+static void bk_launch_fused(BwdArgs a, const BwdWs& place, bool place_warp_mode, cudaStream_t st,
+                            const BwdArgs& cp = BwdArgs{}) {
   BkArgs k;
   k.w = place.bk;
   const int nb = bk::num_buckets(a.n, place_warp_mode);
   k.log2_nb = log2_of(nb);
   k.warp_ctas = place_warp_mode ? (nb >> 3) : 0;
   k.med_ctas = place_warp_mode ? kSmCount : nb;
-  const size_t smem = bk_fused_smem<LANES>(a.n_slots, place_warp_mode);
-  const size_t smem_big = bk_reduce_smem(a.n_slots, bk::kBigCap, bk::kBigThreads);
+  const size_t smem = bk_fused_smem<LANES, PAIR>(a.n_slots, place_warp_mode);
+  const size_t smem_big = bk_reduce_smem(a.n_slots, bk::kBigCap, bk::kBigThreads) + (PAIR ? slot_region(a.n_slots) : 0);
   static bool attr = false;
   if (!attr) {
-    cudaFuncSetAttribute(bk_fused_kernel<LANES>, cudaFuncAttributeMaxDynamicSharedMemorySize,
-                         (int)bk_fused_smem<LANES>(2048, true));
-    cudaFuncSetAttribute(bk_fused_kernel<LANES>, cudaFuncAttributePreferredSharedMemoryCarveout,
+    cudaFuncSetAttribute(bk_fused_kernel<LANES, PAIR>, cudaFuncAttributeMaxDynamicSharedMemorySize,
+                         (int)bk_fused_smem<LANES, PAIR>(2048, true));
+    cudaFuncSetAttribute(bk_fused_kernel<LANES, PAIR>, cudaFuncAttributePreferredSharedMemoryCarveout,
                          (int)cudaSharedmemCarveoutMaxShared);
-    cudaFuncSetAttribute(bk_reduce_big_kernel<LANES>, cudaFuncAttributeMaxDynamicSharedMemorySize,
-                         (int)bk_reduce_smem(2048, bk::kBigCap, bk::kBigThreads));
+    if (!PAIR)
+      cudaFuncSetAttribute(bk_reduce_big_kernel<LANES, PAIR>, cudaFuncAttributeMaxDynamicSharedMemorySize,
+                           (int)bk_reduce_smem(2048, bk::kBigCap, bk::kBigThreads));
     attr = true;
   }
-  const int extra = a.or_chunks * a.n_slots;
-  a.main_ctas = k.warp_ctas + k.med_ctas;
-  bk_fused_kernel<LANES><<<k.warp_ctas + k.med_ctas + extra, bk::kThreads, smem, st>>>(a, k);
-  bk_reduce_big_kernel<LANES><<<kSmCount, bk::kBigThreads, smem_big, st>>>(a, k);
-  launch_long<LANES>(a, st);
+  static size_t big_attr = 0;
+  if (PAIR && smem_big > big_attr) {
+    cudaFuncSetAttribute(bk_reduce_big_kernel<LANES, PAIR>, cudaFuncAttributeMaxDynamicSharedMemorySize, (int)smem_big);
+    big_attr = smem_big;
+  }
+  const int extra = (PAIR ? 2 : 1) * a.or_chunks * a.n_slots;
+  a.main_ctas = k.warp_ctas + (PAIR ? 2 : 1) * k.med_ctas;
+  bk_fused_kernel<LANES, PAIR><<<a.main_ctas + extra, bk::kThreads, smem, st>>>(a, k, cp);
+  bk_reduce_big_kernel<LANES, PAIR><<<kSmCount, bk::kBigThreads, smem_big, st>>>(a, k, cp);
+  launch_long<LANES, PAIR>(a, st, cp);
   count_launches(3);
 }
 
@@ -1548,6 +1628,19 @@
   return er::bwd_ws_bytes(n_lookups_cap > 0 ? n_lookups_cap : 1, dim > 0 ? dim : 1);
 }
 
+struct Companion {
+  float* table;
+  float* state0;
+  float* state1;
+  int32_t row_stride;
+  const er_slot_t* slots;
+  const float* const* grad_bufs;
+  int32_t n_bufs;
+  const float* seg_scale;
+  void* ws;
+  size_t ws_bytes;
+};
+
 static int embedding_bwd_impl(float* table, float* state0, float* state1, int64_t n_rows,
                               int32_t dim, int32_t row_stride, const int64_t* rows,
                               const float* weights, const int32_t* seg_ids,
@@ -1557,7 +1650,7 @@
                               const float* seg_scale, const er_opt_t* opt, int64_t* uniq_rows,
                               float* uniq_grads, int32_t* n_uniq, void* ws, size_t ws_bytes,
                               const void* sorted_ws, size_t sorted_ws_bytes, int32_t sorted_dim,
-                              er_stream_t stream) {
+                              er_stream_t stream, const Companion* comp = nullptr) {
   using namespace er;
   ER_REQUIRE(rows && slots && grad_bufs && opt, "null argument");
   ER_REQUIRE(table || uniq_rows, "nothing to do: table and uniq_rows are both NULL");
@@ -1579,9 +1672,24 @@
     ER_REQUIRE(k == ER_OPT_SGD || state0, "optimizer state0 missing");
     ER_REQUIRE((k != ER_OPT_LAZY_ADAM && k != ER_OPT_ADAM_ROWS) || state1, "adam needs state1 (v)");
   }
+  if (comp) {
+    ER_REQUIRE(comp->table && comp->slots && comp->grad_bufs, "companion: null argument");
+    ER_REQUIRE(comp->row_stride >= 1, "companion: bad row_stride");
+    ER_REQUIRE(comp->n_bufs > 0 && comp->n_bufs <= ER_MAX_BUFS, "companion: n_bufs must be in [1, ER_MAX_BUFS]");
+    ER_REQUIRE(opt->kind == ER_OPT_SGD || comp->state0, "companion: optimizer state0 missing");
+    ER_REQUIRE((opt->kind != ER_OPT_LAZY_ADAM && opt->kind != ER_OPT_ADAM_ROWS) || comp->state1,
+               "companion: adam needs state1 (v)");
+    for (int i = 0; i < comp->n_bufs; ++i) ER_REQUIRE(comp->grad_bufs[i] != nullptr, "companion: null gradient buffer");
+    if (uniq_rows || !(dim == 4 || dim == 8 || dim == 16 || dim == 32))
+      return fail(ER_ERR_UNSUPPORTED, "er_embedding_bwd_pair: the primary must be a table update of dim 4, 8, 16 or 32");
+    if (bk_big_pair_smem(n_slots) > kMaxDynSmem)
+      return fail(ER_ERR_UNSUPPORTED, "er_embedding_bwd_pair: too many slots for the big-bucket CTA's shared memory");
+  }
   if (n_lookups_cap == 0) return ER_OK;
   if (!ws || ws_bytes < bwd_ws_bytes(n_lookups_cap, dim))
     return fail(ER_ERR_WORKSPACE, "er_embedding_bwd: workspace too small");
+  if (comp && (!comp->ws || comp->ws_bytes < bwd_ws_bytes(n_lookups_cap, 1)))
+    return fail(ER_ERR_WORKSPACE, "er_embedding_bwd_pair: companion workspace too small");
   cudaStream_t st = as_stream(stream);
   BwdWs w = bwd_carve(ws, n_lookups_cap, dim);
   const int32_t* n_dev = row_ptr ? row_ptr + n_seg : nullptr;
@@ -1662,6 +1770,37 @@
     a.keys = nullptr;
     a.vals = nullptr;
     a.pairs = src.bk.pairs;
+    if (comp) {
+      if (!aligned)
+        return fail(ER_ERR_UNSUPPORTED, "er_embedding_bwd_pair: the primary's table, states and gradients must be "
+                                        "16-byte aligned");
+      const BwdWs cw = bwd_carve(comp->ws, n_lookups_cap, 1);
+      cudaMemsetAsync(cw.counters, 0, bk::zero_call_bytes(), st);
+      BwdArgs c = a;
+      c.table = comp->table;
+      c.state0 = comp->state0;
+      c.state1 = comp->state1;
+      c.dim = 1;
+      c.row_stride = comp->row_stride;
+      c.slots = comp->slots;
+      for (int i = 0; i < ER_MAX_BUFS; ++i) c.gbufs.p[i] = i < comp->n_bufs ? comp->grad_bufs[i] : nullptr;
+      c.seg_scale = comp->seg_scale;
+      c.counters = cw.counters;
+      c.long_list = cw.long_list;
+      c.run_done = cw.run_done;
+      c.chunk_list = cw.chunk_list;
+      c.partials = cw.partials;
+      c.or_partials = cw.one_row_partials;
+      c.or_tickets = cw.tickets;
+      switch (dim / 4) {
+        case 1: bk_launch_fused<1, true>(a, src, place_warp, st, c); break;
+        case 2: bk_launch_fused<2, true>(a, src, place_warp, st, c); break;
+        case 4: bk_launch_fused<4, true>(a, src, place_warp, st, c); break;
+        default: bk_launch_fused<8, true>(a, src, place_warp, st, c); break;
+      }
+      ER_CUDA_LAUNCH_CHECK();
+      return ER_OK;
+    }
     if (vec_dim && aligned) {
       switch (dim / 4) {
         case 1: bk_launch_fused<1>(a, src, place_warp, st); break;
@@ -1894,3 +2033,21 @@
   ER_CUDA_LAUNCH_CHECK();
   return ER_OK;
 }
+
+extern "C" int er_embedding_bwd_pair(float* table, float* state0, float* state1, int64_t n_rows, int32_t dim,
+                                     int32_t row_stride, const int64_t* rows, const float* weights,
+                                     const int32_t* seg_ids, const int32_t* row_ptr, int64_t n_seg,
+                                     int64_t n_lookups_cap, const er_slot_t* slots, int32_t n_slots,
+                                     const float* const* grad_bufs, int32_t n_bufs, const float* seg_scale,
+                                     const er_opt_t* opt, void* ws, size_t ws_bytes, float* c_table,
+                                     float* c_state0, float* c_state1, int32_t c_row_stride,
+                                     const er_slot_t* c_slots, const float* const* c_grad_bufs, int32_t c_n_bufs,
+                                     const float* c_seg_scale, void* c_ws, size_t c_ws_bytes,
+                                     const void* sorted_ws, size_t sorted_ws_bytes, int32_t sorted_dim,
+                                     er_stream_t stream) {
+  const Companion c{c_table, c_state0, c_state1, c_row_stride, c_slots, c_grad_bufs, c_n_bufs, c_seg_scale,
+                    c_ws, c_ws_bytes};
+  return embedding_bwd_impl(table, state0, state1, n_rows, dim, row_stride, rows, weights, seg_ids, row_ptr, n_seg,
+                            n_lookups_cap, slots, n_slots, grad_bufs, n_bufs, seg_scale, opt, nullptr, nullptr,
+                            nullptr, ws, ws_bytes, sorted_ws, sorted_ws_bytes, sorted_dim, stream, &c);
+}
diff --git a/easyrec_b200/embedding.py b/easyrec_b200/embedding.py
--- a/easyrec_b200/embedding.py
+++ b/easyrec_b200/embedding.py
@@ -158,16 +158,24 @@
 
 def fused_backward_update(call, rows, outs, opt, weights=None, row_ptr=None, seg_ids=None, sorted_from=None):
   a = call.arena
-  gbufs = []
-  for i, o in enumerate(outs):
-    g = o.grad
-    if g is None:
-      g = torch.zeros_like(o)
-    gbufs.append(g.contiguous())
   K.embedding_bwd(a.weight, a.state0, a.state1, a.dim, rows, call.slots_dev, call.n_slots,
-                  call.n_seg, gbufs, opt, call.ws, weights=weights, seg_ids=seg_ids,
+                  call.n_seg, _grad_bufs(outs), opt, call.ws, weights=weights, seg_ids=seg_ids,
                   row_ptr=row_ptr, seg_scale=call.seg_scale, sorted_from=sorted_from)
   adam_dense_decay(a, rows, opt, n_dev=None if row_ptr is None else row_ptr[call.n_seg:])
+
+
+def _grad_bufs(outs):
+  return [(o.grad if o.grad is not None else torch.zeros_like(o)).contiguous() for o in outs]
+
+
+def fused_backward_update_pair(call, c_call, rows, outs, c_outs, opt, weights=None, sorted_from=None):
+  a, c = call.arena, c_call.arena
+  K.embedding_bwd_pair(a.weight, a.state0, a.state1, a.dim, rows, call.slots_dev, call.n_slots, call.n_seg,
+                       _grad_bufs(outs), opt, call.ws, c.weight, c.state0, c.state1, c_call.slots_dev,
+                       _grad_bufs(c_outs), c_call.ws, weights=weights, seg_scale=call.seg_scale,
+                       c_seg_scale=c_call.seg_scale, sorted_from=sorted_from)
+  adam_dense_decay(a, rows, opt)
+  adam_dense_decay(c, rows, opt)
 
 
 class Placements(object):
diff --git a/easyrec_b200/input_layer.py b/easyrec_b200/input_layer.py
--- a/easyrec_b200/input_layer.py
+++ b/easyrec_b200/input_layer.py
@@ -1,4 +1,5 @@
 import collections
+import functools
 import os
 
 import numpy as np
@@ -419,19 +420,45 @@
       torch.cuda.current_stream().wait_stream(self._side)
     cur = torch.cuda.current_stream() if str(self.device).startswith('cuda') else None
     forked = False
+    companion = self._k7_pairs(self._pending) if cur is not None else {}
+    paired = set(companion.values())
+    first = True
     for idx, (m, rows, w, outs, seg_ids) in enumerate(self._pending):
+      if idx in paired:
+        continue
       src = self.placements.sorted_from(rows, m.arena.n_rows, m.arena.dim, m.ws)
-      if idx > 0 and src is not None and self._side is not None and cur is not None:
+      if idx in companion:
+        c = self._pending[companion[idx]]
+        upd = functools.partial(E.fused_backward_update_pair, m, c.call, rows, outs, c.outs, self.opt_holder['opt'],
+                                weights=w, sorted_from=src)
+      else:
+        upd = functools.partial(E.fused_backward_update, m, rows, outs, self.opt_holder['opt'], weights=w,
+                                seg_ids=seg_ids, sorted_from=src)
+      if not first and src is not None and self._side is not None and cur is not None:
         if not forked:
           self._side.wait_stream(cur)
           forked = True
         with torch.cuda.stream(self._side):
-          E.fused_backward_update(m, rows, outs, self.opt_holder['opt'], weights=w, seg_ids=seg_ids, sorted_from=src)
+          upd()
       else:
-        E.fused_backward_update(m, rows, outs, self.opt_holder['opt'], weights=w, seg_ids=seg_ids, sorted_from=src)
+        upd()
+      first = False
     if forked:
       cur.wait_stream(self._side)
     self._pending = []
+
+  @staticmethod
+  def _k7_pairs(pending):
+    pairs = {}
+    for i, p in enumerate(pending):
+      if p.call.arena.dim not in (4, 8, 16, 32) or p.seg_ids is not None:
+        continue
+      for j, q in enumerate(pending):
+        if (q.call.arena.dim == 1 and q.seg_ids is None and q.rows is p.rows and q.weights is p.weights and
+            j not in pairs.values() and q.call.arena.n_rows == p.call.arena.n_rows):
+          pairs[i] = j
+          break
+    return pairs
 
   def ep_hold_updates(self, on=True):
     for ex in self._exchanges():
diff --git a/easyrec_b200/kernels.py b/easyrec_b200/kernels.py
--- a/easyrec_b200/kernels.py
+++ b/easyrec_b200/kernels.py
@@ -307,6 +307,35 @@
                            _p(n_uniq), _p(ws), ws.numel(), _stream()), 'er_embedding_bwd')
 
 
+def embedding_bwd_pair(table, state0, state1, dim, rows, slots_dev, n_slots, n_seg, grad_bufs, opt, ws,
+                       c_table, c_state0, c_state1, c_slots_dev, c_grad_bufs, c_ws, weights=None, seg_scale=None,
+                       c_seg_scale=None, sorted_from=None):
+  lib = _lib.load()
+  n_rows, row_stride = _chk_rows(table, 'table')
+  c_rows, c_row_stride = _chk_rows(c_table, 'c_table')
+  if c_rows != n_rows:
+    raise _lib.ErError('embedding_bwd_pair: the companion table has %d rows, the primary %d' % (c_rows, n_rows))
+  for st, nm, stride in ((state0, 'state0', row_stride), (state1, 'state1', row_stride),
+                         (c_state0, 'c_state0', c_row_stride), (c_state1, 'c_state1', c_row_stride)):
+    if st is not None and _chk_rows(st, nm)[1] != stride:
+      raise _lib.ErError('%s must share its table\'s row stride' % nm)
+  _chk(rows, torch.int64, 'rows')
+  _chk(weights, torch.float32, 'weights')
+  _chk(seg_scale, torch.float32, 'seg_scale')
+  _chk(c_seg_scale, torch.float32, 'c_seg_scale')
+  for i, b in enumerate(list(grad_bufs) + list(c_grad_bufs)):
+    _chk(b, torch.float32, 'grad_bufs[%d]' % i)
+  src_ws, src_dim = sorted_from if sorted_from is not None else (None, 0)
+  _lib.check(
+      lib.er_embedding_bwd_pair(_p(table), _p(state0), _p(state1), n_rows, dim, row_stride, _p(rows), _p(weights),
+                                None, None, n_seg, rows.numel(), _p(slots_dev), n_slots, _buf_array(grad_bufs),
+                                len(grad_bufs), _p(seg_scale), ctypes.byref(opt), _p(ws), ws.numel(),
+                                _p(c_table), _p(c_state0), _p(c_state1), c_row_stride, _p(c_slots_dev),
+                                _buf_array(c_grad_bufs), len(c_grad_bufs), _p(c_seg_scale), _p(c_ws), c_ws.numel(),
+                                _p(src_ws), 0 if src_ws is None else src_ws.numel(), src_dim, _stream()),
+      'er_embedding_bwd_pair')
+
+
 def k7_warp_mode(dim):
   return dim in (1, 4, 8, 16, 32)
 
diff --git a/include/er_b200.h b/include/er_b200.h
--- a/include/er_b200.h
+++ b/include/er_b200.h
@@ -144,6 +144,16 @@
                                 float* uniq_grads, int32_t* n_uniq, void* ws, size_t ws_bytes,
                                 const void* sorted_ws, size_t sorted_ws_bytes, int32_t sorted_dim,
                                 er_stream_t stream);
+
+int er_embedding_bwd_pair(float* table, float* state0, float* state1, int64_t n_rows, int32_t dim,
+                          int32_t row_stride, const int64_t* rows, const float* weights, const int32_t* seg_ids,
+                          const int32_t* row_ptr, int64_t n_seg, int64_t n_lookups_cap, const er_slot_t* slots,
+                          int32_t n_slots, const float* const* grad_bufs, int32_t n_bufs, const float* seg_scale,
+                          const er_opt_t* opt, void* ws, size_t ws_bytes, float* c_table, float* c_state0,
+                          float* c_state1, int32_t c_row_stride, const er_slot_t* c_slots,
+                          const float* const* c_grad_bufs, int32_t c_n_bufs, const float* c_seg_scale, void* c_ws,
+                          size_t c_ws_bytes, const void* sorted_ws, size_t sorted_ws_bytes, int32_t sorted_dim,
+                          er_stream_t stream);
 
 int er_sparse_apply(float* table, float* state0, float* state1, int32_t dim,
                     int32_t row_stride, const int64_t* uniq_rows,
```

New measurement: 10.15 million, median of 6. +2.2%, better.
